# we1pingyu/CALD

Hardware: AMD Instinct MI355X
Metric: unlabeled images scored/sec (CALD consistency sweep) (higher is better)
Workload: dtype f32

## Files before the change

### cald_amd/_ffi.py

```python
import ctypes as C
import os

_HERE = os.path.dirname(os.path.abspath(__file__))
LIB_PATH = os.path.join(_HERE, "lib", "libcaldhip.so")
_lib = None

c_f = C.POINTER(C.c_float)
c_i = C.POINTER(C.c_int)
c_i64 = C.POINTER(C.c_int64)
c_d = C.POINTER(C.c_double)
c_u8 = C.POINTER(C.c_uint8)
c_i8 = C.POINTER(C.c_int8)


class ModelCfg(C.Structure):
    _fields_ = [("arch", C.c_int), ("depth", C.c_int), ("num_classes", C.c_int), ("min_size", C.c_int),
                ("max_size", C.c_int), ("box_score_thresh", C.c_float), ("box_nms_thresh", C.c_float),
                ("detections_per_img", C.c_int), ("rpn_pre_nms_top_n", C.c_int), ("rpn_post_nms_top_n", C.c_int),
                ("rpn_nms_thresh", C.c_float), ("precision", C.c_int)]


PRECISION = {"fp32": 0, "f16x3": 1}


# ... 141 lines not shown
    "cald_op_gap": (C.c_int, [C.c_void_p, c_f, C.c_int, C.c_int, C.c_int, c_f]),
    "cald_op_lossnet": (C.c_int, [C.c_void_p, C.c_int, c_f, c_f]),
    "cald_op_consistency": (C.c_int, [C.c_void_p, C.c_int, c_f, c_f, c_f, C.c_int, c_f, c_f, c_f, C.c_int, C.c_float, c_f]),
    "cald_op_cls_corr": (C.c_int, [C.c_void_p, C.c_int, c_f, c_i64, C.c_int, c_f]),
    "cald_op_score_batch": (C.c_int, [C.c_void_p, C.POINTER(ScoreProbe)]),
    "cald_op_pair_params": (C.c_int, [C.c_int, C.c_int, C.c_int, C.c_double, c_f]),
    "cald_op_ls_tail": (C.c_int, [C.c_int, c_f, C.c_int, c_f, c_i, c_i, c_d]),
    "cald_op_coco_match": (C.c_int, [C.c_void_p, C.c_int, c_i64, c_i64, c_d, c_d, c_d, c_d, c_u8, c_u8, C.c_int, c_d, C.c_int, c_d,
                                     C.POINTER(C.c_int32), c_u8, c_u8]),
    "cald_op_voc_match": (C.c_int, [C.c_void_p, C.c_int, c_i64, c_i64, c_d, c_u8, c_d, c_i64, C.c_int, c_d, C.c_int64, c_d, c_i64, c_u8, c_u8]),
    "cald_op_pil_resize": (C.c_int, [C.c_void_p, C.c_void_p, C.c_int, C.c_int, C.c_void_p, C.c_int, C.c_int]),
    "cald_op_cutout_rects": (C.c_int, [C.c_uint64, C.c_int, C.c_int, C.c_int, c_f, C.c_int, c_i, c_i]),
    "cald_op_cutout_geometry": (C.c_int, [C.c_int, C.c_int, C.c_int, C.c_int, C.c_int, c_i, C.c_int, c_i, c_i]),
    "cald_op_augment": (C.c_int, [C.c_void_p, C.c_int, C.c_double, C.c_uint64, C.c_void_p, C.c_int, C.c_int, C.c_int, c_f,
                                  C.c_void_p, c_f, c_i]),
    "cald_op_noise_stream": (C.c_int, [C.c_void_p, C.c_uint64, C.c_void_p, C.c_int, C.c_int, C.c_int, c_i, c_d, C.POINTER(C.c_void_p)]),
    "cald_op_frcnn_postprocess": (C.c_int, [C.c_void_p, C.c_int, C.c_int, c_f, c_f, c_f, C.c_int, C.c_int, C.c_int, C.c_int, C.c_float, C.c_float,
                                            C.c_int, c_f, c_f, c_i64, c_f, c_f, c_f, c_i]),
    "cald_op_frcnn_postprocess_min": (C.c_int, [C.c_void_p, C.c_int, C.c_int, c_f, c_f, c_f, C.c_int, C.c_int, C.c_int, C.c_int, C.c_float, C.c_float,
                                                C.c_int, C.c_float, c_f, c_f, c_i64, c_f, c_f, c_f, c_i]),
    "cald_op_ssm_postprocess": (C.c_int, [C.c_void_p, C.c_int, C.c_int, c_f, c_f, c_f, C.c_int, C.c_int, C.c_int, C.c_int, C.c_float, C.c_int,
                                          c_i, c_i, c_f, c_f, c_i8]),
    "cald_op_retina_postprocess": (C.c_int, [C.c_void_p, C.POINTER(c_f), C.POINTER(c_f), c_i, C.c_int, C.c_int, c_f] + [C.c_int] * 6
                                   + [C.c_float, C.c_float, C.c_int, c_f, c_f, c_i64, c_f, c_f, c_i]),
    "cald_op_retina_ssm_postprocess": (C.c_int, [C.c_void_p, C.POINTER(c_f), C.POINTER(c_f), c_i, C.c_int, C.c_int, c_f] + [C.c_int] * 6
                                       + [C.c_float, C.c_float, C.c_int, C.c_void_p, C.c_void_p, c_i, c_i, c_i, c_f, c_f, c_i8]),
    "cald_op_rpn_prune": (C.c_int, [C.c_void_p, C.POINTER(RpnPruneProbe)]),
    "cald_op_roi_align": (C.c_int, [C.c_void_p, C.POINTER(c_f), c_i, C.c_int, C.c_int, c_f, c_f]),
    "cald_op_conv2d": (C.c_int, [C.c_void_p, c_f, C.c_int, C.c_int, C.c_int, c_f, C.c_int, C.c_int, C.c_int, C.c_int,
                                 C.c_int, c_f, c_f, c_f, c_f, C.c_int, c_f]),
    "cald_op_conv_probe": (C.c_int, [C.c_void_p, C.c_int, C.POINTER(ConvProbe), C.c_int, C.c_int, C.c_int, C.c_char_p, C.c_int]),
    "cald_op_mfma_f16": (C.c_int, [C.c_void_p, C.POINTER(C.c_uint16), C.POINTER(C.c_uint16), C.POINTER(C.c_uint32), C.POINTER(C.c_uint32), C.c_int64]),
    "cald_op_conv2d_f16x3": (C.c_int, [C.c_void_p, c_f, C.c_int, C.c_int, C.c_int, c_f, C.c_int, C.c_int, C.c_int, C.c_int,
                                       C.c_int, c_f, c_f, c_f, c_f, C.c_int, c_f]),
    "cald_op_conv_bench": (C.c_int, [C.c_void_p] + [C.c_int] * 12 + [c_d, c_d]),
    "cald_op_row_pack_lookup": (C.c_int, [C.c_int, c_i, c_i, C.c_int, C.c_int, C.c_int64, c_i64, c_i, c_i64, c_i64]),
    "cald_op_transform_size": (C.c_int, [C.c_int, C.c_int, C.c_int, C.c_int, c_i, c_i, c_i, c_i]),
    "cald_debug_tensor": (C.c_int, [C.c_void_p, C.c_char_p, C.c_int, c_f, C.c_int64, c_i64]),
    "cald_jpeg_info": (C.c_int, [C.c_void_p, C.c_size_t, c_i, c_i, c_i]),
    "cald_jpeg_decode_batch": (C.c_int, [C.c_void_p, C.c_int, C.POINTER(C.c_void_p), C.POINTER(C.c_size_t), C.POINTER(C.c_void_p)]),
    "cald_jpeg_probe": (C.c_int, [C.c_void_p, C.c_size_t, c_i, c_i, c_i, c_i]),
    "cald_jpeg_decode_batch_any": (C.c_int, [C.c_void_p, C.c_int, C.POINTER(C.c_void_p), C.POINTER(C.c_size_t), C.POINTER(C.c_void_p)]),
    "cald_jpeg_decode_host": (C.c_int, [C.c_void_p, C.c_size_t, C.c_void_p]),
    "cald_profile_enable": (C.c_int, [C.c_void_p, C.c_int]),
    "cald_profile_read": (C.c_int, [C.c_void_p, c_d, c_d, c_i64, c_d]),
    "cald_profile_prune": (C.c_int, [C.c_void_p, c_d, c_d, c_d, c_d, c_d]),
    "cald_profile_roi_rows": (C.c_int, [C.c_void_p, c_d, c_i64]),
    "cald_profile_cutout": (C.c_int, [C.c_void_p, c_d, c_d, c_i64, c_i64]),
    "cald_model_set_cutout_reuse": (C.c_int, [C.c_void_p, C.c_int, c_i]),
    "cald_profile_cutout_stages": (C.c_int, [C.c_void_p, c_d, c_d, c_d, c_d, c_i64]),
    "cald_model_set_cutout_retention_cap": (C.c_int, [C.c_void_p, C.c_int64, c_i64]),
    "cald_op_cutout_fpn_geometry": (C.c_int, [C.c_int, C.c_int, C.c_int, C.c_int, C.c_int, c_i, C.c_int, c_i, c_i]),
    "cald_model_set_look_fuse": (C.c_int, [C.c_void_p, C.c_int, c_i]),
    "cald_model_set_row_packing": (C.c_int, [C.c_void_p, C.c_int, c_i]),
    "cald_model_set_box_min_size": (C.c_int, [C.c_void_p, C.c_float, c_f]),
    "cald_profile_dump": (C.c_int, [C.c_void_p, C.c_char_p]),
    "cald_train_packed_floats": (C.c_int, [C.c_int] * 6 + [c_i64]),
    "cald_train_pack_conv": (C.c_int, [C.c_void_p] * 5 + [C.c_int] * 6 + [C.c_void_p]),
    "cald_train_pack_plan_scratch_floats": (C.c_int, [C.c_int, C.POINTER(PackJob), c_i64]),
    "cald_train_pack_plan_create": (C.c_int, [C.c_void_p, C.c_int, C.POINTER(PackJob), C.c_void_p, C.c_int64, C.POINTER(C.c_void_p)]),
    "cald_train_pack_plan_run": (C.c_int, [C.c_void_p, C.c_void_p]),
    "cald_train_pack_plan_destroy": (C.c_int, [C.c_void_p]),
    "cald_train_conv": (C.c_int, [C.c_void_p, C.c_int, C.c_int, C.c_int, C.c_void_p, C.c_int, C.c_void_p] + [C.c_int] * 8
                        + [C.c_void_p, C.c_void_p, C.c_int, C.c_int, C.c_void_p, C.c_void_p, C.c_int]),
    "cald_train_conv_group": (C.c_int, [C.c_void_p, C.c_int, C.c_int, c_i, C.POINTER(C.c_void_p), C.c_int, C.POINTER(C.c_void_p)] + [C.c_int] * 8
                              + [C.POINTER(C.c_void_p), C.POINTER(C.c_void_p), C.c_int]),
    "cald_train_conv_wgrad": (C.c_int, [C.c_void_p, C.c_int, C.c_int, C.c_int, C.c_void_p, C.c_int, C.c_int, C.c_void_p, C.c_int,
                                        C.c_int, C.c_int, C.c_int, C.c_int, C.c_int, C.c_void_p, C.c_void_p, C.c_void_p, C.c_int]),
    "cald_train_linear_wgrad": (C.c_int, [C.c_void_p, C.c_int, C.c_void_p, C.c_int, C.c_void_p, C.c_int, C.c_int, C.c_int,
                                          C.c_void_p, C.c_void_p, C.c_int]),
    "cald_train_wgrad_plan": (C.c_int, [C.c_longlong] + [C.c_int] * 12 + [C.POINTER(WgradPlan)]),
    "cald_train_relu_bwd": (C.c_int, [C.c_void_p, C.c_longlong, C.c_int, C.c_void_p, C.c_void_p, C.c_void_p]),
    "cald_train_add": (C.c_int, [C.c_void_p, C.c_longlong, C.c_void_p, C.c_void_p, C.c_void_p]),
    "cald_train_dilate": (C.c_int, [C.c_void_p] + [C.c_int] * 7 + [C.c_void_p, C.c_void_p]),
    "cald_train_upsample_bwd": (C.c_int, [C.c_void_p] + [C.c_int] * 6 + [C.c_void_p, C.c_void_p]),
    "cald_train_rpn_proposals": (C.c_int, [C.c_void_p, C.c_int, C.c_int, C.c_int, c_i, C.POINTER(C.c_void_p), c_i, C.c_int, C.c_int, C.c_int,
                                           C.c_float, C.c_float, C.c_void_p, C.c_void_p]),
    "cald_train_roi_sample_host": (C.c_int, [C.c_int, c_i, c_i, c_i, C.c_void_p, C.c_void_p, C.c_void_p, C.c_int, C.c_double, C.c_int, C.c_int,
                                             C.c_void_p, C.c_void_p, C.c_void_p, C.c_void_p, C.c_void_p, C.c_void_p, c_i, c_i, c_i]),
    "cald_train_roi_gather": (C.c_int, [C.c_void_p, C.c_void_p, C.c_void_p, C.c_void_p, C.c_int, C.c_int, C.c_int] + [C.c_float] * 4 + [C.c_void_p, C.c_void_p]),
    "cald_train_anchors": (C.c_int, [C.c_void_p, C.c_int, C.c_int, C.c_int, c_i, C.c_void_p]),
    "cald_train_match": (C.c_int, [C.c_void_p, C.c_int, C.c_void_p, C.c_int, C.c_void_p, C.c_float, C.c_float, C.c_int, C.c_void_p, C.c_void_p]),
    "cald_train_box_encode": (C.c_int, [C.c_void_p, C.c_int, C.c_void_p, C.c_void_p, C.c_float, C.c_float, C.c_float, C.c_float, C.c_void_p]),
    "cald_train_roi_align": (C.c_int, [C.c_void_p, C.POINTER(C.c_void_p), c_i, C.c_int, C.c_int, C.c_void_p, C.c_void_p]),
    "cald_train_roi_align_bwd": (C.c_int, [C.c_void_p, C.c_int, C.POINTER(C.c_void_p), c_i, C.c_int, C.c_int, C.c_void_p, C.c_void_p]),
    "cald_train_softmax_ce": (C.c_int, [C.c_void_p, C.c_int, C.c_int, C.c_int, C.c_void_p, C.c_void_p, C.c_float, C.c_void_p, C.c_void_p]),
    "cald_train_smooth_l1": (C.c_int, [C.c_void_p, C.c_int, C.c_void_p, C.c_void_p, C.c_void_p, C.c_float, C.c_float, C.c_void_p, C.c_float,
                                       C.c_void_p, C.c_void_p]),
    "cald_train_focal_loss": (C.c_int, [C.c_void_p, C.c_int, c_i, C.c_int, C.c_int, C.c_int, C.c_void_p, C.c_void_p, C.c_void_p, C.c_void_p,
                                        C.c_void_p, C.c_float, C.c_float, C.c_void_p, C.c_void_p]),
    "cald_train_bce_logits": (C.c_int, [C.c_void_p, C.c_int, C.c_void_p, C.c_void_p, C.c_void_p, C.c_float, C.c_void_p, C.c_void_p]),
    "cald_train_softmax_ce_seg": (C.c_int, [C.c_void_p, C.c_int, c_i, C.c_int, C.c_int, C.c_void_p, C.c_void_p, C.c_void_p, C.c_void_p, C.c_void_p]),
    "cald_train_smooth_l1_seg": (C.c_int, [C.c_void_p, C.c_int, c_i, C.c_void_p, C.c_void_p, C.c_void_p, C.c_float, c_f, C.c_void_p, C.c_void_p,
                                           C.c_void_p]),
    "cald_train_bce_logits_seg": (C.c_int, [C.c_void_p, C.c_int, c_i, C.c_void_p, C.c_void_p, C.c_void_p, C.c_void_p, C.c_void_p, C.c_void_p]),
    "cald_train_focal_loss_seg": (C.c_int, [C.c_void_p, C.c_int, c_i, C.c_int, C.c_int, C.c_int, C.c_void_p, C.c_void_p, C.c_void_p, C.c_void_p,
                                            c_f, C.c_float, C.c_void_p, C.c_void_p, C.c_void_p, C.c_void_p]),
    "cald_train_seg_mean": (C.c_int, [C.c_void_p, C.c_int, C.c_void_p, C.c_void_p]),
    "cald_train_add_bcast": (C.c_int, [C.c_void_p, C.c_int, C.c_longlong, C.c_int, C.c_void_p, C.c_void_p, C.c_void_p, C.c_void_p, C.c_longlong]),
    "cald_train_preprocess": (C.c_int, [C.c_void_p, C.c_int, C.POINTER(C.c_void_p), C.POINTER(C.c_void_p), c_i, C.c_int, C.c_int, C.c_void_p]),
    "cald_train_maxpool": (C.c_int, [C.c_void_p, C.c_int, C.c_int, C.c_int, C.c_int, C.c_void_p, C.c_void_p]),
    "cald_train_subsample2": (C.c_int, [C.c_void_p, C.c_int, C.c_int, C.c_int, C.c_int, C.c_void_p, C.c_void_p]),
    "cald_train_sgd": (C.c_int, [C.c_void_p, C.c_longlong, C.c_void_p, C.c_void_p, C.c_void_p, C.c_float, C.c_float, C.c_float, C.c_int]),
    "cald_train_seg_cache_size": (C.c_int, []),
    "cald_comm_unique_id": (C.c_int, [C.c_void_p]),
    "cald_comm_init_rank": (C.c_int, [C.c_void_p, C.c_void_p, C.c_int, C.c_int, C.POINTER(C.c_void_p)]),
# ... 36 lines not shown
```

### cald_amd/csrc/conv_h4.hip

```cpp
#include "h16.h"

typedef float f32x16 __attribute__((ext_vector_type(16)));
typedef _Float16 h8 __attribute__((ext_vector_type(8)));
typedef __attribute__((address_space(3))) void lds_void;

#define H4_STAGE 32768
#define H4_NSTAGE 4

template <int EPI, bool HEAD = false>
__device__ __forceinline__ void conv_h4_body(const ConvArgs& a, const int blk) {
    extern __shared__ __attribute__((aligned(1024))) unsigned char smem[];
    const int tid = threadIdx.x, lane = tid & 63, wave = __builtin_amdgcn_readfirstlane(tid >> 6);
    const int NT = a.CoutPad >> 8;
    const int MT2 = (a.total_mtiles + 1) >> 1;
    int mt2, nt;
    {
        const int total = MT2 * NT, b = blk, xcd = b & 7, idx = b >> 3, Q = total >> 3, R = total & 7;
        const int L = (xcd < R ? xcd * (Q + 1) : R * (Q + 1) + (xcd - R) * Q) + idx;
        mt2 = L / NT; nt = L - mt2 * NT;
    }
    const int n0 = nt << 8;
    const int Cin = a.Cin, KW = a.KW, KH = a.KH, CoutPad = a.CoutPad;

    const bool ldA = wave < 4;
    const int lw = wave & 3;
    const int l_row = lane >> 2;
    const int l_piece = (lane & 3) ^ ((lane >> 4) & 3);
    int voff[4];
    unsigned rowmask[4];
    __amdgpu_buffer_rsrc_t rs;
    int Wi_l = 1;
    if (ldA) {
        const int mt = 2 * mt2 + (lw >> 1);
        const int v = seg_find_view(a.seg_out, a.V, mt);
        const LevelSeg so = a.seg_out[v], si = a.seg_in[v];
        const int Wo = so.W, Hi = si.H, Wi = si.W;
        Wi_l = Wi;
        int Mv = so.H * Wo;
        if (a.dyn_rows) { const int d = a.dyn_rows[v]; Mv = d < Mv ? d : Mv; }
        if (mt >= a.total_mtiles) Mv = 0;
        const int mrow0 = (mt - so.tile_start) * 128 + (lw & 1) * 64;
#pragma unroll
        for (int i = 0; i < 4; i++) {
            const int m = mrow0 + 16 * i + l_row;
            const int oy = m / Wo, ox = m - oy * Wo;
            const int iy0 = oy * a.stride - a.pad, ix0 = ox * a.stride - a.pad;
            unsigned msk = 0;
            if (m < Mv)
                for (int t = 0; t < KH * KW; t++) {
                    const int th = t / KW, tw = t - th * KW;
                    const int iy = iy0 + th, ix = ix0 + tw;
                    if (iy >= 0 && iy < Hi && ix >= 0 && ix < Wi) msk |= 1u << t;
                }
            rowmask[i] = msk;
            voff[i] = ((oy * a.stride) * Wi + ox * a.stride) * Cin * 4 + l_piece * 16;
        }
        const unsigned char* in_v = reinterpret_cast<const unsigned char*>(a.in16) + (si.pix_off * (long long)Cin - (long long)a.pad * (Wi + 1) * Cin) * 4;
        rs = __builtin_amdgcn_make_buffer_rsrc((void*)in_v, 0, 0x7FFE0000, 0x00020000);
    } else {
#pragma unroll
        for (int i = 0; i < 4; i++) {
            const int n = 64 * lw + 16 * i + l_row;
            rowmask[i] = 0xffffffffu;
            voff[i] = ((l_piece >> 1) * CoutPad + n) * 32 + (l_piece & 1) * 16;
        }
        rs = __builtin_amdgcn_make_buffer_rsrc((void*)(reinterpret_cast<const unsigned char*>(a.w16) + (long long)n0 * 32), 0, 0x7FFE0000, 0x00020000);
    }
    const int lds_l = (ldA ? 0 : 16384) + lw * 4096;
    int u_kh = 0, u_kw = 0, u_ci = 0, u_kt = 0;

#define H4_ISSUE(SLOT)                                                                                                       \
    {                                                                                                                        \
        const int soffA = ((u_kh * Wi_l + u_kw) * Cin + u_ci) * 4, soffB = u_kt * (2 * CoutPad * 32);                        \
        const int soff = ldA ? soffA : soffB;                                                                                \
        const unsigned bit = ldA ? (1u << (u_kh * KW + u_kw)) : 1u;                                                          \
        _Pragma("unroll") for (int i = 0; i < 4; i++) {                                                                      \
            const int vo = (rowmask[i] & bit) ? voff[i] : 0x7FFF0000;                                                        \
            __builtin_amdgcn_raw_ptr_buffer_load_lds(rs, (lds_void*)(smem + (SLOT) * H4_STAGE + lds_l + i * 1024), 16, vo, soff, 0, 0); \
        }                                                                                                                    \
        u_kt++; u_kw++;                                                                                                      \
        const bool ww = u_kw == KW; u_kw = ww ? 0 : u_kw; u_kh += ww ? 1 : 0;                                                \
        const bool wh = u_kh == KH; u_kh = wh ? 0 : u_kh; u_ci += wh ? 16 : 0;                                               \
    }

    const int wm = wave >> 2, wn = wave & 3;
    const int l31 = lane & 31, kh_lane = lane >> 5, sw = (l31 >> 2) & 3;
    const int fa = (wm * 128 + l31) * 64, fb = 16384 + (wn * 64 + l31) * 64;
    const int s_hi = ((kh_lane) ^ sw) * 16, s_lo = ((2 + kh_lane) ^ sw) * 16;

    f32x16 acc[4][2];
#pragma unroll
    for (int i = 0; i < 4; i++)
#pragma unroll
        for (int j = 0; j < 2; j++)
#pragma unroll
            for (int r = 0; r < 16; r++) acc[i][j][r] = 0.0f;

    const int KT = a.Kpad >> 4;
// ... 92 lines not shown
#undef H4_MFMA4
#undef H4_READ
#undef H4_ISSUE
#undef H4_STEP

    if (HEAD) {
        int tid = threadIdx.x;
        asm volatile("" : "+v"(tid));
        const int wave = __builtin_amdgcn_readfirstlane(tid >> 6), wm = wave >> 2, wn = wave & 3, l31 = tid & 31, kh_lane = (tid >> 5) & 1;
        const float unscale = a.w16_unscale;
        const float bs0 = a.bias[wn * 64 + l31], bs1 = a.bias[wn * 64 + 32 + l31];
        const bool have2 = 2 * mt2 + 1 < a.total_mtiles;
#pragma unroll
        for (int t = 0; t < 2; t++) {
            __syncthreads();
            if (wm == 0 || have2) {
                int sbase = (wm << 16) + (kh_lane << 12) + (((wn * 16 + (l31 >> 2)) ^ (4 * kh_lane)) << 4) + (l31 & 3) * 4;
                asm volatile("" : "+v"(sbase));
#pragma unroll
                for (int j = 0; j < 2; j++) {
                    const float bs = j ? bs1 : bs0;
#pragma unroll
                    for (int ii = 0; ii < 2; ii++)
#pragma unroll
                        for (int r = 0; r < 16; r++) {
                            float val = acc[2 * t + ii][j][r] * unscale;
                            val = val + bs;
                            val = val > 0.0f ? val : 0.0f;
                            const int rc = ii * 32 + (r & 3) + 8 * (r >> 2);
                            *reinterpret_cast<float*>(smem + (sbase ^ (((j << 7) ^ (rc << 4)) | (rc << 10)))) = val;
                        }
                }
            }
            __syncthreads();
            if (wave < 6) {
                const int srow = tid & 127, q = wave >> 1;
                const int mt = 2 * mt2 + (srow >> 6);
                if (mt < a.total_mtiles) {
                    const int v = seg_find_view(a.seg_out, a.V, mt);
                    const LevelSeg so = a.seg_out[v];
                    const int m = (mt - so.tile_start) * 128 + 64 * t + (srow & 63);
                    const float4* const hrow = reinterpret_cast<const float4*>(smem + srow * 1024);
                    typedef const __attribute__((address_space(4))) float cfloat;
                    cfloat* const w = (cfloat*)a.head_w + q * 256;
                    float s0 = 0.0f;
#pragma unroll 16
                    for (int g = 0; g < 64; g++) {
                        const float4 hv = hrow[(g ^ srow) & 63];
                        s0 = __builtin_fmaf(hv.x, w[4 * g], s0);
                        s0 = __builtin_fmaf(hv.y, w[4 * g + 1], s0);
                        s0 = __builtin_fmaf(hv.z, w[4 * g + 2], s0);
                        s0 = __builtin_fmaf(hv.w, w[4 * g + 3], s0);
                    }
                    if (m < so.H * so.W) a.head_out[(so.pix_off + m) * (long long)a.head_ld + q] = s0 + a.head_b[q];
                }
            }
        }
        return;
    }

    const int mt = 2 * mt2 + wm;
    if (mt >= a.total_mtiles) return;
    const int v = seg_find_view(a.seg_out, a.V, mt);
    const LevelSeg so = a.seg_out[v];
    int Mv = so.H * so.W;
    if (a.dyn_rows) { const int d = a.dyn_rows[v]; Mv = d < Mv ? d : Mv; }
    const int m0 = (mt - so.tile_start) * 128;
    if (m0 >= Mv) return;
    h16_epilogue<EPI, 4, 2>(a, acc, so, v, m0, n0 + wn * 64, Mv, lane);
}

template <int EPI>
__global__ __launch_bounds__(512, 2) void conv_h4_kernel(const ConvArgs a) { conv_h4_body<EPI>(a, (int)blockIdx.x); }
__global__ __launch_bounds__(512, 2) void conv_h4_group_kernel(const ConvGroup g) {
    int i = 0;
    while (i + 1 < g.n && g.blk0[i + 1] <= (int)blockIdx.x) i++;
    const int local = (int)blockIdx.x - g.blk0[i];
    const ConvArgs& a = g.p[i];
    if (local >= ((a.total_mtiles + 1) >> 1) * (a.CoutPad >> 8)) return;
    conv_h4_body<0>(a, local);
}

__global__ __launch_bounds__(512, 2) void conv_h4_look_kernel(const ConvGroup g) {
    int i = 0;
    while (i + 1 < g.n && g.blk0[i + 1] <= (int)blockIdx.x) i++;
    const int local = (int)blockIdx.x - g.blk0[i];
    const ConvArgs& a = g.p[i];
    if (local >= (a.total_mtiles + 1) >> 1) return;
    conv_h4_body<0, true>(a, local);
}

static bool h4_covers(const ConvArgs& a) {
    if (a.head_out && !(a.head_w && a.head_ld >= 3 && a.Cout == 256 && a.CoutPad == 256 && !a.residual && !a.up && !a.dyn_rows && a.bias && !a.scale && a.relu)) return false;
    return a.w16 && a.in16 && !a.in_relu && a.CoutPad % 256 == 0 && a.Cin % 16 == 0 && a.KH * a.KW <= 32 && !a.mask && !(a.residual && a.up) &&
           !a.gather && !a.row_map && !a.energy4 && (a.out || a.out16 || a.head_out);
}
static int h4_mode() { static const int mode = getenv("CALD_H4") ? atoi(getenv("CALD_H4")) : 1; return mode; }
static PerDeviceOnce h4_once[5];
const char* launch_conv_h4(const ConvArgs& a, hipStream_t stream, bool forced) {
    if (!(forced || h4_mode()) || !h4_covers(a) || a.head_out) return nullptr;
    const int wgs = ((a.total_mtiles + 1) >> 1) * (a.CoutPad >> 8);
    if (!forced && h4_mode() == 1 && (a.Kpad < 1024 || wgs < 512)) return nullptr;
    if (wgs == 0) return "none (no output tiles)";
    const dim3 grid((unsigned)wgs), block(512);
    const size_t lds = (size_t)H4_NSTAGE * H4_STAGE;
    if (a.residual) { allow_big_lds(h4_once[1], conv_h4_kernel<1>); hipLaunchKernelGGL((conv_h4_kernel<1>), grid, block, lds, stream, a); return "conv_h4_kernel<1>"; }
    if (a.up) { allow_big_lds(h4_once[2], conv_h4_kernel<2>); hipLaunchKernelGGL((conv_h4_kernel<2>), grid, block, lds, stream, a); return "conv_h4_kernel<2>"; }
    allow_big_lds(h4_once[0], conv_h4_kernel<0>); hipLaunchKernelGGL((conv_h4_kernel<0>), grid, block, lds, stream, a);
    return "conv_h4_kernel<0>";
}
static int h4_group_plan(const ConvArgs* p, int n, bool forced, ConvGroup* g, int* blocks) {
    if (!(forced || h4_mode()) || n < 1 || n > CALD_MAX_GROUP) return 0;
    int blk = 0;
    const bool head = p[0].head_out != nullptr;
    for (int i = 0; i < n; i++) {
        if (!h4_covers(p[i]) || p[i].residual || p[i].up || (p[i].head_out != nullptr) != head) return 0;
        if (g) { g->blk0[i] = blk; g->p[i] = p[i]; }
        blk += (((p[i].total_mtiles + 1) >> 1) * (p[i].CoutPad >> 8) + 7) & ~7;
    }
    if (g) { g->n = n; g->blk0[n] = blk; }
    if (!forced && h4_mode() == 1 && (blk < 512 || p[0].Kpad < 1024)) return 0;
    *blocks = blk;
    return blk == 0 ? 2 : 1;
}
bool conv_h4_group_takes(const ConvArgs* p, int n, bool forced) { int blk; return h4_group_plan(p, n, forced, nullptr, &blk) != 0; }
const char* launch_conv_h4_group(const ConvArgs* p, int n, hipStream_t stream, bool forced) {
    ConvGroup g; int blk = 0;
    const int take = h4_group_plan(p, n, forced, &g, &blk);
    if (!take) return nullptr;
    if (take == 2) return "none (no output tiles)";
    if (p[0].head_out) {
        allow_big_lds(h4_once[4], conv_h4_look_kernel);
        hipLaunchKernelGGL(conv_h4_look_kernel, dim3((unsigned)blk), dim3(512), (size_t)H4_NSTAGE * H4_STAGE, stream, g);
        return "conv_h4_look_kernel";
    }
    allow_big_lds(h4_once[3], conv_h4_group_kernel);
    hipLaunchKernelGGL(conv_h4_group_kernel, dim3((unsigned)blk), dim3(512), (size_t)H4_NSTAGE * H4_STAGE, stream, g);
    return "conv_h4_group_kernel";
}
```

### cald_amd/csrc/ctx.hip

```cpp
#include "host.h"

static thread_local char g_err[512] = "";
int cald_host::fail(int code, const char* fmt, ...) {
    va_list ap; va_start(ap, fmt); vsnprintf(g_err, sizeof(g_err), fmt, ap); va_end(ap);
    return code;
}

int cald_internal_fail(int code, const char* fmt, ...) {
    va_list ap; va_start(ap, fmt); vsnprintf(g_err, sizeof(g_err), fmt, ap); va_end(ap);
    return code;
}
void cald_internal_train_release(cald_ctx* c);

extern "C" const char* cald_last_error(void) { return g_err; }
extern "C" int cald_version(void) { return 100; }

hipStream_t cald_internal_stream(cald_ctx* c) { return c->stream; }
int cald_internal_device(cald_ctx* c) { return c->device; }
const float* cald_internal_zeros(cald_ctx* c) { return c->d_zeros; }
int cald_internal_scratch(cald_ctx* c, size_t bytes, void** out) {
    if (bytes > c->train_scratch_cap) {
        HIPCHK(hipStreamSynchronize(c->stream));
        if (c->train_scratch) HIPCHK(hipFree(c->train_scratch));
        c->train_scratch = nullptr; c->train_scratch_cap = 0;
// ... 109 lines not shown
    return 0;
}

extern "C" int cald_profile_prune(cald_ctx* c, double* look_ms, double* look_flops, double* selected_frac2, double* worst_bound_ratio, double* pruned_flops) {
    if (!c) return fail(CALD_ERR_INVALID, "ctx is null");
    HIPCHK(hipStreamSynchronize(c->stream));
    double ms = 0.0, fl = 0.0;
    for (const ProfLaunch& L : c->prof_launches)
        if (L.tag) { float t = 0.f; HIPCHK(hipEventElapsedTime(&t, L.e0, L.e1)); ms += t; fl += L.flops; }
    unsigned long long st[4] = {0, 0, 0, 0};
    HIPCHK(hipMemcpy(st, c->d_prune_stat, 32, hipMemcpyDeviceToHost));
    if (look_ms) *look_ms = ms;
    if (look_flops) *look_flops = fl;
    if (selected_frac2) for (int l = 0; l < 2; l++) selected_frac2[l] = st[2 * l + 1] ? (double)st[2 * l] / (double)st[2 * l + 1] : 0.0;
    if (worst_bound_ratio) *worst_bound_ratio = (double)c->prune_worst;
    if (pruned_flops) {
        double fl2 = 0.0;
        for (int l = 0; l < 2; l++) if (st[2 * l + 1]) fl2 += c->prof_prune_flops_cap[l] / 2.0 * (1.0 - (double)st[2 * l] / (double)st[2 * l + 1]);
        *pruned_flops = fl2;
    }
    return 0;
}

extern "C" int cald_profile_roi_rows(cald_ctx* c, double* mean_rows_per_view, int64_t* views) {
    if (!c) return fail(CALD_ERR_INVALID, "ctx is null");
    HIPCHK(hipStreamSynchronize(c->stream));
    unsigned long long rows = 0;
    HIPCHK(hipMemcpy(&rows, c->d_roi_rows, 8, hipMemcpyDeviceToHost));
    if (views) *views = c->prof_roi_views;
    if (mean_rows_per_view) *mean_rows_per_view = c->prof_roi_views ? (double)rows / (double)c->prof_roi_views : 0.0;
    return 0;
}

extern "C" int cald_profile_cutout(cald_ctx* c, double* rows3, double* dense_rows3, int64_t* batches, int64_t* fallbacks) {
    if (!c) return fail(CALD_ERR_INVALID, "ctx is null");
    for (int i = 0; i < 3; i++) { if (rows3) rows3[i] = c->cut_rows[i]; if (dense_rows3) dense_rows3[i] = c->cut_dense[i]; }
    if (batches) *batches = c->cut_batches;
    if (fallbacks) *fallbacks = c->cut_fallbacks;
    return 0;
}

extern "C" int cald_profile_cutout_stages(cald_ctx* c, double* rows6, double* dense_rows6, double* tiles6, double* dense_tiles6, int64_t* kept3) {
    if (!c) return fail(CALD_ERR_INVALID, "ctx is null");
    for (int i = 0; i < 6; i++) {
        if (rows6) rows6[i] = c->cut_st_rows[i];
        if (dense_rows6) dense_rows6[i] = c->cut_st_dense[i];
        if (tiles6) tiles6[i] = c->cut_st_tiles[i];
        if (dense_tiles6) dense_tiles6[i] = c->cut_st_dense_tiles[i];
    }
    if (kept3) for (int i = 0; i < 3; i++) kept3[i] = c->cut_kept[i];
    return 0;
}

extern "C" int cald_profile_dump(cald_ctx* c, const char* path) {
    if (!c || !path) return fail(CALD_ERR_INVALID, "null argument");
    HIPCHK(hipStreamSynchronize(c->stream));
    FILE* f = fopen(path, "w");
    if (!f) return fail(CALD_ERR_INVALID, "cannot open %s", path);
    fprintf(f, "launch,desc,gflop,ms,tflops\n");
    std::vector<unsigned long long> lg((size_t)CALD_PRUNE_LOG * 4, 0ull);
    if (!c->prof_gather.empty()) HIPCHK(hipMemcpy(lg.data(), c->d_prune_log, lg.size() * 8, hipMemcpyDeviceToHost));
    for (size_t i = 0; i < c->prof_launches.size(); i++) {
        const ProfLaunch& L = c->prof_launches[i];
        float t = 0.f; hipEventElapsedTime(&t, L.e0, L.e1);
        double fl = L.flops;
        const char* extra = L.tag ? ",f16x3-lookahead" : "";
        auto g = c->prof_gather.find(i);
        if (g != c->prof_gather.end()) {
            for (int l = 0; l < 2; l++) {
                const unsigned long long sel = lg[(size_t)g->second.log * 4 + 2 * l], tot = lg[(size_t)g->second.log * 4 + 2 * l + 1];
                if (tot) fl -= g->second.cap[l] * (1.0 - (double)sel / (double)tot);
            }
            extra = ",gathered-rows";
        }
        fprintf(f, "%zu,\"%s%s\",%.3f,%.4f,%.2f\n", i, L.desc.c_str(), extra, fl / 1e9, t, fl / (t * 1e-3) / 1e12);
    }
    fclose(f);
    return 0;
}
extern "C" int cald_profile_prune_fallbacks(cald_ctx* c, int64_t* n) {
    if (!c || !n) return fail(CALD_ERR_INVALID, "null argument");
    *n = (int64_t)c->prune_fallbacks;
    return 0;
}

int cald_host::prof_begin(cald_ctx* c, ProfLaunch& t) {
    if (!c->prof) return 0;
    HIPCHK(hipEventCreate(&t.e0)); HIPCHK(hipEventCreate(&t.e1));
    HIPCHK(hipEventRecord(t.e0, c->stream));
    return 0;
}
int cald_host::prof_end(cald_ctx* c, ProfLaunch& t, double flops, int tag, const char* fmt, ...) {
    if (!c->prof) return 0;
    HIPCHK(hipEventRecord(t.e1, c->stream));
    char d[160];
    va_list ap; va_start(ap, fmt); vsnprintf(d, sizeof(d), fmt, ap); va_end(ap);
    t.flops = flops; t.tag = tag; t.desc = d;
    c->prof_launches.push_back(t); c->prof_flops += flops;
    return 0;
}

int cald_host::conv_refused(const ConvArgs& a) {
    return fail(CALD_ERR_UNSUPPORTED, "no conv kernel implements this launch (Cin=%d Cout=%d k=%dx%d residual=%d up=%d mask=%d gather=%d energy4=%d out16=%d)",
                a.Cin, a.Cout, a.KH, a.KW, a.residual != nullptr, a.up != nullptr, a.mask != nullptr, a.gather != nullptr, a.energy4 != nullptr,
                a.out16 != nullptr);
}
// ... 9 lines not shown
```

### cald_amd/csrc/forward.hip

```cpp
#include "host.h"

#define ROI_DENSE_VIEWS 32
void cald_host::build_plan(BatchPlan& P, int V, const ViewDesc* views, const int (*hp)[2], bool retina) {
    memset(&P, 0, sizeof(P));
    for (int l = 0; l < CALD_MAX_LEVELS; l++) {
        long long off = 0; int tile = 0;
        for (int v = 0; v <= V; v++) {
            LevelSeg& s = P.seg[l][v];
            s.pix_off = off; s.tile_start = tile;
            if (v == V) break;
            int H, W;
            if (l == 7 && retina) { int h6 = (hp[v][0] / 32 - 1) / 2 + 1, w6 = (hp[v][1] / 32 - 1) / 2 + 1; H = (h6 - 1) / 2 + 1; W = (w6 - 1) / 2 + 1; }
            else if (l == 7) { H = 1; W = CALD_ROI_CAP; }
            else if (l == 8) {
                const int first = v * ROI_DENSE_VIEWS, cnt = first < V ? (V - first < ROI_DENSE_VIEWS ? V - first : ROI_DENSE_VIEWS) : 0;
                H = cnt ? 1 : 0; W = cnt * CALD_ROI_CAP;
            }
            else if (l == 6) { H = (hp[v][0] / 32 - 1) / 2 + 1; W = (hp[v][1] / 32 - 1) / 2 + 1; }
            else { H = hp[v][0] >> l; W = hp[v][1] >> l; }
            s.H = H; s.W = W;
            off += (long long)H * W;
            tile += (H * W + 127) / 128;
        }
    }
// ... 14 lines not shown
        T1 = B.get<float>(px[2] * 128); T2 = B.get<float>(px[2] * 64); D = B.get<float>(px[2] * 256);
        for (int i = 0; i < 4; i++) { Cf[i] = B.get<float>(px[2 + i] * CCH[i]); S.only(Cf[i]); }
        S.only(p1); S.only(T1); S.only(T2); S.only(X[0]); S.only(X[1]); S.only(D);
    }
};
struct PyramidBufs {
    float *inner[4], *Pf[5]; unsigned* Pf16[5];
    void layout(Bump& B, SplitReg& S, const long long* px, bool retina) {
        const int first = retina ? 3 : 2, nl = retina ? 3 : 4;
        for (int i = 0; i < nl; i++) { inner[i] = B.get<float>(px[first + i] * 256); S.only(inner[i]); }
        for (int i = 0; i < 5; i++) {
            Pf[i] = B.get<float>(px[first + i] * 256);
            if (i == 4 || (retina && i < 3)) S.only(Pf[i]); else S.both(Pf[i], Pf16[i], px[first + i] * 256);
        }
    }
};
void cald_host::RetinaTailBufs::layout(Bump& B, int V, int K, int per_class, int maxa) {
    max_anchors = maxa;
    cand_cap = 1024; while (cand_cap < maxa) cand_cap <<= 1;
    cand_count = B.get<int>((size_t)V * K); cand_key = B.get<unsigned long long>((size_t)V * K * cand_cap);
    cand_box = B.get<float>((size_t)V * K * cand_cap * 4); cand_skip = B.get<unsigned char>((size_t)V * K * cand_cap);
    kept_anchor = B.get<int>((size_t)V * K * per_class); kept_box = B.get<float>((size_t)V * K * per_class * 4); kept_count = B.get<int>((size_t)V * K);
}
void cald_host::RetinaSsmBufs::layout(Bump& B, int V, int K, int per_class, int maxa) {
    cand_cap = maxa > 0 ? maxa : 1; nblk = (cand_cap + 255) / 256;
    const size_t VK = (size_t)V * K, rows = VK * per_class;
    cand_count = B.get<int>(VK); blk_off = B.get<int>(VK * nblk); list = B.get<int>(VK * cand_cap); vmax = B.get<unsigned>(V); al = B.get<int>(V);
    picks = B.get<int>(VK * CALD_SSM_RETINA_TAKE); n_picks = B.get<int>(VK);
    kept_anchor = B.get<int>(rows); kept_box = B.get<float>(rows * 4); kept_count = B.get<int>(VK);
    row_off = B.get<int>(VK); count = B.get<int>(V); total = B.get<int>(1);
    boxes = B.get<float>(rows * 4); scores = B.get<float>(rows); labels = B.get<signed char>(rows * (K - 1));
}
struct RetinaBufs {
    float *ret_t[2][2][5], *cls_h[5], *reg_h[5]; RetinaTailBufs tail;
    void layout(Bump& B, SplitReg& S, const long long* px, int V, int cls_ld, int K, int per_class, int max_anchors, RetinaSsmBufs* ssm_tail) {
        for (int h = 0; h < 2; h++) for (int q = 0; q < 2; q++) for (int i = 0; i < 5; i++) { ret_t[h][q][i] = B.get<float>(px[3 + i] * 256); S.only(ret_t[h][q][i]); }
        for (int i = 0; i < 5; i++) { cls_h[i] = B.get<float>(px[3 + i] * cls_ld); reg_h[i] = B.get<float>(px[3 + i] * 36); }
        if (ssm_tail) ssm_tail->layout(B, V, K, per_class, max_anchors); else tail.layout(B, V, K, per_class, max_anchors);
    }
};
void cald_host::ProposalBufs::layout(Bump& B, int V) { proposals = B.get<float>((size_t)V * CALD_ROI_CAP * 4); prop_count = B.get<int>(V); }
struct RpnBufs {
    float *rpn_tl[5], *rpn_h[5], *cand_box, *sorted_box, *sorted_raw; unsigned long long* cand_key; int* sorted_count; ProposalBufs prop;
    void layout(Bump& B, const long long* px, int V, int pre) {
        for (int i = 0; i < 5; i++) { rpn_tl[i] = B.get<float>(px[2 + i] * 256); rpn_h[i] = B.get<float>(px[2 + i] * 15); }
        cand_key = B.get<unsigned long long>((size_t)V * 5 * pre); cand_box = B.get<float>((size_t)V * 5 * pre * 4);
        sorted_box = B.get<float>((size_t)V * 5 * pre * 4); sorted_raw = B.get<float>((size_t)V * 5 * pre * 4); sorted_count = B.get<int>(V);
        prop.layout(B, V);
    }
};
struct PruneBufs {
    float *energy[2] = {}, *pn[2] = {}, *rows[2][2] = {}; int *map[2][2] = {}, *nsel[2] = {}; unsigned* p16[2] = {}; unsigned* tau = nullptr;
    float* look[2] = {};
    void layout(Bump& B, const long long* px, int V, bool capture) {
        for (int i = 0; i < 2; i++) {
            energy[i] = B.get<float>(px[2 + i] * 4); pn[i] = B.get<float>(px[2 + i]); p16[i] = B.get<unsigned>(px[2 + i] * 256);
            for (int s2 = 0; s2 < 2; s2++) { rows[s2][i] = B.get<float>(px[2 + i] * 15); map[s2][i] = B.get<int>(px[2 + i]); }
            if (capture) look[i] = B.get<float>(px[2 + i] * 15);
        }
        for (int s2 = 0; s2 < 2; s2++) nsel[s2] = B.get<int>((size_t)2 * V);
        tau = B.get<unsigned>((size_t)2 * V);
    }
};
void cald_host::RoiBufs::layout(Bump& B, int V, int C) { order = B.get<int>((size_t)V * 1024); roi = B.get<float>((size_t)V * CALD_ROI_CAP * 49 * C); }
void cald_host::PostBufs::layout(Bump& B, int V, int C, int cap) {
    key_cap = cap;
    prob = B.get<float>((size_t)V * CALD_ROI_CAP * C); pmax = B.get<float>((size_t)V * CALD_ROI_CAP);
    keys = B.get<unsigned long long>((size_t)V * key_cap); cbox = B.get<float>((size_t)V * 2 * key_cap * 4); key_count = B.get<int>(V);
    skip = B.get<unsigned char>((size_t)V * key_cap);
}
void cald_host::SsmBufs::layout(Bump& B, int V, int C, int cap) {
    const size_t K = (size_t)(C - 1), rows = (size_t)V * K * cap;
    prob = B.get<float>((size_t)V * CALD_ROI_CAP * C); vmax = B.get<unsigned>(V);
    kept_prop = B.get<int>(rows); kept_box = B.get<float>(rows * 4); cls_count = B.get<int>((size_t)V * K); row_off = B.get<int>((size_t)V * K);
    al = B.get<int>(V); count = B.get<int>(V); total = B.get<int>(1);
    boxes = B.get<float>(rows * 4); scores = B.get<float>(rows * K); labels = B.get<signed char>(rows * K);
}
struct BoxBufs {
    RoiBufs roi; float *f6, *f7, *pr; PostBufs post;
    void layout(Bump& B, SplitReg& S, int V, int pred_ld, int C, int key_cap) {
        roi.layout(B, V, 256);
        f6 = B.get<float>((size_t)V * CALD_ROI_CAP * 1024); f7 = B.get<float>((size_t)V * CALD_ROI_CAP * 1024);
        S.only(roi.roi); S.only(f6); S.only(f7);
        pr = B.get<float>((size_t)V * CALD_ROI_CAP * pred_ld);
        post.layout(B, V, C, key_cap);
    }
};
struct AuditBufs {
    unsigned long long *next_key, *trunc_key, *kept_key; float* post_maxc;
    void layout(Bump& B, int V, int det_cap) {
        next_key = B.get<unsigned long long>((size_t)V * 10); trunc_key = B.get<unsigned long long>((size_t)V * 2);
        kept_key = B.get<unsigned long long>((size_t)V * det_cap); post_maxc = B.get<float>(V);
    }
};

RoiArgs cald_host::roi_args(const RoiBufs& S, const float* const* feat, const BatchPlan* plan, int C, int V, const ProposalBufs& P, bool out16) {
    RoiArgs ro{};
    for (int i = 0; i < 4; i++) { ro.feat[i] = feat[i]; ro.seg[i] = plan->seg[2 + i]; }
    ro.C = C; ro.V = V; ro.proposals = P.proposals; ro.prop_count = P.prop_count; ro.out = S.roi; ro.order = S.order; ro.out16 = out16 ? 1 : 0;
    return ro;
}
PostArgs cald_host::post_args(const PostBufs& S, const float* pred, int pred_ld, int C, int V, const ProposalBufs& P, const ViewDesc* views,
                              float score_thr, float nms_thr, const DetBuffers& det) {
    PostArgs pa{};
    pa.pred = pred; pa.pred_ld = pred_ld; pa.C = C; pa.V = V; pa.proposals = P.proposals; pa.prop_count = P.prop_count; pa.views = views; pa.score_thr = score_thr; pa.nms_thr = nms_thr;
    pa.prob = S.prob; pa.pmax = S.pmax; pa.keys = S.keys; pa.cbox = S.cbox; pa.key_count = S.key_count; pa.key_cap = S.key_cap; pa.det = det;
    pa.skip = S.skip;
    return pa;
}
// ... 57 lines not shown
    for (int v = 0; v < V; v++) {
        const LevelSeg& s = seg[v];
        if (!(s.H % 8 == 0 && s.W % 16 == 0 && seg[v + 1].tile_start - s.tile_start == (s.H / 8) * (s.W / 16))) return false;
    }
    return true;
}
static double fill_conv_args(cald_model* m, ConvArgs& a, const ConvLayer& L, const float* in, float* out, int lin, int lout, int V, bool relu,
                             const float* residual = nullptr, const float* up = nullptr, int lup = 0, const int* dyn = nullptr,
                             bool in_relu = false) {
    const BatchPlan* dp = m->ctx->d_plan;
    a.in = in; a.out = out; a.w = L.w; a.w4 = L.w4; a.w16 = L.w16; a.w16_unscale = L.w16_unscale; a.bias = L.bias; a.scale = L.scale; a.shift = L.shift;
    a.residual = residual; a.up = up;
    a.seg_in = dp->seg[lin]; a.seg_out = dp->seg[lout]; a.seg_up = dp->seg[lup];
    a.dyn_rows = dyn; a.row_map = nullptr; a.gather = nullptr; a.V = V;
    a.Cin = L.Cin; a.Cout = L.Cout; a.CoutPad = L.CoutPad; a.Kpad = L.Kpad;
    a.KH = L.KH; a.KW = L.KW; a.stride = L.stride; a.pad = L.pad; a.relu = relu ? 1 : 0;
    a.total_mtiles = level_tiles(m->plan, lout, V); a.packed_rows = 0;
    a.out_ld = L.Cout; a.in_relu = in_relu ? 1 : 0; a.zeros = m->ctx->d_zeros;
    a.mask = nullptr;
    for (int v = 0; v < V; v++) {
        const long long pin = (long long)m->plan.seg[lin][v].H * m->plan.seg[lin][v].W, pout = (long long)m->plan.seg[lout][v].H * m->plan.seg[lout][v].W;
        if (pin * L.Cin * 4 > 0x7FFE0000LL || pout * L.Cout * 4 > 0x7FFE0000LL) {
            return (double)fail(CALD_ERR_UNSUPPORTED, "a view's activation tensor exceeds 2 GB (level %d -> %d, %lld x %d / %lld x %d elements)", lin, lout, pin, L.Cin, pout, L.Cout);
        }
    }
    a.in16 = nullptr; a.out16 = nullptr; a.ex16 = 0; a.energy4 = nullptr; a.trace = nullptr;
    a.head_w = nullptr; a.head_out = nullptr; a.head_ld = 0; a.head_b[0] = a.head_b[1] = a.head_b[2] = 0.0f;
    if (!m->split.empty()) {
        const float* ex = residual ? residual : up;
        if (ex) {
            auto fe = m->split.find(ex);
            if (fe != m->split.end() && fe->second.fp32_dead) {
                if (!a.w16) return (double)fail(CALD_ERR_STATE, "a layer outside conv_h3 / conv_h4 adds a tensor kept in split form only");
                a.ex16 = 1;
            }
        }
        auto fi = m->split.find(in);
        if (fi != m->split.end()) {
            if (a.w16 && !in_relu) a.in16 = fi->second.s16;
            else if (fi->second.fp32_dead) return (double)fail(CALD_ERR_STATE, "a layer outside conv_h3 reads a tensor kept in split form only");
        }
        auto fo = m->split.find(out);
        if (fo != m->split.end()) {
            if (!a.w16) return (double)fail(CALD_ERR_STATE, "a layer outside conv_h3 writes a tensor with a split twin");
            a.out16 = fo->second.s16;
            if (fo->second.fp32_dead) a.out = nullptr;
        }
    }
    a.wstem = L.wstem && stem_grid_exact(m->plan.seg[lout], V) ? L.wstem : nullptr;
    return 2.0 * (double)level_pix(m->plan, lout, V) * (double)L.Cout * (double)(L.KH * L.KW * L.CinTrue);
}
bool cald_host::conv_pack_default() {
    static const bool on = !(getenv("CALD_CONV_PACK") && atoi(getenv("CALD_CONV_PACK")) == 0);
    return on;
}
static void offer_packing(cald_model* m, ConvArgs& a, int lin, int lout, int lup, int V) {
    if (!(m->row_packing < 0 ? conv_pack_default() : m->row_packing != 0) || a.dyn_rows || a.row_map || a.gather || a.mask) return;
    a.packed_rows = conv_pack_rows(m->plan.seg[lin], m->plan.seg[lout], a.up ? m->plan.seg[lup] : nullptr, V, a.Cin, a.out_ld);
}
static int conv_on(cald_model* m, const ConvLayer& L, const float* in, float* out, int lin, int lout, int V, bool relu,
                   const float* residual = nullptr, const float* up = nullptr, int lup = 0, const int* dyn = nullptr,
                   bool in_relu = false) {
    ConvArgs a;
    const double flops = fill_conv_args(m, a, L, in, out, lin, lout, V, relu, residual, up, lup, dyn, in_relu);
    if (flops < 0.0) return (int)flops;
    offer_packing(m, a, lin, lout, lup, V);
    return run_conv(m->ctx, a, flops);
}
static int conv_pair_on(cald_model* m, const ConvLayer& L2, const ConvLayer& L3, const float* in, float* mid, float* out, int lin, int lout,
                        int V, const float* residual) {
    cald_ctx* c = m->ctx;
    if (m->cfg.precision == CALD_PRECISION_FP32 && L2.stride == 1 && lin == lout) {
        ConvArgs a2, a3;
            const double f2 = fill_conv_args(m, a2, L2, in, mid, lin, lout, V, true);
        const double f3 = fill_conv_args(m, a3, L3, mid, out, lout, lout, V, true, residual);
        if (f2 < 0.0 || f3 < 0.0) return (int)(f2 < 0.0 ? f2 : f3);
        ProfLaunch t; int rc;
        if ((rc = prof_begin(c, t))) return rc;
        if (launch_conv_p4_fused(a2, a3, c->stream) != nullptr)
            return prof_end(c, t, f2 + f3, 0, "mt=%d,Cin=%d,Cout=%d,k=3x3+1x1,s=1,fused->%d", a2.total_mtiles, a2.Cin, a2.Cout, a3.Cout);
        if (c->prof) { hipEventDestroy(t.e0); hipEventDestroy(t.e1); }
    }
    int rc = conv_on(m, L2, in, mid, lin, lout, V, true);
    if (rc) return rc;
    return conv_on(m, L3, mid, out, lout, lout, V, true, residual);
}
static int conv_group_on(cald_model* m, const ConvSpec* sp, int n, int V) {
    ConvArgs a[CALD_MAX_GROUP];
    double flops = 0.0; int tiles = 0;
    for (int i = 0; i < n; i++) {
        const double f = fill_conv_args(m, a[i], *sp[i].L, sp[i].in, sp[i].out, sp[i].level, sp[i].level, V, sp[i].relu, nullptr, nullptr, 0, sp[i].dyn);
        if (f < 0.0) return (int)f;
        a[i].row_map = sp[i].row_map;
        if (sp[i].in16) a[i].in16 = sp[i].in16;
        if (sp[i].out16) a[i].out16 = sp[i].out16;
        a[i].energy4 = sp[i].energy4;
        offer_packing(m, a[i], sp[i].level, sp[i].level, 0, V);
        flops += f; tiles += a[i].total_mtiles;
    }
    cald_ctx* c = m->ctx;
    const char* names[CALD_MAX_GROUP];
    ProfLaunch t; int rc;
    if ((rc = prof_begin(c, t))) return rc;
    const int launches = launch_conv_group(a, n, c->stream, names);
    if (c->prof) c->prof_extra_launches += launches - 1;
    if ((rc = prof_end(c, t, flops, c->prof_tag_now, "mt=%d,Cin=%d,Cout=%d,k=%dx%d,s=%d,group=%d", tiles, a[0].Cin, a[0].Cout, a[0].KH, a[0].KW, a[0].stride, n))) return rc;
// ... 113 lines not shown
        HIPCHK(hipEventSynchronize(c->stage_ev[si]));
        memcpy(c->h_stage[si], &m->plan, sizeof(BatchPlan));
        memcpy(c->h_stage[si] + sizeof(BatchPlan), views, sizeof(ViewDesc) * V);
        HIPCHK(hipMemcpyAsync(c->d_plan, c->h_stage[si], sizeof(BatchPlan), hipMemcpyHostToDevice, c->stream));
        HIPCHK(hipMemcpyAsync(c->d_views, c->h_stage[si] + sizeof(BatchPlan), sizeof(ViewDesc) * V, hipMemcpyHostToDevice, c->stream));
        HIPCHK(hipEventRecord(c->stage_ev[si], c->stream));
        dp = c->d_plan; st = c->stream;
        m->dbg.clear();
        return 0;
    }
    int dense_block(const Bottleneck& B, const float* cur, float* dst, int lvl, int lout) {
        int rc; const float* idn = cur;
        if (B.has_down) { if ((rc = conv_on(m, B.down, cur, Fb.D, lvl, lout, V, false))) return rc; idn = Fb.D; }
        if ((rc = conv_on(m, B.c1, cur, Fb.T1, lvl, lvl, V, true))) return rc;
        return conv_pair_on(m, B.c2, B.c3, Fb.T1, Fb.T2, dst, lvl, lout, V, idn);
    }
    int gathered_block(const Bottleneck& B, int b, const float* cur, float* dst, int lvl, int lout) {
        int rc; const float* idn = cur;
        if (B.has_down) { if ((rc = gconv_on(m, B.down, cur, Fb.D, lvl, lout, V, false, nullptr, *ru, b, 0))) return rc; idn = Fb.D; }
        if ((rc = gconv_on(m, B.c1, cur, Fb.T1, lvl, lvl, V, true, nullptr, *ru, b, 1))) return rc;
        if ((rc = gconv_on(m, B.c2, Fb.T1, Fb.T2, lvl, lout, V, true, nullptr, *ru, b, 0))) return rc;
        return gconv_on(m, B.c3, Fb.T2, dst, lout, lout, V, true, idn, *ru, b, 0);
    }
    int body() {
        int rc;
        launch_preprocess(c->d_views, dp->seg[0], Fb.in0, V, max_pix0, st);
        m->dbg["input"] = {Fb.in0, 0, 4, 0};
        if ((rc = conv_on(m, m->conv1, Fb.in0, Fb.c1, 0, 1, V, true))) return rc;
        m->dbg["conv1"] = {Fb.c1, 1, 64, 0};
        launch_maxpool(Fb.c1, Fb.p1, dp->seg[1], dp->seg[2], 64, V, max_pix2, st, m->split.count(Fb.p1) != 0);
        m->dbg["pool1"] = {Fb.p1, 2, 64, 0};
        const float* cur = Fb.p1; int lvl = 2, layer = 0, xi = 0;
        for (size_t b = 0; b < m->blocks.size(); b++) {
            const Bottleneck& B = m->blocks[b];
            const int lout = lvl + (B.c2.stride == 2 ? 1 : 0);
            const bool kept = ru && (int)b < ru->nblk;
            float* dst = kept ? ru->out[b] : (B.layer_end ? Fb.Cf[layer] : Fb.X[xi]);
            if ((rc = kept && ru->mode == 2 && ru->gather[layer] ? gathered_block(B, (int)b, cur, dst, lvl, lout) : dense_block(B, cur, dst, lvl, lout))) return rc;
            if (B.layer_end) Fb.Cf[layer] = dst;
            cur = dst; lvl = lout;
            if (B.layer_end) layer++; else xi ^= 1;
        }
        const char* cn[4] = {"C2", "C3", "C4", "C5"};
        for (int i = 0; i < 4; i++) m->dbg[cn[i]] = {Fb.Cf[i], 2 + i, CCH[i], 0};
        return 0;
    }
    void name_pyramid(int first, int n) { for (int i = 0; i < n; i++) m->dbg["P" + std::to_string(first + i)] = {Fp.Pf[i], first + i, 256, 0}; }
    int fpn() {
        const int first = retina ? 3 : 2, nl = retina ? 3 : 4, c0 = 4 - nl;
        int rc; ConvSpec sp[4];
        const bool kept = ru && ru->fpn && !retina;
        if (kept) {
            for (int i = 0; i < 4; i++) Fp.Pf[i] = ru->pf[i];
            if (prune) for (int i = 0; i < 2; i++) { Fq.p16[i] = ru->p16[i]; Fq.energy[i] = ru->energy[i]; }
        }
        if ((rc = conv_on(m, m->fpn_inner[nl - 1], Fb.Cf[3], Fp.inner[nl - 1], 5, 5, V, false))) return rc;
        for (int i = nl - 2; i >= 0; i--)
            if ((rc = conv_on(m, m->fpn_inner[i], Fb.Cf[c0 + i], Fp.inner[i], first + i, first + i, V, false, nullptr, Fp.inner[i + 1], first + 1 + i))) return rc;
        for (int i = 0; i < nl; i++) m->dbg["inner" + std::to_string(first + i)] = {Fp.inner[i], first + i, 256, 0};
        for (int i = 0; i < nl; i++) sp[i] = {&m->fpn_layer[i], Fp.inner[i], Fp.Pf[i], first + i, false};
        if (prune)
            for (int i = 0; i < 2; i++) { sp[i].out16 = Fq.p16[i]; sp[i].energy4 = Fq.energy[i]; }
        if ((rc = kept && ru->mode == 2 && ru->gather_fpn ? gconv_group_on(m, sp, nl, V, *ru) : conv_group_on(m, sp, nl, V))) return rc;
        if (!retina) return 0;
        if ((rc = conv_on(m, m->p6, Fp.Pf[2], Fp.Pf[3], 5, 6, V, false))) return rc;
        if (feat && !feat->p7) return 0;
        return conv_on(m, m->p7, Fp.Pf[3], Fp.Pf[4], 6, 7, V, false, nullptr, nullptr, 0, nullptr, true);
    }
    void hand_out(int first, int n) {
        name_pyramid(first, n);
        for (int i = 0; i < n; i++) {
            auto sp = m->split.find(Fp.Pf[i]);
            feat->P[i] = Fp.Pf[i]; feat->split_only[i] = sp != m->split.end() && sp->second.fp32_dead; feat->plan_level[i] = first + i;
        }
    }
    int retina_head_and_tail() {
        int rc;
        for (int t = 0; t < 4; t++) {
            ConvSpec sp[10];
            for (int hsel = 0; hsel < 2; hsel++)
                for (int i = 0; i < 5; i++)
                    sp[hsel * 5 + i] = {&(hsel == 0 ? m->cls_tower : m->reg_tower)[t], t == 0 ? Fp.Pf[i] : Fr.ret_t[hsel][(t - 1) & 1][i],
                                        Fr.ret_t[hsel][t & 1][i], 3 + i, true};
            if ((rc = conv_group_on(m, sp, 10, V))) return rc;
        }
        for (int hsel = 0; hsel < 2; hsel++) {
            ConvSpec sp[5];
            for (int i = 0; i < 5; i++) sp[i] = {hsel == 0 ? &m->cls_out : &m->reg_out, Fr.ret_t[hsel][1][i], hsel == 0 ? Fr.cls_h[i] : Fr.reg_h[i], 3 + i, false};
            if ((rc = conv_group_on(m, sp, 5, V))) return rc;
        }
        for (int i = 0; i < 5; i++) {
            m->dbg["cls" + std::to_string(i)] = {Fr.cls_h[i], 3 + i, m->cls_out.Cout, 0};
            m->dbg["reg" + std::to_string(i)] = {Fr.reg_h[i], 3 + i, 36, 0};
        }
        if (rssm) return retina_ssm_tail();
        launch_retina_postprocess(retina_args(Fr.tail, Fr.cls_h, Fr.reg_h, dp, c->d_views, m->d_anchors, 9, m->cfg.num_classes, V, m->cfg.box_score_thresh,
                                              m->cfg.box_nms_thresh, m->cfg.detections_per_img, det), Fr.tail.max_anchors, st);
        return 0;
    }
    int retina_ssm_tail() {
        const RetinaSsmArgs sa = retina_ssm_args(rssm->out, Fr.cls_h, Fr.reg_h, dp, c->d_views, m->d_anchors, 9, m->cfg.num_classes, V, m->cfg.box_score_thresh,
                                                 m->cfg.box_nms_thresh, m->cfg.detections_per_img);
        launch_retina_ssm_phase_a(sa, st);
        HIPCHK(hipGetLastError());
        if (int rc = retina_ssm_pick_stop(c, rssm->out, V, m->cfg.num_classes, rssm->pick, rssm->user, rssm->image0, nullptr)) return rc;
        launch_retina_ssm_phase_b(sa, st);
        return 0;
    }
    void p6_subsample() {
        auto tw = m->split.find(Fp.Pf[3]);
        const bool p6_split = m->split.count(Fp.Pf[4]) != 0 && tw != m->split.end();
        launch_subsample2(p6_split ? reinterpret_cast<const float*>(tw->second.s16) : Fp.Pf[3], Fp.Pf[4], dp->seg[5], dp->seg[6], 256, V, max_pix6, st);
        name_pyramid(2, 5);
    }
    void name_rpn(int first) { for (int i = first; i < 5; i++) m->dbg["rpn" + std::to_string(i)] = {Fn.rpn_h[i], 2 + i, 15, 0}; }
    int rpn_dense() {
        int rc; ConvSpec sp[5];
        for (int i = 0; i < 5; i++) sp[i] = {&m->rpn_conv, Fp.Pf[i], Fn.rpn_tl[i], 2 + i, true};
        if ((rc = conv_group_on(m, sp, 5, V))) return rc;
        for (int i = 0; i < 5; i++) sp[i] = {&m->rpn_head, Fn.rpn_tl[i], Fn.rpn_h[i], 2 + i, false};
        if ((rc = conv_group_on(m, sp, 5, V))) return rc;
        name_rpn(0);
        return 0;
    }
    int look_fused_on(const ConvSpec* sp, bool* fused) {
        ConvArgs a[2]; double flops = 0.0; int tiles = 0;
        for (int i = 0; i < 2; i++) {
            const double f = fill_conv_args(m, a[i], *sp[i].L, sp[i].in, nullptr, sp[i].level, sp[i].level, V, sp[i].relu);
            if (f < 0.0) return (int)f;
            a[i].in16 = sp[i].in16;
            a[i].head_w = m->look_head_w; a[i].head_out = Fn.rpn_h[i]; a[i].head_ld = 15;
            for (int q = 0; q < 3; q++) a[i].head_b[q] = m->look_head_b[q];
            flops += f + 2.0 * (double)level_pix(m->plan, sp[i].level, V) * 256.0 * 3.0; tiles += a[i].total_mtiles;
        }
        if (!m->look_head_w || !conv_h4_group_takes(a, 2, m->look_fuse == 2)) return 0;
        if (m->prune_capture)
            for (int i = 0; i < 2; i++) HIPCHK(hipMemsetAsync(Fn.rpn_h[i], 0, (size_t)level_pix(m->plan, 2 + i, V) * 15 * sizeof(float), st));
        ProfLaunch t; int rc;
        if ((rc = prof_begin(c, t))) return rc;
        const char* k = launch_conv_h4_group(a, 2, st, m->look_fuse == 2);
        *fused = true;
        if (!k) { prof_end(c, t, 0.0, c->prof_tag_now, "refused"); return conv_refused(a[0]); }
        return prof_end(c, t, flops, c->prof_tag_now, "mt=%d,Cin=%d,Cout=%d,k=%dx%d,s=%d,group=2,head=3", tiles, a[0].Cin, a[0].Cout, a[0].KH, a[0].KW, a[0].stride);
    }
    int rpn_pruned() {
        int rc; ConvSpec sp[5];
        RpnPruneArgs pr;
        for (int i = 0; i < 2; i++) {
            pr.seg[i] = dp->seg[2 + i]; pr.energy[i] = Fq.energy[i]; pr.pnorm[i] = Fq.pn[i]; pr.head[i] = Fn.rpn_h[i]; pr.head_out[i] = Fn.rpn_h[i];
            for (int s2 = 0; s2 < 2; s2++) { pr.head_rows[s2][i] = Fq.rows[s2][i]; pr.row_map[s2][i] = Fq.map[s2][i]; }
        }
        int log_slot[2];
        for (int s2 = 0; s2 < 2; s2++) {
            log_slot[s2] = (c->prof && c->prune_log_n < CALD_PRUNE_LOG) ? c->prune_log_n++ : -1;
            pr.nsel[s2] = Fq.nsel[s2]; pr.log[s2] = log_slot[s2] >= 0 ? c->d_prune_log + (size_t)log_slot[s2] * 4 : nullptr;
        }
        pr.tau_key = Fq.tau; pr.stat = c->prof ? c->d_prune_stat : nullptr; pr.check = c->d_prune_check;
        for (int q = 0; q < 3; q++) { pr.c1[q] = m->prune_c1[q]; pr.c0[q] = m->prune_c0[q]; }
        pr.head_ld = 15; pr.pre_n = m->cfg.rpn_pre_nms_top_n; pr.V = V;
        c->prof_tag_now = 1;
        for (int i = 0; i < 2; i++) { sp[i] = {&m->rpn_conv16, Fp.Pf[i], Fn.rpn_tl[i], 2 + i, true}; sp[i].in16 = Fq.p16[i]; }
        bool fused = false;
        rc = m->look_fuse ? look_fused_on(sp, &fused) : 0;
        if (!rc && !fused) {
            rc = conv_group_on(m, sp, 2, V);
            for (int i = 0; i < 2; i++) sp[i] = {&m->rpn_head, Fn.rpn_tl[i], Fn.rpn_h[i], 2 + i, false};
            if (!rc) rc = conv_group_on(m, sp, 2, V);
        }
        c->prof_tag_now = 0;
        if (rc) return rc;
        const double cap_conv[2] = {2.0 * (double)level_pix(m->plan, 2, V) * 2304.0 * 256.0, 2.0 * (double)level_pix(m->plan, 3, V) * 2304.0 * 256.0};
        const double cap_head[2] = {2.0 * (double)level_pix(m->plan, 2, V) * 256.0 * 15.0, 2.0 * (double)level_pix(m->plan, 3, V) * 256.0 * 15.0};
        if (m->prune_capture)
            for (int i = 0; i < 2; i++) {
                HIPCHK(hipMemcpyAsync(Fq.look[i], Fn.rpn_h[i], (size_t)level_pix(m->plan, 2 + i, V) * 15 * sizeof(float), hipMemcpyDeviceToDevice, st));
                const char* ln[2] = {"rpn_look0", "rpn_look1"}; const char* bn[2] = {"rpn_pnorm0", "rpn_pnorm1"};
                m->dbg[ln[i]] = {Fq.look[i], 2 + i, 15, 0}; m->dbg[bn[i]] = {Fq.pn[i], 2 + i, 1, 0};
            }
        for (int s2 = 0; s2 < 2; s2++) {
            const int np = s2 == 1 ? 5 : 2;
            launch_rpn_prune_select(pr, max_pix2, s2, st);
            for (int i = 0; i < np; i++) sp[i] = {&m->rpn_conv, Fp.Pf[i], Fn.rpn_tl[i], 2 + i, true};
            for (int i = 0; i < 2; i++) { sp[i].dyn = Fq.nsel[s2] + i * V; sp[i].row_map = Fq.map[s2][i]; }
            if ((rc = conv_group_on(m, sp, np, V))) return rc;
            if (c->prof) {
                for (int i = 0; i < 2; i++) c->prof_prune_flops_cap[i] += cap_conv[i];
                if (log_slot[s2] >= 0) c->prof_gather[c->prof_launches.size() - 1] = {log_slot[s2], {cap_conv[0], cap_conv[1]}};
            }
            for (int i = 0; i < np; i++) sp[i] = {&m->rpn_head, Fn.rpn_tl[i], i < 2 ? Fq.rows[s2][i] : Fn.rpn_h[i], 2 + i, false};
            for (int i = 0; i < 2; i++) sp[i].dyn = Fq.nsel[s2] + i * V;
            if ((rc = conv_group_on(m, sp, np, V))) return rc;
            if (c->prof) {
                for (int i = 0; i < 2; i++) c->prof_prune_flops_cap[i] += cap_head[i];
                if (log_slot[s2] >= 0) c->prof_gather[c->prof_launches.size() - 1] = {log_slot[s2], {cap_head[0], cap_head[1]}};
            }
        }
        launch_rpn_prune_scatter(pr, max_pix2, st);
        name_rpn(m->prune_capture ? 0 : 2);
        return 0;
    }
    void proposals() {
        RpnArgs ra;
        for (int i = 0; i < 5; i++) { ra.head[i] = Fn.rpn_h[i]; ra.seg[i] = dp->seg[2 + i]; }
        ra.seg0 = dp->seg[0]; ra.views = c->d_views; ra.base_anchors = m->d_anchors;
        ra.head_ld = 15; ra.A = 3; ra.V = V; ra.pre_n = m->cfg.rpn_pre_nms_top_n; ra.post_n = m->cfg.rpn_post_nms_top_n;
        ra.nms_thr = m->cfg.rpn_nms_thresh; ra.min_size = RPN_MIN_SIZE;
        ra.cand_key = Fn.cand_key; ra.cand_box = Fn.cand_box; ra.sorted_box = Fn.sorted_box; ra.sorted_raw = Fn.sorted_raw;
        ra.sorted_count = Fn.sorted_count; ra.proposals = Fn.prop.proposals; ra.prop_stride = CALD_ROI_CAP; ra.prop_count = Fn.prop.prop_count;
        ra.next_key = audit_out ? Fa.next_key : nullptr; ra.trunc_key = audit_out ? Fa.trunc_key : nullptr;
        launch_rpn(ra, st);
        m->dbg["proposals"] = {Fn.prop.proposals, 7, 4, 1};
    }
    int box_head() {
        int rc;
        launch_roi_align(roi_args(Fx.roi, Fp.Pf, dp, 256, V, Fn.prop, m->split.count(Fx.roi.roi) != 0), st);
        m->dbg["roi"] = {Fx.roi.roi, 7, 12544, 1};
// ... 108 lines not shown
```

### cald_amd/csrc/host.h

```cpp
#pragma once
#include "../../include/cald_hip.h"
#include "common.h"
#include "kernels.h"
#include "host_logic.h"

#include <climits>
#include <cmath>
#include <cstdarg>
#include <cstdio>
#include <cstring>
#include <algorithm>
#include <map>
#include <string>
#include <vector>

namespace cald_host {
int fail(int code, const char* fmt, ...);
#define HIPCHK(x) do { hipError_t e_ = (x); if (e_ != hipSuccess) return fail(CALD_ERR_HIP, "%s failed: %s (%s:%d)", #x, hipGetErrorString(e_), __FILE__, __LINE__); } while (0)

struct PilCoef { int ksize; int* d_bounds; int* d_kk; };
struct PilKey { int in, out, fid; bool operator<(const PilKey& o) const { return in != o.in ? in < o.in : (out != o.out ? out < o.out : fid < o.fid); } };
struct ProfLaunch {
    hipEvent_t e0 = nullptr, e1 = nullptr;
    double flops = 0.0;
    int tag = 0;
    std::string desc;
};
}
using namespace cald_host;

#define CALD_PRUNE_LOG 4096
struct cald_ctx {
    int device = 0;
    hipStream_t stream = nullptr;
    bool own_stream = false;
    char* arena = nullptr; size_t arena_cap = 0, arena_off = 0;
    BatchPlan* d_plan = nullptr;
    ViewDesc* d_views = nullptr;
    float* d_zeros = nullptr;
    static const int NSTAGE = 8;
    char* h_stage[NSTAGE] = {nullptr}; hipEvent_t stage_ev[NSTAGE] = {nullptr}; int stage_i = 0;
    bool prof = false;
    std::vector<ProfLaunch> prof_launches;
    double prof_flops = 0.0; int64_t prof_extra_launches = 0;
    int prof_tag_now = 0;
    double prof_prune_flops_cap[2] = {0.0, 0.0};
    hipEvent_t tot0 = nullptr, tot1 = nullptr; bool tot_open = false; double tot_ms = 0.0;
    float prune_worst = 0.0f;
    long long prune_fallbacks = 0;
    float* d_prune_check = nullptr;
    unsigned long long* d_prune_stat = nullptr;
    unsigned long long* d_prune_log = nullptr; int prune_log_n = 0;
    struct GatherNote { int log; double cap[2]; };
    std::map<size_t, GatherNote> prof_gather;
    unsigned long long* d_roi_rows = nullptr; double prof_roi_rows_cap = 0.0, prof_roi_flops_cap = 0.0; long long prof_roi_views = 0;
    std::map<PilKey, PilCoef> pil;
    char* train_scratch = nullptr; size_t train_scratch_cap = 0;
    double cut_rows[3] = {0.0, 0.0, 0.0}, cut_dense[3] = {0.0, 0.0, 0.0};
    long long cut_batches = 0, cut_fallbacks = 0;
    double cut_st_rows[6] = {}, cut_st_dense[6] = {}, cut_st_tiles[6] = {}, cut_st_dense_tiles[6] = {};
    long long cut_kept[3] = {0, 0, 0};
};

namespace cald_host {
struct ScopedDev {
    std::vector<void*> ptrs;
    hipStream_t st;
    explicit ScopedDev(hipStream_t s) : st(s) {}
    ~ScopedDev() { if (!ptrs.empty()) { hipStreamSynchronize(st); for (void* p : ptrs) hipFree(p); } }
    void release() { ptrs.clear(); }
    template <typename T> int alloc(T** out, size_t bytes) {
        HIPCHK(hipMalloc((void**)out, bytes ? bytes : 1));
        ptrs.push_back((void*)*out);
        return 0;
    }
    template <typename T> int upload(T** out, const void* h, size_t bytes) {
        *out = nullptr;
        if (!h) return 0;
        if (int rc = alloc(out, bytes)) return rc;
        HIPCHK(hipMemcpy((void*)*out, h, bytes, hipMemcpyHostToDevice));
        return 0;
    }
};
struct Bump {
    char* base; size_t off = 0; bool dry;
    explicit Bump(char* b, bool d) : base(b), dry(d) {}
    template <typename T> T* get(size_t count) {
        size_t bytes = (count * sizeof(T) + 255) & ~(size_t)255;
        T* p = dry ? nullptr : reinterpret_cast<T*>(base + off);
        off += bytes;
        return p;
    }
};

struct HostTensor { std::vector<float> data; std::vector<int64_t> shape; };
struct ConvLayer {
    float *w = nullptr, *w4 = nullptr, *bias = nullptr, *scale = nullptr, *shift = nullptr;
    float* wstem = nullptr;
    uint16_t* w16 = nullptr; float w16_unscale = 1.0f;
    int Cin = 0, Cout = 0, CoutPad = 0, K = 0, Kpad = 0, KH = 1, KW = 1, stride = 1, pad = 0;
    int CinTrue = 0;
};
struct Bottleneck { ConvLayer c1, c2, c3, down; bool has_down = false; bool layer_end = false; };
struct DebugEntry { const float* ptr; int level; int C; int kind; };
}

struct cald_model {
    cald_ctx* ctx = nullptr;
    cald_model_cfg cfg;
    std::map<std::string, HostTensor> sd;
    bool finalized = false;
    ConvLayer conv1; std::vector<Bottleneck> blocks;
    ConvLayer fpn_inner[4], fpn_layer[4], rpn_conv, rpn_head, fc6, fc7, pred;
    ConvLayer rpn_conv16; bool prune = false; float prune_c1[3] = {0, 0, 0}, prune_c0[3] = {0, 0, 0};
    bool prune_allowed = false;
    int look_fuse = 1; float* look_head_w = nullptr; float look_head_b[3] = {0, 0, 0};
    int row_packing = -1;
    bool prune_bound_voided = false;
    bool prune_capture = false;
    ConvLayer p6, p7, cls_tower[4], reg_tower[4], cls_out, reg_out;
    int det_cap() const { return cfg.arch == CALD_ARCH_RETINANET ? cfg.num_classes * cfg.detections_per_img : cfg.detections_per_img; }
    float* d_anchors = nullptr;
    std::vector<void*> owned;
    std::map<std::string, DebugEntry> dbg;
    BatchPlan plan; int last_V = 0;
    struct SplitFmt { unsigned* s16; bool fp32_dead; };
    std::map<const float*, SplitFmt> split;
    std::vector<ViewDesc> last_views;
    DetBuffers sweep_det; int sweep_det_views = 0;
    DetBuffers sweep_det2; int sweep_det2_views = 0;
    struct SweepScratch {
        size_t dev_bytes = 0, pin_bytes = 0, aug_cap = 0;
        char* dev = nullptr; char* pin = nullptr; uint8_t* d_aug = nullptr;
        hipEvent_t ev_ref[2] = {nullptr, nullptr}, ev_score[2] = {nullptr, nullptr};
    } ss;
    float box_min_size = 0.0f;
    int key_cap = 32768;
    struct CutReuse {
        int mode = -1;
        char* slot[2] = {nullptr, nullptr}; size_t cap[2] = {0, 0};
        bool ext_refused = false;
        size_t ext_cap = 0;
        char* h_gp[2] = {nullptr, nullptr}; char* d_gp = nullptr;
    } cr;
};

namespace cald_host {
struct ConvPack {
    std::vector<float> w, w4, wstem;
    std::vector<uint16_t> w16; float w16_unscale = 1.0f;
    int Cout = 0, CoutPad = 0, K = 0, Kpad = 0;
};
struct ConvSpec { const ConvLayer* L; const float* in; float* out; int level; bool relu; const int* dyn = nullptr; const int* row_map = nullptr; const unsigned* in16 = nullptr;
                  unsigned* out16 = nullptr; float* energy4 = nullptr; };

#define CUT_MAX_BLOCKS 36
#define CUT_STAGE_LATERAL 4
#define CUT_STAGE_OUTPUT 5
#define CUT_KEPT_FPN 0
#define CUT_KEPT_STAGES 1
#define CUT_KEPT_NONE 2
struct FwdReuse {
    int mode = 0;
    int nblk = 0;
    float* out[CUT_MAX_BLOCKS] = {};
    bool gather[3] = {false, false, false};
    const char* d_gp = nullptr;
    int tiles[CUT_MAX_BLOCKS][2] = {};
    double rows[CUT_MAX_BLOCKS][2] = {};
    bool fpn = false, gather_fpn = false;
    float* pf[4] = {}; unsigned* p16[2] = {}; float* energy[2] = {};
    int fpn_tiles[4] = {};
    double fpn_rows[4] = {};
};
struct FwdFeatures {
    const int (*pad_to)[2] = nullptr;
    bool p7 = false;
    const float* P[5] = {}; bool split_only[5] = {}; int plan_level[5] = {};
};
struct ProposalBufs { float* proposals = nullptr; int* prop_count = nullptr; void layout(Bump& B, int V); };
struct RoiBufs { float* roi = nullptr; int* order = nullptr; void layout(Bump& B, int V, int C); };
struct PostBufs {
    float *prob = nullptr, *pmax = nullptr, *cbox = nullptr; unsigned long long* keys = nullptr; int* key_count = nullptr; int key_cap = 0;
    unsigned char* skip = nullptr;
    void layout(Bump& B, int V, int C, int key_cap);
};
struct SsmBufs {
    float *prob = nullptr, *kept_box = nullptr, *boxes = nullptr, *scores = nullptr; unsigned* vmax = nullptr; signed char* labels = nullptr;
    int *kept_prop = nullptr, *cls_count = nullptr, *row_off = nullptr, *al = nullptr, *count = nullptr, *total = nullptr;
    void layout(Bump& B, int V, int C, int cap);
};
struct FwdSsm { SsmBufs out; };
#define SSM_NMS_THR 0.3f
#define SSM_CONF_THR 0.5f
struct RetinaTailBufs {
    int *cand_count = nullptr, *kept_anchor = nullptr, *kept_count = nullptr, cand_cap = 0, max_anchors = 0; unsigned long long* cand_key = nullptr;
    float *cand_box = nullptr, *kept_box = nullptr; unsigned char* cand_skip = nullptr;
    void layout(Bump& B, int V, int K, int per_class, int max_anchors);
};
struct RetinaSsmBufs {
    int *cand_count = nullptr, *blk_off = nullptr, *list = nullptr, *al = nullptr, *picks = nullptr, *n_picks = nullptr, *kept_anchor = nullptr, *kept_count = nullptr,
        *row_off = nullptr, *count = nullptr, *total = nullptr, cand_cap = 0, nblk = 0;
    unsigned* vmax = nullptr; float *kept_box = nullptr, *boxes = nullptr, *scores = nullptr; signed char* labels = nullptr;
    void layout(Bump& B, int V, int K, int per_class, int max_anchors);
};
struct FwdRetinaSsm { cald_ssm_pick_fn pick = nullptr; void* user = nullptr; int image0 = 0; RetinaSsmBufs out; };
RetinaSsmArgs retina_ssm_args(const RetinaSsmBufs& S, const float* const* cls, const float* const* reg, const BatchPlan* plan, const ViewDesc* views,
                              const float* base_anchors, int A, int K, int V, float score_thr, float nms_thr, int per_class);
int retina_ssm_pick_stop(cald_ctx* c, const RetinaSsmBufs& S, int V, int K, cald_ssm_pick_fn pick, void* user, int image0, int* h_counts);
RoiArgs roi_args(const RoiBufs& S, const float* const* feat, const BatchPlan* plan, int C, int V, const ProposalBufs& P, bool out16);
PostArgs post_args(const PostBufs& S, const float* pred, int pred_ld, int C, int V, const ProposalBufs& P, const ViewDesc* views,
                   float score_thr, float nms_thr, const DetBuffers& det);
SsmArgs ssm_args(const SsmBufs& S, const float* pred, int pred_ld, int C, int V, const ProposalBufs& P, const ViewDesc* views, float score_thr, int cap);
RetinaArgs retina_args(const RetinaTailBufs& S, const float* const* cls, const float* const* reg, const BatchPlan* plan, const ViewDesc* views,
                       const float* base_anchors, int A, int K, int V, float score_thr, float nms_thr, int per_class, const DetBuffers& det);
inline size_t cut_plan_set_bytes(int V) { return (size_t)(V + 1) * sizeof(LevelSeg) + (size_t)V * sizeof(GatherSet); }
inline long long level_pix(const BatchPlan& P, int l, int V) { return P.seg[l][V].pix_off; }

int arena_reserve(cald_ctx* c, size_t bytes);
int prof_begin(cald_ctx* c, ProfLaunch& t);
int prof_end(cald_ctx* c, ProfLaunch& t, double flops, int tag, const char* fmt, ...);
int conv_refused(const ConvArgs& a);
int run_conv(cald_ctx* c, const ConvArgs& a, double flops);
int pil_resize(cald_ctx* c, const uint8_t* src, int H, int W, uint8_t* dst, int oh, int ow, uint8_t* tmp, int fid = 0);
std::vector<float> pack_w4(const std::vector<float>& w, int Kpad, int CoutPad);
void pack_conv(const std::vector<const float*>& ts, const std::vector<int>& couts, int cin, int cinp, int kh, int kw, int stride, int pad,
// ... 29 lines not shown
```

### cald_amd/csrc/host_logic.h

```cpp
#pragma once
#include <algorithm>
#include <cmath>
#include <cstdint>
#include <cstdio>
#include <cstdlib>
#include <cstring>
#include <vector>

static inline void transform_size(int H, int W, int min_size, int max_size, int* Hr, int* Wr, int* Hp, int* Wp) {
    double mn = (double)(H < W ? H : W), mx = (double)(H > W ? H : W);
    double scale = (double)min_size / mn;
    if (mx * scale > (double)max_size) scale = (double)max_size / mx;
    *Hr = (int)std::floor((double)H * scale);
    *Wr = (int)std::floor((double)W * scale);
    *Hp = ((*Hr + 31) / 32) * 32;
    *Wp = ((*Wr + 31) / 32) * 32;
}

struct PyRandom {
    uint32_t mt[624]; int idx;
    void init_genrand(uint32_t s) {
        mt[0] = s;
        for (int i = 1; i < 624; i++) mt[i] = 1812433253u * (mt[i - 1] ^ (mt[i - 1] >> 30)) + (uint32_t)i;
        idx = 624;
// ... 270 lines not shown
static inline bool cut_resize_span(int a, int b, int n_src, int nr, int* lo, int* hi) {
    const double sc = (double)n_src / (double)nr;
    int l = nr, h = -1;
    for (int y = 0; y < nr; y++) {
        double f = sc * ((double)y + 0.5) - 0.5; if (f < 0.0) f = 0.0;
        const int t0 = (int)f;
        if (t0 + 2 >= a && t0 - 1 <= b) { if (y < l) l = y; h = y; }
    }
    *lo = l; *hi = h;
    return l <= h;
}
static inline void cut_geometry(int H, int W, int Hr, int Wr, int Hp, int Wp, int nrect, const int* rects, int nblk, const int* stride,
                                CutSet* pool1, CutSet* out, CutSet* t1) {
    CutSet s; s.n = 0;
    for (int i = 0; i < nrect && i < CUT_SET_MAX; i++) {
        const int* q = rects + 4 * i;
        if (q[2] <= q[0] || q[3] <= q[1]) continue;
        CutRect r;
        if (cut_resize_span(q[0], q[2] - 1, W, Wr, &r.x0, &r.x1) && cut_resize_span(q[1], q[3] - 1, H, Hr, &r.y0, &r.y1)) s.r[s.n++] = r;
    }
    s = cut_map(s, 7, 2, 3, Hp >> 1, Wp >> 1);
    s = cut_map(s, 3, 2, 1, Hp >> 2, Wp >> 2);
    *pool1 = s;
    int l = 2;
    for (int b = 0; b < nblk; b++) {
        const int lo = l + (stride[b] == 2 ? 1 : 0);
        out[b] = cut_map(s, 3, stride[b], 1, Hp >> lo, Wp >> lo);
        t1[b] = cut_window(out[b], stride[b], Hp >> l, Wp >> l);
        s = out[b]; l = lo;
    }
}
static inline CutRect cut_hull(const CutRect& a, const CutRect& b) {
    return {a.x0 < b.x0 ? a.x0 : b.x0, a.y0 < b.y0 ? a.y0 : b.y0, a.x1 > b.x1 ? a.x1 : b.x1, a.y1 > b.y1 ? a.y1 : b.y1};
}
static inline void cut_fpn_geometry(int Hp, int Wp, const CutSet* c, CutSet* inner, CutSet* outp) {
    inner[3] = c[3];
    for (int i = 2; i >= 0; i--) {
        const int Hl = Hp >> (2 + i), Wl = Wp >> (2 + i);
        const CutSet& up = inner[i + 1];
        CutSet s; s.n = 0;
        if (up.n == c[i].n) {
            for (int q = 0; q < up.n; q++) {
                CutRect u = {2 * up.r[q].x0, 2 * up.r[q].y0, 2 * up.r[q].x1 + 1, 2 * up.r[q].y1 + 1};
                if (u.x1 > Wl - 1) u.x1 = Wl - 1; if (u.y1 > Hl - 1) u.y1 = Hl - 1;
                s.r[s.n++] = cut_hull(u, c[i].r[q]);
            }
        } else if (up.n || c[i].n) {
            s.n = 1; s.r[0] = {0, 0, Wl - 1, Hl - 1};
        }
        inner[i] = s;
    }
    for (int i = 0; i < 4; i++) outp[i] = cut_map(inner[i], 3, 1, 1, Hp >> (2 + i), Wp >> (2 + i));
}
static inline int cut_disjoint(const CutSet& s, CutRect* o, int cap) {
    int ys[2 * CUT_SET_MAX], ny = 0;
    for (int i = 0; i < s.n; i++) { ys[ny++] = s.r[i].y0; ys[ny++] = s.r[i].y1 + 1; }
    for (int i = 1; i < ny; i++) for (int j = i; j > 0 && ys[j] < ys[j - 1]; j--) { const int t = ys[j]; ys[j] = ys[j - 1]; ys[j - 1] = t; }
    int n = 0;
    for (int k = 0; k + 1 < ny; k++) {
        const int ya = ys[k], yb = ys[k + 1] - 1;
        if (ya > yb) continue;
        int x0[CUT_SET_MAX], x1[CUT_SET_MAX], nx = 0;
        for (int i = 0; i < s.n; i++)
            if (s.r[i].y0 <= ya && s.r[i].y1 >= yb) { x0[nx] = s.r[i].x0; x1[nx] = s.r[i].x1; nx++; }
        for (int i = 1; i < nx; i++) for (int j = i; j > 0 && x0[j] < x0[j - 1]; j--) {
            int t = x0[j]; x0[j] = x0[j - 1]; x0[j - 1] = t; t = x1[j]; x1[j] = x1[j - 1]; x1[j - 1] = t;
        }
        for (int i = 0; i < nx;) {
            const int a = x0[i];
            int b = x1[i++];
            while (i < nx && x0[i] <= b + 1) { if (x1[i] > b) b = x1[i]; i++; }
            bool ext = false;
            for (int q = 0; q < n && !ext; q++)
                if (o[q].x0 == a && o[q].x1 == b && o[q].y1 == ya - 1) { o[q].y1 = yb; ext = true; }
            if (ext) continue;
            if (n == cap) return -1;
            o[n++] = {a, ya, b, yb};
        }
    }
    return n;
}
```

### cald_amd/csrc/kernels.h

```cpp
#pragma once
#include "common.h"

struct ViewDesc {
    const uint8_t* src;
    int H, W;
    int flip;
    int nrect;
    int rects[4 * CALD_MAX_CUT];
    int Hr, Wr;
    int Ho, Wo;
    const float* noise;
    int swap;
};

struct DetBuffers {
    float* boxes;
    float* scores;
    long long* labels;
    float* props;
    float* prob_max;
    float* scores_cls;
    int* count;
    int cap;
    int C;
// ... 97 lines not shown
    int pred_ld, C, V;
    const float* proposals;
    const int* prop_count;
    const ViewDesc* views;
    float score_thr, nms_thr, conf_thr;
    int cap;
    float* prob;
    unsigned* vmax;
    int* kept_prop;
    float* kept_box;
    int* cls_count;
    int* row_off;
    int* al;
    int* count;
    int* total;
    float* boxes;
    float* scores;
    signed char* labels;
};
void launch_ssm_postprocess(const SsmArgs& a, hipStream_t st);

struct ScoreArgs {
    DetBuffers det;
    const int* ref_view;
    const int* aug_view;
    const int* aug_kind;
    const float* aug_param;
    const int* ref_sel;
    const int* ref_n;
    const int* pair_img;
    int P;
    float bp;
    float* cons;
};
void launch_consistency(const ScoreArgs& a, hipStream_t st);
void launch_cls_corr(const DetBuffers& det, const int* ref_sel, const int* ref_n, const int* view_img, const int* view_is_ref,
                     int V, float* out , hipStream_t st);

struct RpnPruneArgs {
    const LevelSeg* seg[2];
    float* energy[2];
    float* pnorm[2];
    const float* head[2];
    float* head_out[2];
    const float* head_rows[2][2];
    int* row_map[2][2];
    int* nsel[2];
    unsigned* tau_key;
    unsigned long long* stat;
    unsigned long long* log[2];
    float* check;
    float c1[3], c0[3];
    int head_ld, pre_n, V;
};
void launch_rpn_prune_select(const RpnPruneArgs& a, int max_pix, int stage, hipStream_t st);
void launch_rpn_prune_scatter(const RpnPruneArgs& a, int max_pix, hipStream_t st);

#define CALD_VM 16
enum { VM_RPN_TOPK = 0, VM_RPN_IOU, VM_RPN_ORDER, VM_RPN_TRUNC, VM_RPN_SMALL, VM_ROI_LEVEL, VM_ROI_EDGE, VM_POST_THR, VM_POST_IOU,
       VM_POST_ORDER, VM_POST_CAP, VM_POST_SUBORDER, VM_POST_TOP2 };
struct AuditArgs {
    const unsigned long long* cand_key; const float* cand_box; const float* sorted_box; const unsigned char* flags;
    const unsigned long long* next_key; const unsigned long long* trunc_key;
    int pre_n, post_n; float rpn_nms_thr, min_size;
    const float* proposals; const int* prop_count; const LevelSeg* seg[4];
    const float* prob; const float* pred; int pred_ld, C; const ViewDesc* views;
    const unsigned long long* keys; const int* key_count; int key_cap;
    const unsigned long long* kept_key; const float* post_maxc; const int* det_count; int cap;
    float score_thr, post_nms_thr;
    int V;
    float delta;
    float* out;
};
void launch_audit(const AuditArgs& a, hipStream_t st);
void launch_pair_audit(const ScoreArgs& a, float* out, hipStream_t st);

struct RetinaArgs {
    const float* cls[5];
    const float* reg[5];
    const LevelSeg* seg[5];
    const LevelSeg* seg0;
    const ViewDesc* views;
    const float* base_anchors;
    int cls_ld, reg_ld, A, K, V;
    float score_thr, nms_thr, min_box;
    int per_class;
    int cand_cap;
    int* cand_count;
    unsigned long long* cand_key;
    float* cand_box;
    unsigned char* cand_skip;
    int* kept_anchor;
    float* kept_box;
    int* kept_count;
    DetBuffers det;
};
void launch_retina_postprocess(const RetinaArgs& a, int max_anchors, hipStream_t st);
__device__ inline int retina_level_of(const RetinaArgs& a, int v, int i, int* local) {
    int l = 0;
    int base = 0;
#pragma unroll
    for (int t = 0; t < 5; t++) {
        const int n = a.seg[t][v].H * a.seg[t][v].W * a.A;
        if (i >= base + n && t < 4) { base += n; l = t + 1; }
        else break;
    }
// ... 54 lines not shown
```

### cald_amd/csrc/model.hip

```cpp
#include "host.h"

extern "C" int cald_model_create(cald_ctx* ctx, const cald_model_cfg* cfg, cald_model** out) {
    if (!ctx || !cfg || !out) return fail(CALD_ERR_INVALID, "null argument");
    if (cfg->arch != CALD_ARCH_FRCNN && cfg->arch != CALD_ARCH_RETINANET) return fail(CALD_ERR_INVALID, "unknown arch %d", cfg->arch);
    if (cfg->depth != 50 && cfg->depth != 101) return fail(CALD_ERR_INVALID, "depth must be 50 or 101");
    if (cfg->num_classes < 2 || cfg->num_classes > 256) return fail(CALD_ERR_INVALID, "num_classes out of range");
    if (cfg->rpn_pre_nms_top_n > 1024 || cfg->rpn_post_nms_top_n > CALD_ROI_CAP || cfg->rpn_pre_nms_top_n < 1 || cfg->rpn_post_nms_top_n < 1)
        return fail(CALD_ERR_INVALID, "rpn top-n out of range (pre <= 1024, post <= %d)", CALD_ROI_CAP);
    if (cfg->detections_per_img < 1 || cfg->detections_per_img > 1024) return fail(CALD_ERR_INVALID, "detections_per_img out of range");
    if (cfg->precision != CALD_PRECISION_FP32 && cfg->precision != CALD_PRECISION_F16X3) return fail(CALD_ERR_INVALID, "unknown precision %d", cfg->precision);
    cald_model* m = new cald_model();
    m->ctx = ctx; m->cfg = *cfg;
    {
        const float thr = cfg->box_score_thresh;
        long long per = cfg->num_classes - 1;
        if (thr > 0.0f && std::isfinite(thr)) { const long long lim = (long long)std::ceil(1.0 / (double)thr) - 1; if (lim < per) per = lim < 1 ? 1 : lim; }
        long long need = (long long)CALD_ROI_CAP * per;
        int kc = 1024; while (kc < need) kc <<= 1;
        m->key_cap = kc;
    }
    memset(&m->sweep_det, 0, sizeof(m->sweep_det)); memset(&m->sweep_det2, 0, sizeof(m->sweep_det2));
    *out = m;
    return 0;
}
// ... 262 lines not shown
        if (m->cls_out.Cout != 9 * m->cfg.num_classes || m->reg_out.Cout != 36)
            return fail(CALD_ERR_INVALID, "RetinaNet heads must have 9*num_classes / 36 outputs (got %d / %d)", m->cls_out.Cout, m->reg_out.Cout);
        std::vector<float> base(5 * 9 * 4);
        const float ratios[3] = {0.5f, 1.0f, 2.0f};
        for (int l = 0; l < 5; l++) {
            const int x = 32 << l;
            const float sizes[3] = {(float)x, (float)(int)((double)x * pow(2.0, 1.0 / 3)), (float)(int)((double)x * pow(2.0, 2.0 / 3))};
            for (int r = 0; r < 3; r++) {
                float hr = sqrtf(ratios[r]), wr = 1.0f / hr;
                for (int sidx = 0; sidx < 3; sidx++) {
                    float ws = wr * sizes[sidx], hs = hr * sizes[sidx];
                    float* b = &base[((l * 9) + r * 3 + sidx) * 4];
                    b[0] = rintf(-ws / 2.0f); b[1] = rintf(-hs / 2.0f); b[2] = rintf(ws / 2.0f); b[3] = rintf(hs / 2.0f);
                }
            }
        }
        if ((rc = upload(m, base, &m->d_anchors))) return rc;
    }
    m->sd.clear();
    m->finalized = true;
    return 0;
}
extern "C" int cald_model_set_rpn_prune(cald_model* m, int on, int* was) {
    if (!m) return fail(CALD_ERR_INVALID, "model is null");
    if (!m->finalized) return fail(CALD_ERR_STATE, "model not finalized");
    if (was) *was = m->prune ? 1 : 0;
    m->prune = on != 0 && m->prune_allowed;
    return 0;
}
extern "C" int cald_model_set_cutout_reuse(cald_model* m, int mode, int* was) {
    if (!m || mode < -1 || mode > 2) return fail(CALD_ERR_INVALID, "bad argument");
    if (was) *was = m->cr.mode;
    m->cr.mode = mode;
    return 0;
}
extern "C" int cald_model_set_cutout_retention_cap(cald_model* m, int64_t bytes, int64_t* was) {
    if (!m || bytes < 0) return fail(CALD_ERR_INVALID, "bad argument");
    if (was) *was = (int64_t)m->cr.ext_cap;
    m->cr.ext_cap = (size_t)bytes;
    return 0;
}
extern "C" int cald_model_set_row_packing(cald_model* m, int mode, int* was) {
    if (!m || mode < -1 || mode > 1) return fail(CALD_ERR_INVALID, "bad argument");
    if (was) *was = m->row_packing;
    m->row_packing = mode;
    return 0;
}
extern "C" int cald_model_set_look_fuse(cald_model* m, int mode, int* was) {
    if (!m || mode < 0 || mode > 2) return fail(CALD_ERR_INVALID, "bad argument");
    if (was) *was = m->look_fuse;
    m->look_fuse = mode;
    return 0;
}
extern "C" int cald_model_set_box_min_size(cald_model* m, float min_size, float* was) {
    if (!m || !(min_size >= 0.0f)) return fail(CALD_ERR_INVALID, "bad argument");
    if (m->cfg.arch != CALD_ARCH_FRCNN) return fail(CALD_ERR_INVALID, "box_min_size belongs to the Faster R-CNN tail (RetinaNet's always removes small boxes)");
    if (was) *was = m->box_min_size;
    m->box_min_size = min_size;
    return 0;
}
extern "C" int cald_model_set_rpn_prune_capture(cald_model* m, int on) {
    if (!m) return fail(CALD_ERR_INVALID, "model is null");
    if (on && !(m->prune && m->prune_allowed)) return fail(CALD_ERR_STATE, "certified RPN pruning is not active on this model");
    m->prune_capture = on != 0;
    return 0;
}
extern "C" int cald_model_rpn_prune_bound(cald_model* m, float* c1, float* c0) {
    if (!m || !c1 || !c0) return fail(CALD_ERR_INVALID, "null argument");
    if (!m->rpn_conv16.w16) return fail(CALD_ERR_STATE, "the model has no look-ahead layer (not an exact Faster R-CNN model)");
    for (int a = 0; a < 3; a++) { c1[a] = m->prune_c1[a]; c0[a] = m->prune_c0[a]; }
    return 0;
}
extern "C" int cald_model_set_rpn_prune_bound(cald_model* m, const float* c1, const float* c0) {
    if (!m || !c1 || !c0) return fail(CALD_ERR_INVALID, "null argument");
    if (!m->rpn_conv16.w16) return fail(CALD_ERR_STATE, "the model has no look-ahead layer (not an exact Faster R-CNN model)");
    for (int a = 0; a < 3; a++) { m->prune_c1[a] = c1[a]; m->prune_c0[a] = c0[a]; }
    m->prune_bound_voided = true;
    return 0;
}
extern "C" int cald_model_destroy(cald_model* m) {
    if (!m) return 0;
    hipSetDevice(m->ctx->device);
    hipStreamSynchronize(m->ctx->stream);
    for (void* p : m->owned) hipFree(p);
    if (m->sweep_det_views) free_det(m->sweep_det);
    if (m->sweep_det2_views) free_det(m->sweep_det2);
    if (m->ss.dev) hipFree(m->ss.dev);
    if (m->ss.pin) hipHostFree(m->ss.pin);
    if (m->ss.d_aug) hipFree(m->ss.d_aug);
    for (int i = 0; i < 2; i++) { if (m->cr.slot[i]) hipFree(m->cr.slot[i]); if (m->cr.h_gp[i]) hipHostFree(m->cr.h_gp[i]); }
    if (m->cr.d_gp) hipFree(m->cr.d_gp);
    for (int i = 0; i < 2; i++) { if (m->ss.ev_ref[i]) hipEventDestroy(m->ss.ev_ref[i]); if (m->ss.ev_score[i]) hipEventDestroy(m->ss.ev_score[i]); }
    delete m;
    return 0;
}
```

### cald_amd/csrc/ops.hip

```cpp
#include "host.h"

extern "C" int cald_op_transform_size(int H, int W, int min_size, int max_size, int* Hr, int* Wr, int* Hp, int* Wp) {
    if (H <= 0 || W <= 0 || min_size <= 0 || max_size <= 0) return fail(CALD_ERR_INVALID, "bad sizes");
    transform_size(H, W, min_size, max_size, Hr, Wr, Hp, Wp);
    return 0;
}

extern "C" int cald_op_cutout_rects(uint64_t seed, int H, int W, int N, const float* boxes, int cut_num, int* rects_out, int* n_out) {
    if (cut_num < 0 || cut_num > CALD_MAX_CUT) return fail(CALD_ERR_INVALID, "cut_num must be 0..%d", CALD_MAX_CUT);
    *n_out = cutout_rects(seed, H, W, N, boxes, cut_num, rects_out);
    return 0;
}

extern "C" int cald_op_cutout_geometry(int H, int W, int min_size, int max_size, int nrect, const int* rects, int nblk, const int* strides, int* out) {
    if (H < 1 || W < 1 || nrect < 0 || nrect > CALD_MAX_CUT || (nrect && !rects) || nblk < 0 || nblk > 64 || (nblk && !strides) || !out)
        return fail(CALD_ERR_INVALID, "bad argument");
    int Hr, Wr, Hp, Wp;
    transform_size(H, W, min_size, max_size, &Hr, &Wr, &Hp, &Wp);
    std::vector<CutSet> o(nblk + 1), t(nblk + 1);
    cut_geometry(H, W, Hr, Wr, Hp, Wp, nrect, rects, nblk, strides, &o[0], o.data() + 1, t.data() + 1);
    t[0].n = 0;
    for (int e = 0; e <= nblk; e++)
        for (int k = 0; k < 2; k++) {
            const CutSet& sset = k ? t[e] : o[e];
            int* q = out + (size_t)(2 * e + k) * (1 + 4 * CUT_SET_MAX);
            memset(q, 0, sizeof(int) * (1 + 4 * CUT_SET_MAX));
            q[0] = sset.n;
            for (int i = 0; i < sset.n; i++) { q[1 + 4 * i] = sset.r[i].x0; q[2 + 4 * i] = sset.r[i].y0; q[3 + 4 * i] = sset.r[i].x1; q[4 + 4 * i] = sset.r[i].y1; }
        }
    return 0;
}
extern "C" int cald_op_cutout_fpn_geometry(int H, int W, int min_size, int max_size, int nrect, const int* rects, int nblk, const int* strides, int* out) {
    if (H < 1 || W < 1 || nrect < 0 || nrect > CALD_MAX_CUT || (nrect && !rects) || nblk < 4 || nblk > 64 || !strides || !out)
        return fail(CALD_ERR_INVALID, "bad argument");
    int ends[4], ne = 0;
    for (int b = 0; b < nblk; b++)
        if (b == nblk - 1 || strides[b + 1] == 2) { if (ne == 4) return fail(CALD_ERR_INVALID, "more than four stages"); ends[ne++] = b; }
    if (ne != 4) return fail(CALD_ERR_INVALID, "the strides describe %d stages, not four", ne);
    int Hr, Wr, Hp, Wp;
    transform_size(H, W, min_size, max_size, &Hr, &Wr, &Hp, &Wp);
    std::vector<CutSet> o(nblk), t(nblk);
    CutSet pool1, cs[4], sets[8];
    cut_geometry(H, W, Hr, Wr, Hp, Wp, nrect, rects, nblk, strides, &pool1, o.data(), t.data());
    for (int i = 0; i < 4; i++) cs[i] = o[ends[i]];
    cut_fpn_geometry(Hp, Wp, cs, sets, sets + 4);
    for (int e = 0; e < 8; e++) {
        int* q = out + (size_t)e * (1 + 4 * CUT_SET_MAX);
        memset(q, 0, sizeof(int) * (1 + 4 * CUT_SET_MAX));
        q[0] = sets[e].n;
        for (int i = 0; i < sets[e].n; i++) { q[1 + 4 * i] = sets[e].r[i].x0; q[2 + 4 * i] = sets[e].r[i].y0; q[3 + 4 * i] = sets[e].r[i].x1; q[4 + 4 * i] = sets[e].r[i].y1; }
    }
    return 0;
}
static int get_pil(cald_ctx* c, int inSize, int outSize, int fid, PilCoef* out) {
    PilKey key{inSize, outSize, fid};
    auto it = c->pil.find(key);
    if (it == c->pil.end()) {
        std::vector<int> b, k;
        PilCoef pc; pc.ksize = pil_coeffs(inSize, outSize, fid, b, k);
        ScopedDev sd(c->stream); int rc;
        if ((rc = sd.upload(&pc.d_bounds, b.data(), b.size() * sizeof(int))) || (rc = sd.upload(&pc.d_kk, k.data(), k.size() * sizeof(int)))) return rc;
        sd.release();
        it = c->pil.insert(std::make_pair(key, pc)).first;
    }
    *out = it->second;
    return 0;
}
int cald_host::pil_resize(cald_ctx* c, const uint8_t* src, int H, int W, uint8_t* dst, int oh, int ow, uint8_t* tmp, int fid) {
    const uint8_t* cur = src;
    if (ow != W) {
        PilCoef pc; int rc = get_pil(c, W, ow, fid, &pc); if (rc) return rc;
        uint8_t* hdst = (oh != H) ? tmp : dst;
        launch_pil_horizontal(src, H, W, hdst, ow, pc.d_bounds, pc.d_kk, pc.ksize, c->stream);
        cur = hdst;
    }
    if (oh != H) {
        PilCoef pc; int rc = get_pil(c, H, oh, fid, &pc); if (rc) return rc;
        launch_pil_vertical(cur, H, ow, dst, oh, pc.d_bounds, pc.d_kk, pc.ksize, c->stream);
    } else if (ow == W) {
        HIPCHK(hipMemcpyAsync(dst, src, (size_t)H * W * 3, hipMemcpyDeviceToDevice, c->stream));
    }
    return 0;
}
extern "C" int cald_op_pil_resize(cald_ctx* c, const uint8_t* src_dev, int H, int W, uint8_t* dst_dev, int oh, int ow) {
    if (!c || !src_dev || !dst_dev || H <= 0 || W <= 0 || oh <= 0 || ow <= 0) return fail(CALD_ERR_INVALID, "bad arguments");
    ScopedDev sd(c->stream);
    uint8_t* tmp; int rc;
    if ((rc = sd.alloc(&tmp, (size_t)H * ow * 3))) return rc;
    return pil_resize(c, src_dev, H, W, dst_dev, oh, ow, tmp);
}

extern "C" int cald_op_noise_stream(cald_ctx* c, uint64_t seed, const uint8_t* src_dev, int H, int W, int nseg, const int* kinds,
                                    const double* params, void* const* dsts) {
    if (!c || !src_dev || H <= 0 || W <= 0 || !kinds || !params || !dsts) return fail(CALD_ERR_INVALID, "cald_op_noise_stream: bad arguments");
    if (nseg < 1 || nseg > CALD_MAX_NOISE_SEG) return fail(CALD_ERR_INVALID, "cald_op_noise_stream: 1..%d segments", CALD_MAX_NOISE_SEG);
    NoiseJob nj; memset(&nj, 0, sizeof(nj));
    nj.seed = seed; nj.src = src_dev; nj.H = H; nj.W = W; nj.nseg = nseg;
    for (int g = 0; g < nseg; g++) {
        NoiseSeg& sg = nj.seg[g];
        if (!dsts[g]) return fail(CALD_ERR_INVALID, "cald_op_noise_stream: segment %d has no destination", g);
        sg.dst = dsts[g];
        if (kinds[g] == CALD_AUG_GAUSS) {
            if (randn_unsupported(H, W))
// ... 489 lines not shown

extern "C" int cald_op_retina_postprocess(cald_ctx* c, const float* const* cls, const float* const* reg, const int* level_hw, int A, int K,
                                          const float* base_anchors, int Hp, int Wp, int Hr, int Wr, int Ho, int Wo,
                                          float score_thr, float nms_thr, int per_class,
                                          float* boxes_out, float* scores_out, int64_t* labels_out, float* prob_max_out,
                                          float* scores_cls_out, int* n_out) {
    if (!c || !cls || !reg || !level_hw || !base_anchors || !boxes_out || !scores_out || !labels_out || !prob_max_out || !scores_cls_out || !n_out)
        return fail(CALD_ERR_INVALID, "null argument");
    RetinaHookIn in; int rc;
    if ((rc = in.check(cls, reg, level_hw, A, K, Hp, Wp, Hr, Wr, Ho, Wo, per_class))) return rc;
    HIPCHK(hipSetDevice(c->device));
    ScopedDev sd(c->stream); ScopedDet det;
    RetinaTailBufs S;
    if ((rc = carve(sd, [&](Bump& B) { in.layout(B, A, K); S.layout(B, 1, K, per_class, (int)in.anchors); })) || (rc = det.alloc(1, K * per_class, K)) ||
        (rc = in.upload(cls, reg, base_anchors, A, K))) return rc;
    launch_retina_postprocess(retina_args(S, in.d_cls, in.d_reg, in.d_p, in.d_vd, in.d_base, A, K, 1, score_thr, nms_thr, per_class, det.d), S.max_anchors, c->stream);
    HIPCHK(hipGetLastError());
    return download_dets(c, det.d, "retina", boxes_out, scores_out, labels_out, nullptr, prob_max_out, scores_cls_out, n_out);
}

extern "C" int cald_op_retina_ssm_postprocess(cald_ctx* c, const float* const* cls, const float* const* reg, const int* level_hw, int A, int K,
                                              const float* base_anchors, int Hp, int Wp, int Hr, int Wr, int Ho, int Wo,
                                              float score_thr, float nms_thr, int per_class, cald_ssm_pick_fn pick, void* user,
                                              int* al_out, int* n_out, int* counts_out, float* boxes_out, float* scores_out, int8_t* labels_out) {
    if (!c || !cls || !reg || !level_hw || !base_anchors || !pick || !al_out || !n_out || !counts_out || !boxes_out || !scores_out || !labels_out)
        return fail(CALD_ERR_INVALID, "null argument");
    if (K < 2) return fail(CALD_ERR_INVALID, "the RetinaNet SSM tail needs K >= 2 (labels have K - 1 columns)");
    RetinaHookIn in; int rc;
    if ((rc = in.check(cls, reg, level_hw, A, K, Hp, Wp, Hr, Wr, Ho, Wo, per_class))) return rc;
    HIPCHK(hipSetDevice(c->device));
    ScopedDev sd(c->stream);
    RetinaSsmBufs S;
    if ((rc = carve(sd, [&](Bump& B) { in.layout(B, A, K); S.layout(B, 1, K, per_class, (int)in.anchors); })) || (rc = in.upload(cls, reg, base_anchors, A, K))) return rc;
    const RetinaSsmArgs sa = retina_ssm_args(S, in.d_cls, in.d_reg, in.d_p, in.d_vd, in.d_base, A, K, 1, score_thr, nms_thr, per_class);
    launch_retina_ssm_phase_a(sa, c->stream);
    HIPCHK(hipGetLastError());
    if ((rc = retina_ssm_pick_stop(c, S, 1, K, pick, user, 0, counts_out))) return rc;
    launch_retina_ssm_phase_b(sa, c->stream);
    HIPCHK(hipGetLastError());
    HIPCHK(hipStreamSynchronize(c->stream));
    int al = 0, n = 0, total = 0;
    HIPCHK(hipMemcpy(&al, S.al, 4, hipMemcpyDeviceToHost)); HIPCHK(hipMemcpy(&n, S.count, 4, hipMemcpyDeviceToHost)); HIPCHK(hipMemcpy(&total, S.total, 4, hipMemcpyDeviceToHost));
    if (n < 0 || n > K * per_class || total != n || (al && n)) return fail(CALD_ERR_HIP, "retina ssm postprocess returned %d rows (al %d, total %d, cap %d)", n, al, total, K * per_class);
    if (n) {
        HIPCHK(hipMemcpy(boxes_out, S.boxes, (size_t)n * 16, hipMemcpyDeviceToHost));
        HIPCHK(hipMemcpy(scores_out, S.scores, (size_t)n * 4, hipMemcpyDeviceToHost));
        HIPCHK(hipMemcpy(labels_out, S.labels, (size_t)n * (K - 1), hipMemcpyDeviceToHost));
    }
    if (al) memset(counts_out, 0, (size_t)K * 4);
    *al_out = al; *n_out = n;
    return 0;
}

extern "C" int cald_op_rpn_prune(cald_ctx* c, cald_rpn_prune_probe* p) {
    if (!c || !p) return fail(CALD_ERR_INVALID, "cald_op_rpn_prune: null argument");
    if (p->V < 1 || p->V > CALD_PRUNE_PROBE_MAX_VIEWS || p->guard < 0 || p->guard > 4096 || p->head_ld < 3 || p->head_ld > 64 || p->pre_n < 1)
        return fail(CALD_ERR_INVALID, "cald_op_rpn_prune: 1..%d views, guard 0..4096, head_ld 3..64, pre_n >= 1", CALD_PRUNE_PROBE_MAX_VIEWS);
    const int V = p->V, ld = p->head_ld; const size_t G = (size_t)p->guard;
    constexpr int SV = CALD_PRUNE_PROBE_MAX_VIEWS + 1;
    LevelSeg seg[2 * SV]; memset(seg, 0, sizeof(seg));
    size_t pix[2]; int max_pix = 0;
    for (int l = 0; l < 2; l++) {
        for (int v = 0; v < V; v++) {
            const int H = p->hw[l][v][0], W = p->hw[l][v][1];
            if (H < 1 || W < 1 || (long long)H * W > (1 << 19)) return fail(CALD_ERR_INVALID, "cald_op_rpn_prune: level %d view %d: 1 <= H * W <= 2^19", l, v);
            seg[l * SV + v].H = H; seg[l * SV + v].W = W; seg[l * SV + v + 1].pix_off = seg[l * SV + v].pix_off + (long long)H * W;
            if (H * W > max_pix) max_pix = H * W;
        }
        pix[l] = (size_t)seg[l * SV + V].pix_off;
        if (!p->energy[l] || !p->exact[l] || !p->head[l] || !p->pnorm[l]) return fail(CALD_ERR_INVALID, "cald_op_rpn_prune: level %d: null array", l);
    }
    for (int s = 0; s < 2; s++) if (!p->nsel[s] || !p->row_map[s][0] || !p->row_map[s][1] || !p->tau_key) return fail(CALD_ERR_INVALID, "cald_op_rpn_prune: null output array");
    HIPCHK(hipSetDevice(c->device));
    ScopedDev sd(c->stream);
    RpnPruneArgs pr; memset(&pr, 0, sizeof(pr));
    const LevelSeg* d_seg; float* d_rows[2][2]; int rc;
    const size_t nw = (size_t)2 * V + G;
    if ((rc = sd.upload(&d_seg, seg, sizeof(seg))) || (rc = sd.upload(&pr.tau_key, p->tau_key, nw * 4)) || (rc = sd.upload(&pr.check, p->check, 8)) ||
        (rc = sd.alloc(&pr.stat, 32))) return rc;
    HIPCHK(hipMemset(pr.stat, 0, 32));
    for (int l = 0; l < 2; l++) {
        pr.seg[l] = d_seg + l * SV;
        if ((rc = sd.upload(&pr.energy[l], p->energy[l], pix[l] * 16)) || (rc = sd.upload(&pr.pnorm[l], p->pnorm[l], (pix[l] + G) * 4)) ||
            (rc = sd.upload(&pr.head_out[l], p->head[l], (pix[l] + G) * ld * 4))) return rc;
        pr.head[l] = pr.head_out[l];
        for (int s = 0; s < 2; s++) {
            if ((rc = sd.upload(&pr.row_map[s][l], p->row_map[s][l], (pix[l] + G) * 4)) || (rc = sd.alloc(&d_rows[s][l], pix[l] * ld * 4))) return rc;
            pr.head_rows[s][l] = d_rows[s][l];
        }
    }
    for (int s = 0; s < 2; s++) if ((rc = sd.upload(&pr.nsel[s], p->nsel[s], nw * 4))) return rc;
    for (int q = 0; q < 3; q++) { pr.c1[q] = p->c1[q]; pr.c0[q] = p->c0[q]; }
    pr.head_ld = ld; pr.pre_n = p->pre_n; pr.V = V;
    auto maps_back = [&](int s) {
        HIPCHK(hipMemcpy(p->nsel[s], pr.nsel[s], nw * 4, hipMemcpyDeviceToHost));
        for (int l = 0; l < 2; l++) HIPCHK(hipMemcpy(p->row_map[s][l], pr.row_map[s][l], (pix[l] + G) * 4, hipMemcpyDeviceToHost));
        return 0;
    };
    for (int s = 0; s < 2; s++) {
        launch_rpn_prune_select(pr, max_pix, s, c->stream);
        HIPCHK(hipGetLastError()); HIPCHK(hipStreamSynchronize(c->stream));
        if ((rc = maps_back(s))) return rc;
        if (s == 0) HIPCHK(hipMemcpy(p->tau_key, pr.tau_key, nw * 4, hipMemcpyDeviceToHost));
        for (int l = 0; l < 2; l++) {
            std::vector<float> rows(pix[l] * ld, NAN);
            for (int v = 0; v < V; v++) {
                const LevelSeg& sg = seg[l * SV + v];
                const int npx = sg.H * sg.W, ns = p->nsel[s][l * V + v];
                if (ns < 0 || ns > npx) return fail(CALD_ERR_HIP, "cald_op_rpn_prune: stage %d level %d view %d selected %d of %d pixels", s, l, v, ns, npx);
                for (int r = 0; r < ns; r++) {
                    const int px = p->row_map[s][l][sg.pix_off + r];
                    if (px < 0 || px >= npx) return fail(CALD_ERR_HIP, "cald_op_rpn_prune: stage %d level %d view %d row %d maps to pixel %d of %d", s, l, v, r, px, npx);
                    memcpy(&rows[(size_t)(sg.pix_off + r) * ld], p->exact[l] + (size_t)(sg.pix_off + px) * ld, (size_t)ld * 4);
                }
            }
            HIPCHK(hipMemcpy(d_rows[s][l], rows.data(), rows.size() * 4, hipMemcpyHostToDevice));
        }
    }
    launch_rpn_prune_scatter(pr, max_pix, c->stream);
    HIPCHK(hipGetLastError()); HIPCHK(hipStreamSynchronize(c->stream));
    for (int s = 0; s < 2; s++) if ((rc = maps_back(s))) return rc;
    for (int l = 0; l < 2; l++) {
        HIPCHK(hipMemcpy(p->head[l], pr.head_out[l], (pix[l] + G) * ld * 4, hipMemcpyDeviceToHost));
        HIPCHK(hipMemcpy(p->pnorm[l], pr.pnorm[l], (pix[l] + G) * 4, hipMemcpyDeviceToHost));
    }
    HIPCHK(hipMemcpy(p->check, pr.check, 8, hipMemcpyDeviceToHost));
    HIPCHK(hipMemcpy(p->stat, pr.stat, 32, hipMemcpyDeviceToHost));
    return 0;
}

extern "C" int cald_op_roi_align(cald_ctx* c, const float* const* feats, const int* level_hw, int C, int R, const float* rois, float* out) {
    if (!c || !feats || !level_hw || !rois || !out) return fail(CALD_ERR_INVALID, "null argument");
    if (R < 1 || R > CALD_ROI_CAP || C < 4 || C % 4) return fail(CALD_ERR_INVALID, "bad geometry (1 <= R <= %d, C a positive multiple of 4)", CALD_ROI_CAP);
    HIPCHK(hipSetDevice(c->device));
    BatchPlan P; memset(&P, 0, sizeof(P));
    size_t pix[4];
    for (int l = 0; l < 4; l++) {
        const int H = level_hw[2 * l], W = level_hw[2 * l + 1];
        if (H < 1 || W < 1 || !feats[l]) return fail(CALD_ERR_INVALID, "level %d is malformed", l);
        P.seg[2 + l][0].H = H; P.seg[2 + l][0].W = W; P.seg[2 + l][1].pix_off = (long long)H * W; pix[l] = (size_t)H * W;
    }
    ScopedDev sd(c->stream);
    ProposalBufs pb; RoiBufs S; float* d_f[4]; BatchPlan* d_p; int rc;
    if ((rc = carve(sd, [&](Bump& B) { for (int l = 0; l < 4; l++) d_f[l] = B.get<float>(pix[l] * C); d_p = B.get<BatchPlan>(1); pb.layout(B, 1); S.layout(B, 1, C); })) ||
        (rc = put_proposals(pb, rois, R))) return rc;
    for (int l = 0; l < 4; l++) HIPCHK(hipMemcpy(d_f[l], feats[l], pix[l] * C * 4, hipMemcpyHostToDevice));
    HIPCHK(hipMemcpy(d_p, &P, sizeof(P), hipMemcpyHostToDevice));
    launch_roi_align(roi_args(S, d_f, d_p, C, 1, pb, false), c->stream);
    HIPCHK(hipGetLastError()); HIPCHK(hipStreamSynchronize(c->stream));
    HIPCHK(hipMemcpy(out, S.roi, (size_t)R * 49 * C * 4, hipMemcpyDeviceToHost));
    return 0;
}

extern "C" int cald_op_cls_corr(cald_ctx* c, int n, const float* scores, const int64_t* labels, int C, float* out) {
    if (!c || !out || n < 0 || C < 2 || C > 256) return fail(CALD_ERR_INVALID, "bad arguments");
    HIPCHK(hipSetDevice(c->device));
    ScopedDev sd(c->stream); ScopedDet sdet;
    int rc = sdet.alloc(1, n > 0 ? n : 1, C); if (rc) return rc;
    const DetBuffers& d = sdet.d;
    if (n) { HIPCHK(hipMemcpy(d.scores, scores, (size_t)n * 4, hipMemcpyHostToDevice)); HIPCHK(hipMemcpy(d.labels, labels, (size_t)n * 8, hipMemcpyHostToDevice)); }
    HIPCHK(hipMemcpy(d.count, &n, 4, hipMemcpyHostToDevice));
    int h[2] = {0, 0}; int* dh; float* dout;
    if ((rc = sd.upload(&dh, h, 8)) || (rc = sd.alloc(&dout, (size_t)(C - 1) * 4))) return rc;
    launch_cls_corr(d, nullptr, nullptr, dh, dh + 1, 1, dout, c->stream);
    HIPCHK(hipGetLastError());
    HIPCHK(hipStreamSynchronize(c->stream));
    HIPCHK(hipMemcpy(out, dout, (size_t)(C - 1) * 4, hipMemcpyDeviceToHost));
    return 0;
}

extern "C" int cald_op_score_batch(cald_ctx* c, cald_score_probe* q) {
    if (!c || !q) return fail(CALD_ERR_INVALID, "null argument");
    const int V = q->V, cap = q->cap, C = q->C, B = q->n_img, P = q->P;
    if (!q->boxes || !q->props || !q->scores || !q->labels || !q->scores_cls || !q->prob_max || !q->count || !q->view_img || !q->view_isref ||
        !q->ref_sel || !q->ref_n || !q->ref_view || !q->aug_view || !q->pair_img || !q->aug_kind || !q->aug_param ||
        !q->cons || !q->cls_corr || !q->pair_audit || !q->max_iou || !q->lt) return fail(CALD_ERR_INVALID, "null argument");
    if (C < 2 || C > 256) return fail(CALD_ERR_INVALID, "C %d outside 2..256", C);
    if (V < 1 || V > CALD_MAX_VIEWS || cap < 1 || B < 1 || P < 0) return fail(CALD_ERR_INVALID, "bad geometry (1 <= V <= %d, cap >= 1, n_img >= 1, P >= 0)", CALD_MAX_VIEWS);
    for (int v = 0; v < V; v++) {
        if (q->count[v] < 0 || q->count[v] > cap) return fail(CALD_ERR_INVALID, "view %d: count %d outside 0..%d", v, q->count[v], cap);
        if (q->view_img[v] < 0 || q->view_img[v] >= B) return fail(CALD_ERR_INVALID, "view %d: image %d out of range", v, q->view_img[v]);
// ... 69 lines not shown
```

### cald_amd/csrc/rpn_prune.hip

```cpp
#include "common.h"
#include "kernels.h"
#include <cfloat>

namespace {
__device__ __forceinline__ float prune_patch_norm(const float* e, int y, int x, int H, int W) {
    float s = 0.0f;
#pragma unroll
    for (int dy = -1; dy <= 1; dy++)
#pragma unroll
        for (int dx = -1; dx <= 1; dx++) {
            const int yy = y + dy, xx = x + dx;
            if (yy >= 0 && yy < H && xx >= 0 && xx < W) {
                const float* q = e + (yy * W + xx) * 4;
                s = s + ((q[0] + q[1]) + (q[2] + q[3]));
            }
        }
    return sqrtf(s) * 1.0001f;
}
template <int MODE>
__global__ __launch_bounds__(1024) void prune_select_kernel(RpnPruneArgs a) {
    extern __shared__ unsigned mask[];
    __shared__ int hist[256];
    __shared__ unsigned s_prefix, s_mask;
    __shared__ int s_remaining, s_total, s_wave_cnt[16];
    const int l = blockIdx.x, v = blockIdx.y, tid = threadIdx.x;
    const LevelSeg sg = a.seg[l][v];
    const int H = sg.H, W = sg.W, npx = H * W, A = 3, n = npx * A;
    const int k = n < a.pre_n ? n : a.pre_n;
    const int ld = a.head_ld;
    const float* head = a.head[l] + sg.pix_off * (long long)ld;
    const float* en = a.energy[l] + sg.pix_off * 4;
    float* pnv = a.pnorm[l] + sg.pix_off;
    constexpr int ST = MODE == 2 ? 1 : 0;
    int* rmap = a.row_map[ST][l] + sg.pix_off;
    const int words = (npx + 31) >> 5;
    for (int i = tid; i < words; i += 1024) mask[i] = 0u;
    if (tid == 0) { s_prefix = 0u; s_mask = 0u; s_remaining = k; }
    __syncthreads();
    auto bound = [&](int an, float pn) { return a.c1[an] * pn + a.c0[an]; };
    if (MODE != 2) {
        for (int p = tid; p < npx; p += 1024) {
            const float pn = prune_patch_norm(en, p / W, p % W, H, W);
            pnv[p] = pn;
            if (!(pn < 4094.0f) && a.check) atomicMax(reinterpret_cast<unsigned*>(a.check) + 1, __float_as_uint(1.0f));
        }
    }
    const int ns0 = MODE == 2 ? a.nsel[0][l * a.V + v] : 0;
    const float* rows0 = MODE == 2 ? a.head_rows[0][l] + sg.pix_off * (long long)ld : nullptr;
    const bool all_kept = n <= k;
    if (!all_kept) {
        for (int pass = 0; pass < 4; pass++) {
            const int shift = 24 - 8 * pass;
            if (tid < 256) hist[tid] = 0;
            __syncthreads();
            const unsigned prefix = s_prefix, msk = s_mask;
            if (MODE == 2) {
                for (int i = tid; i < ns0 * A; i += 1024) {
                    const unsigned key = det_orderable(rows0[(long long)(i / A) * ld + (i % A)]);
                    if ((key & msk) == prefix) atomicAdd(&hist[(key >> shift) & 255u], 1);
                }
            } else {
                for (int p = tid; p < npx; p += 1024) {
                    const float pn = pnv[p];
                    for (int an = 0; an < A; an++) {
                        const unsigned key = det_orderable(head[(long long)p * ld + an] - bound(an, pn));
                        if ((key & msk) == prefix) atomicAdd(&hist[(key >> shift) & 255u], 1);
                    }
                }
            }
            __syncthreads();
            if (tid == 0) {
                int cum = 0, rem = s_remaining;
                for (int b = 255; b >= 0; b--) {
                    const int h = hist[b];
                    if (cum + h >= rem) { s_remaining = rem - cum; s_prefix = prefix | ((unsigned)b << shift); s_mask = msk | (255u << shift); break; }
                    cum += h;
                }
            }
            __syncthreads();
        }
    }
    unsigned tau = all_kept ? 0u : s_prefix;
    unsigned tau_lb = tau;
    if (MODE == 1 && tid == 0) a.tau_key[l * a.V + v] = tau;
    if (MODE == 2) {
        tau_lb = a.tau_key[l * a.V + v];
        tau = (ns0 * A >= k && tau > tau_lb) ? tau : tau_lb;
    }
    for (int p = tid; p < npx; p += 1024) {
        const float pn = pnv[p];
        bool keep = false, first = false;
        for (int an = 0; an < A; an++) {
            const float lg = head[(long long)p * ld + an];
            const float B = bound(an, pn);
            const float ub = lg + B, lb = lg - B;
            if (MODE == 1) keep = keep || !(lb == lb) || det_orderable(lb) >= tau;
            if (MODE == 2) { first = first || !(lb == lb) || det_orderable(lb) >= tau_lb; keep = keep || !(ub == ub) || det_orderable(ub) >= tau; }
        }
        if (MODE == 2) {
            if (first) keep = false;
            else if (!keep) { float* hw = a.head_out[l] + (sg.pix_off + p) * (long long)ld; hw[0] = -FLT_MAX; hw[1] = -FLT_MAX; hw[2] = -FLT_MAX; }
        }
        if (keep) atomicOr(&mask[p >> 5], 1u << (p & 31));
    }
    __syncthreads();
    const int lane = tid & 63, wave = tid >> 6;
    int base = 0;
    for (int w0 = 0; w0 < words; w0 += 1024) {
        const int wi = w0 + tid;
        const unsigned bits = wi < words ? mask[wi] : 0u;
        const int cnt = __popc(bits);
        int inc = cnt;
#pragma unroll
        for (int off = 1; off < 64; off <<= 1) { const int t = __shfl_up(inc, off, 64); if (lane >= off) inc += t; }
        if (lane == 63) s_wave_cnt[wave] = inc;
        __syncthreads();
        int wbase = 0;
        for (int q = 0; q < wave; q++) wbase += s_wave_cnt[q];
        int o = base + wbase + inc - cnt;
        unsigned b = bits;
        while (b) { const int t = __ffs(b) - 1; b &= b - 1; rmap[o++] = wi * 32 + t; }
        if (tid == 1023) s_total = wbase + inc;
        __syncthreads();
        base += s_total;
        __syncthreads();
    }
    if (tid == 0) {
        a.nsel[ST][l * a.V + v] = base;
        if (a.stat) { atomicAdd(a.stat + 2 * l, (unsigned long long)base); if (MODE != 2) atomicAdd(a.stat + 2 * l + 1, (unsigned long long)npx); }
        if (a.log[ST]) { atomicAdd(a.log[ST] + 2 * l, (unsigned long long)base); atomicAdd(a.log[ST] + 2 * l + 1, (unsigned long long)npx); }
    }
}

__global__ __launch_bounds__(256) void prune_scatter_kernel(RpnPruneArgs a) {
    __shared__ float s_worst[4];
    const int l = blockIdx.z & 1, st = blockIdx.z >> 1, v = blockIdx.y;
    const LevelSeg sg = a.seg[l][v];
    const int ns = a.nsel[st][l * a.V + v], ld = a.head_ld;
    const int* rmap = a.row_map[st][l] + sg.pix_off;
    const float* src = a.head_rows[st][l] + sg.pix_off * (long long)ld;
    const float* pnv = a.pnorm[l] + sg.pix_off;
    float* dst = a.head_out[l] + sg.pix_off * (long long)ld;
    float worst = 0.0f;
    for (int i = blockIdx.x * 256 + threadIdx.x; i < ns * ld; i += gridDim.x * 256) {
        const int r = i / ld, c = i - r * ld;
        const int p = rmap[r];
        const float exact = src[i];
        if (c < 3) {
            const float approx = dst[(long long)p * ld + c];
            const float B = a.c1[c] * pnv[p] + a.c0[c];
            const float ratio = fabsf(approx - exact) / B;
            worst = (ratio == ratio) ? fmaxf(worst, ratio) : INFINITY;
        }
        dst[(long long)p * ld + c] = exact;
    }
#pragma unroll
    for (int off = 32; off >= 1; off >>= 1) worst = fmaxf(worst, __shfl_xor(worst, off, 64));
    if ((threadIdx.x & 63) == 0) s_worst[threadIdx.x >> 6] = worst;
    __syncthreads();
    if (threadIdx.x == 0 && a.check) {
        worst = fmaxf(fmaxf(s_worst[0], s_worst[1]), fmaxf(s_worst[2], s_worst[3]));
        unsigned* const ck = reinterpret_cast<unsigned*>(a.check);
        const unsigned wb = __float_as_uint(worst);
        if (worst > 0.0f && *reinterpret_cast<volatile unsigned*>(ck) < wb) atomicMax(ck, wb);
    }
}
}

void launch_rpn_prune_select(const RpnPruneArgs& a, int max_pix, int stage, hipStream_t st) {
    const size_t lds = (size_t)((max_pix + 31) / 32) * 4;
    static PerDeviceOnce once1, once2;
    if (stage == 0) { allow_big_lds(once1, prune_select_kernel<1>); hipLaunchKernelGGL(prune_select_kernel<1>, dim3(2, a.V), dim3(1024), lds, st, a); }
    else { allow_big_lds(once2, prune_select_kernel<2>); hipLaunchKernelGGL(prune_select_kernel<2>, dim3(2, a.V), dim3(1024), lds, st, a); }
}
void launch_rpn_prune_scatter(const RpnPruneArgs& a, int max_pix, hipStream_t st) {
    const long long want = ((long long)max_pix * a.head_ld + 1023) / 1024;
    const unsigned bx = (unsigned)(want < 1 ? 1 : want > 64 ? 64 : want);
    hipLaunchKernelGGL(prune_scatter_kernel, dim3(bx, a.V, 4), dim3(256), 0, st, a);
}
```

### cald_amd/csrc/sweep.hip

```cpp
#include "host.h"

void cald_host::free_det(DetBuffers& d) {
    hipFree(d.boxes); hipFree(d.scores); hipFree(d.labels); hipFree(d.props); hipFree(d.prob_max); hipFree(d.scores_cls); hipFree(d.count);
    memset(&d, 0, sizeof(d));
}
int cald_host::alloc_det(DetBuffers& d, int V, int cap, int C) {
    memset(&d, 0, sizeof(d));
    d.cap = cap; d.C = C;
    hipError_t e = hipMalloc((void**)&d.boxes, (size_t)V * cap * 16);
    if (e == hipSuccess) e = hipMalloc((void**)&d.scores, (size_t)V * cap * 4);
    if (e == hipSuccess) e = hipMalloc((void**)&d.labels, (size_t)V * cap * 8);
    if (e == hipSuccess) e = hipMalloc((void**)&d.props, (size_t)V * cap * 16);
    if (e == hipSuccess) e = hipMalloc((void**)&d.prob_max, (size_t)V * cap * 4);
    if (e == hipSuccess) e = hipMalloc((void**)&d.scores_cls, (size_t)V * cap * C * 4);
    if (e == hipSuccess) e = hipMalloc((void**)&d.count, (size_t)V * 4);
    if (e != hipSuccess) {
        free_det(d);
        return fail(CALD_ERR_HIP, "hipMalloc of detection buffers (%d views x %d rows x %d classes) failed: %s", V, cap, C, hipGetErrorString(e));
    }
    return 0;
}
static int ensure_det(cald_model* m, DetBuffers& set, int& views, int VT) {
    if (views >= VT) return 0;
    if (views) {
        HIPCHK(hipStreamSynchronize(m->ctx->stream));
        free_det(set);
        views = 0;
    }
    int rc = alloc_det(set, VT, m->det_cap(), m->cfg.num_classes);
    if (rc) return rc;
    views = VT;
    return 0;
}
static DetBuffers det_at(const DetBuffers& D, size_t o) {
    DetBuffers d2 = D;
    const int cap = D.cap, C = D.C;
    d2.boxes += o * cap * 4; d2.scores += o * cap; d2.labels += o * cap; d2.props += o * cap * 4;
    d2.prob_max += o * cap; d2.scores_cls += o * cap * C; d2.count += o;
    return d2;
}
static ViewDesc plain_view(const uint8_t* src, int H, int W) {
    ViewDesc d; memset(&d, 0, sizeof(d));
    d.src = src; d.H = H; d.W = W;
    return d;
}
static std::vector<ViewDesc> ref_views(const uint8_t* const* images_dev, const int* H, const int* W, int i0, int nb) {
    std::vector<ViewDesc> views(nb);
    for (int i = 0; i < nb; i++) views[i] = plain_view(images_dev[i0 + i], H[i0 + i], W[i0 + i]);
    return views;
}

static int sweep_fwd_views() {
    static const int env = getenv("CALD_FWD_VIEWS") ? atoi(getenv("CALD_FWD_VIEWS")) : 96;
    return env < 1 ? 1 : (env > CALD_MAX_VIEWS ? CALD_MAX_VIEWS : env);
}
static int fwd_count(int n) { return (n + sweep_fwd_views() - 1) / sweep_fwd_views(); }
static void fwd_span(int n, int f, int* a0, int* nv) {
    const int n_fw = fwd_count(n);
    *a0 = (int)(((long long)n * f) / n_fw); *nv = (int)(((long long)n * (f + 1)) / n_fw) - *a0;
}
static bool cut_reuse_env() {
    static const bool on = !(getenv("CALD_CUTOUT_REUSE") && atoi(getenv("CALD_CUTOUT_REUSE")) == 0);
    return on;
}
#define CUT_GATHER_MAX_COST 0.7
#define CUT_FPN_MAX_COST CUT_GATHER_MAX_COST

namespace {
struct SweepBatch {
    int i0 = 0, nb = 0, P = 0, VV = 0; bool live = false;
    int* h_count; float* h_boxes; int* h_ints; float* h_par; NoiseJob* h_jobs; float* h_cons; float* h_clsc; float* h_vm; float* h_pm;
    std::vector<int> ref_n, pair_img, view_img, pair_aug, view_aug;
    std::vector<char> view_inert;
    std::vector<float> cut_margin;
    bool kept = false;
    bool kept_fpn = false;
    std::vector<int> ref_sel, pair_kind, view_isref;
    std::vector<float> pair_par;
    std::vector<ViewDesc> aviews;
};

struct SweepRun {
    cald_model* m; int n_images; const uint8_t* const* images_dev; const int* H; const int* W; const int64_t* pool_pos;
    const cald_sweep_cfg* cfg; double* consistency_out; double* cls_corr_out; float* margins_out; bool force_dense;
    cald_ctx* c = nullptr;
    bool audit = false, prune_ok = false, retina = false, reuse = false;
    int C = 0, cap = 0, A = 0, B = 0, VT = 0, NB = 0, P_MAX = 0, cut_a = -1;
    PairLayout lay{0, 0, 0}; size_t n_ints = 0;
    DetBuffers* DS[2] = {nullptr, nullptr};
    int* d_ints = nullptr; float *d_par = nullptr, *d_cons = nullptr, *d_clsc = nullptr; NoiseJob* d_jobs = nullptr; unsigned long long* d_lsum = nullptr;
    float *d_vm[2] = {nullptr, nullptr}, *d_pm = nullptr;
    SweepBatch bt[2];
    int nblk = 0, blk_lin[CUT_MAX_BLOCKS], blk_lout[CUT_MAX_BLOCKS], blk_stage[CUT_MAX_BLOCKS], blk_stride[CUT_MAX_BLOCKS];
    int ngeo = 0, geo_stride[CUT_MAX_BLOCKS], c_blk[4] = {0, 0, 0, 0};
    bool fpn_ok = false;
    std::vector<BatchPlan> rplan;

    static size_t al(size_t b) { return (b + 255) & ~(size_t)255; }

    int setup() {
        if (!m || !images_dev || !H || !W || !pool_pos || !cfg || !consistency_out || !cls_corr_out) return fail(CALD_ERR_INVALID, "null argument");
        audit = margins_out != nullptr;
        prune_ok = !audit && !force_dense;
        if (!m->finalized) return fail(CALD_ERR_STATE, "model not finalized");
        c = m->ctx;
        HIPCHK(hipSetDevice(c->device));
        C = m->cfg.num_classes; cap = m->det_cap();
        A = cfg->n_augs;
        if (A < 0 || A > CALD_MAX_AUGS) return fail(CALD_ERR_INVALID, "n_augs %d outside [0, %d]", A, CALD_MAX_AUGS);
        int n_noise = 0; bool any_gauss = false;
        for (int a = 0; a < A; a++) {
            const int k = cfg->augs[a].kind;
            if (k < CALD_AUG_FLIP || k > CALD_AUG_ROTATE) return fail(CALD_ERR_INVALID, "augmentation %d: unknown kind %d", a, k);
            if (k == CALD_AUG_CUTOUT && (cfg->augs[a].param < 1.0 || cfg->augs[a].param > (double)CALD_MAX_CUT))
                return fail(CALD_ERR_INVALID, "cutout: cut_num must be in [1, %d]", CALD_MAX_CUT);
// ... 40 lines not shown
            bt[q].h_count = b.get<int>(VT); bt[q].h_boxes = b.get<float>((size_t)B * cap * 4); bt[q].h_ints = b.get<int>(n_ints);
            bt[q].h_par = b.get<float>((size_t)P_MAX * 12); bt[q].h_jobs = b.get<NoiseJob>(B); bt[q].h_cons = b.get<float>(P_MAX);
            bt[q].h_clsc = b.get<float>((size_t)VT * (C - 1));
            bt[q].h_vm = b.get<float>((size_t)VT * CALD_VM); bt[q].h_pm = b.get<float>((size_t)P_MAX * 2);
        }
        if (m->prune && prune_ok) HIPCHK(hipMemsetAsync(c->d_prune_check, 0, 8, c->stream));
        for (int a = 0; a < A && cut_a < 0; a++) if (cfg->augs[a].kind == CALD_AUG_CUTOUT) cut_a = a;
        init_blocks();
        reuse = (m->cr.mode < 0 ? cut_reuse_env() : m->cr.mode != 0) && cut_a >= 0 && !audit && m->cfg.precision == CALD_PRECISION_FP32 && nblk < CUT_MAX_BLOCKS;
        rplan.resize(reuse ? 1 : 0);
        return 0;
    }
    void init_blocks() {
        retina = m->cfg.arch == CALD_ARCH_RETINANET;
        for (int b = 0, layer = 0, l = 2; b < (int)m->blocks.size() && layer < 3 && nblk < CUT_MAX_BLOCKS; b++) {
            const Bottleneck& Bk = m->blocks[b];
            blk_stride[nblk] = Bk.c2.stride; blk_lin[nblk] = l; l += Bk.c2.stride == 2 ? 1 : 0; blk_lout[nblk] = l; blk_stage[nblk] = layer;
            nblk++;
            if (Bk.layer_end) layer++;
        }
        {
            int layer = 0; bool fits = true;
            for (size_t b = 0; b < m->blocks.size(); b++) {
                if (ngeo == CUT_MAX_BLOCKS || layer > 3) { fits = false; break; }
                geo_stride[ngeo] = m->blocks[b].c2.stride;
                if (m->blocks[b].layer_end) c_blk[layer++] = ngeo;
                ngeo++;
            }
            fpn_ok = fits && layer == 4 && !retina && ngeo >= nblk;
            if (!fpn_ok) { ngeo = nblk; for (int b = 0; b < nblk; b++) geo_stride[b] = blk_stride[b]; }
        }
    }

    void plan_of(int nv, const ViewDesc* vs, BatchPlan& P) const {
        int hp[CALD_MAX_VIEWS][2];
        for (int v = 0; v < nv; v++) { int Hr, Wr; transform_size(vs[v].H, vs[v].W, m->cfg.min_size, m->cfg.max_size, &Hr, &Wr, &hp[v][0], &hp[v][1]); }
        build_plan(P, nv, vs, hp, retina);
    }
    size_t retain_layout(const BatchPlan& P, int nv, char* base, float** out) const {
        size_t off = 0;
        for (int b = 0; b < nblk; b++) {
            if (out) out[b] = reinterpret_cast<float*>(base + off);
            off += al((size_t)level_pix(P, blk_lout[b], nv) * (size_t)m->blocks[b].c3.Cout * 4);
        }
        return off;
    }
    size_t retain_layout_fpn(const BatchPlan& P, int nv, char* base, FwdReuse* ru) const {
        size_t off = retain_layout(P, nv, base, ru ? ru->out : nullptr);
        auto take = [&](size_t bytes) { char* p = base + off; off += al(bytes); return p; };
        for (int i = 0; i < 4; i++) { char* p = take((size_t)level_pix(P, 2 + i, nv) * 256 * 4); if (ru) ru->pf[i] = reinterpret_cast<float*>(p); }
        if (m->prune && prune_ok)
            for (int i = 0; i < 2; i++) {
                char* p = take((size_t)level_pix(P, 2 + i, nv) * 256 * 4); char* e = take((size_t)level_pix(P, 2 + i, nv) * 4 * 4);
                if (ru) { ru->p16[i] = reinterpret_cast<unsigned*>(p); ru->energy[i] = reinterpret_cast<float*>(e); }
            }
        if (ru) ru->fpn = true;
        return off;
    }

    int enqueue_ref(int k) {
        SweepBatch& b = bt[k & 1];
        b.i0 = k * B; b.nb = (n_images - b.i0 < B) ? n_images - b.i0 : B; b.live = true; b.P = 0; b.VV = b.nb;
        std::vector<ViewDesc> views = ref_views(images_dev, H, W, b.i0, b.nb);
        const DetBuffers& D = *DS[k & 1];
        FwdReuse ru;
        if (int r = retain(k, views.data(), ru)) return r;
        int r = forward_model(m, b.nb, views.data(), D, audit ? d_vm[k & 1] : nullptr, prune_ok, b.kept ? &ru : nullptr);
        if (r) return r;
        if (hipMemcpyAsync(b.h_count, D.count, (size_t)b.nb * 4, hipMemcpyDeviceToHost, c->stream) != hipSuccess ||
            hipMemcpyAsync(b.h_boxes, D.boxes, (size_t)b.nb * cap * 16, hipMemcpyDeviceToHost, c->stream) != hipSuccess ||
            hipEventRecord(m->ss.ev_ref[k & 1], c->stream) != hipSuccess) return fail(CALD_ERR_HIP, "D2H of reference detections failed");
        return 0;
    }
    int retain(int k, const ViewDesc* views, FwdReuse& ru) {
        SweepBatch& b = bt[k & 1];
        b.kept = b.kept_fpn = false;
        if (reuse) {
            plan_of(b.nb, views, rplan[0]);
            cald_model::CutReuse& R = m->cr;
            const int q = k & 1;
            const size_t need3 = retain_layout(rplan[0], b.nb, nullptr, nullptr), needx = fpn_ok ? retain_layout_fpn(rplan[0], b.nb, nullptr, nullptr) : 0;
            bool ext = fpn_ok && !R.ext_refused && !(R.ext_cap && needx > R.ext_cap);
            for (int attempt = 0; attempt < 2; attempt++) {
                const size_t need = ext ? needx : need3;
                if (need <= R.cap[q]) break;
                HIPCHK(hipStreamSynchronize(c->stream));
                if (R.slot[q]) hipFree(R.slot[q]);
                R.slot[q] = nullptr; R.cap[q] = 0;
                if (hipMalloc((void**)&R.slot[q], need + (need >> 3)) == hipSuccess) { R.cap[q] = need + (need >> 3); break; }
                (void)hipGetLastError(); R.slot[q] = nullptr;
                if (!ext) break;
                ext = false; R.ext_refused = true;
            }
            if (R.slot[q]) {
                ru.mode = 1; ru.nblk = nblk; b.kept = true; b.kept_fpn = ext;
                if (ext) retain_layout_fpn(rplan[0], b.nb, R.slot[q], &ru); else retain_layout(rplan[0], b.nb, R.slot[q], ru.out);
            } else c->cut_fallbacks++;
            c->cut_kept[!b.kept ? CUT_KEPT_NONE : b.kept_fpn ? CUT_KEPT_FPN : CUT_KEPT_STAGES]++;
        }
        return 0;
    }

    int build_aug_views(int k) {
        SweepBatch& b = bt[k & 1];
        cald_model::SweepScratch& S = m->ss;
        const int nb = b.nb, i0 = b.i0;
        if (hipEventSynchronize(S.ev_ref[k & 1]) != hipSuccess) return fail(CALD_ERR_HIP, "reference forward failed: %s", hipGetErrorString(hipGetLastError()));
// ... 54 lines not shown
            for (int a = 0; a < A && !r; a++) {
                const int kd = cfg->augs[a].kind; const double prm = cfg->augs[a].param;
                float par[12] = {0};
                cur_a = a;
                if (kd == CALD_AUG_FLIP) { ViewDesc v = base; v.flip = 1; pair_params(1, Hi, Wi, prm, par); add_view(v, 1, par); }
                else if (kd == CALD_AUG_GAUSS) {
                    NoiseSeg& sg = nj.seg[nj.nseg++]; sg.kind = 0; sg.p0 = (float)prm; sg.p1 = 0.0f;
                    sg.dst = take((size_t)Hi * Wi * 3 * sizeof(float));
                    ViewDesc v = base; v.noise = reinterpret_cast<const float*>(sg.dst); add_view(v, 0, nullptr);
                } else if (kd == CALD_AUG_SALT_PEPPER) {
                    NoiseSeg& sg = nj.seg[nj.nseg++]; sg.kind = 1; sg.p0 = (float)(prm / 2.0); sg.p1 = (float)(1.0 - prm / 2.0);
                    sg.dst = take((size_t)Hi * Wi * 3);
                    ViewDesc v = base; v.src = reinterpret_cast<const uint8_t*>(sg.dst); add_view(v, 0, nullptr);
                } else if (kd == CALD_AUG_COLOR_ADJUST) {
                    uint8_t* tmp = take((size_t)Hi * Wi * 3); uint8_t* dst = take((size_t)Hi * Wi * 3);
                    launch_color_adjust(images_dev[i0 + i], Hi, Wi, (float)prm, tmp, d_lsum + b.pair_img.size(), dst, c->stream);
                    ViewDesc v = base; v.src = dst; add_view(v, 0, nullptr);
                } else if (kd == CALD_AUG_COLOR_SWAP) {
                    ViewDesc v = base; v.swap = pyrng.randbelow(6); add_view(v, 0, nullptr);
                } else if (kd == CALD_AUG_CUTOUT) {
                    ViewDesc v = base;
                    float cm = INFINITY;
                    v.nrect = cutout_rects(pyrng, Hi, Wi, b.ref_n[i], sub, (int)prm, v.rects, &cm);
                    if (cm < b.cut_margin[i]) b.cut_margin[i] = cm;
                    add_view(v, 0, nullptr);
                } else if (kd == CALD_AUG_RESIZE) {
                    const int ow = (int)((double)Wi * prm), oh = (int)((double)Hi * prm);
                    uint8_t* dst = take((size_t)oh * ow * 3); uint8_t* tmp = take((size_t)Hi * ow * 3);
                    if ((r = pil_resize(c, images_dev[i0 + i], Hi, Wi, dst, oh, ow, tmp, 0))) break;
                    pair_params(2, Hi, Wi, prm, par); add_view(plain_view(dst, oh, ow), 2, par);
                } else if (kd == CALD_AUG_ROTATE) {
                    int fx[6], nh, nw; pil_rotate_setup(Hi, Wi, prm, fx, &nh, &nw);
                    uint8_t* rot = take((size_t)nh * nw * 3); uint8_t* tmp = take((size_t)nh * Wi * 3); uint8_t* dst = take((size_t)Hi * Wi * 3);
                    launch_affine_nearest(images_dev[i0 + i], Hi, Wi, rot, nh, nw, fx, c->stream);
                    if ((r = pil_resize(c, rot, nh, nw, dst, Hi, Wi, tmp, 1))) break;
                    ViewDesc v = base; v.src = dst;
                    pair_params(3, Hi, Wi, prm, par);
                    add_view(v, 3, par);
                }
            }
            if (r) return r;
            if (nj.nseg) b.h_jobs[njobs++] = nj;
        }
        if (njobs) {
            if (hipMemcpyAsync(d_jobs, b.h_jobs, sizeof(NoiseJob) * njobs, hipMemcpyHostToDevice, c->stream) != hipSuccess) return fail(CALD_ERR_HIP, "H2D of noise jobs failed");
            launch_noise_stream(d_jobs, njobs, c->stream);
        }
        return 0;
    }

    int cut_plan(int k, int V, const ViewDesc* vs, FwdReuse& ru) {
        cald_model::CutReuse& R = m->cr;
        const bool fpn = bt[k & 1].kept_fpn;
        const size_t per = cut_plan_set_bytes(V), total = per * (2 * (size_t)nblk + (fpn ? 4 : 0));
        if (!R.d_gp) {
            const size_t cap = cut_plan_set_bytes(CALD_MAX_VIEWS) * (2 * CUT_MAX_BLOCKS + 4);
            HIPCHK(hipMalloc((void**)&R.d_gp, cap));
            HIPCHK(hipHostMalloc((void**)&R.h_gp[0], cap)); HIPCHK(hipHostMalloc((void**)&R.h_gp[1], cap));
        }
        plan_of(V, vs, rplan[0]);
        const BatchPlan& P = rplan[0];
        char* const h = R.h_gp[k & 1];
        std::vector<CutSet> g_out((size_t)V * ngeo), g_t1((size_t)V * ngeo), g_fpn((size_t)V * 4);
        for (int v = 0; v < V; v++) {
            int Hr, Wr, Hp, Wp; CutSet pool1;
            transform_size(vs[v].H, vs[v].W, m->cfg.min_size, m->cfg.max_size, &Hr, &Wr, &Hp, &Wp);
            cut_geometry(vs[v].H, vs[v].W, Hr, Wr, Hp, Wp, vs[v].nrect, vs[v].rects, ngeo, geo_stride, &pool1, &g_out[(size_t)v * ngeo], &g_t1[(size_t)v * ngeo]);
            if (fpn) {
                CutSet cs[4], inner[4];
                for (int i = 0; i < 4; i++) cs[i] = g_out[(size_t)v * ngeo + c_blk[i]];
                cut_fpn_geometry(Hp, Wp, cs, inner, &g_fpn[(size_t)v * 4]);
            }
        }
        auto put_set = [&](size_t index, int lvl, const CutSet* sets, size_t stride_v, int* tiles_out, double* rows_out) {
            LevelSeg* sg = reinterpret_cast<LevelSeg*>(h + index * per);
            GatherSet* gs = reinterpret_cast<GatherSet*>(reinterpret_cast<char*>(sg) + (size_t)(V + 1) * sizeof(LevelSeg));
            int tiles = 0; double rows = 0.0;
            for (int v = 0; v < V; v++) {
                LevelSeg L = P.seg[lvl][v]; L.tile_start = tiles; sg[v] = L;
                CutRect rr[CALD_GATHER_RECTS];
                int n = cut_disjoint(sets[(size_t)v * stride_v], rr, CALD_GATHER_RECTS);
                if (n < 0) { n = 1; rr[0] = {0, 0, L.W - 1, L.H - 1}; }
                GatherSet& G = gs[v]; memset(&G, 0, sizeof(G));
                G.nr = n;
                for (int q = 0; q < n; q++) {
                    G.x0[q] = rr[q].x0; G.y0[q] = rr[q].y0; G.w[q] = rr[q].x1 - rr[q].x0 + 1;
                    G.cum[q + 1] = G.cum[q] + G.w[q] * (rr[q].y1 - rr[q].y0 + 1);
                }
                tiles += (G.cum[n] + 127) / 128; rows += (double)G.cum[n];
            }
            sg[V] = P.seg[lvl][V]; sg[V].tile_start = tiles;
            *tiles_out = tiles; *rows_out = rows;
        };
        auto kf = [](const ConvLayer& L) { return (double)L.Cout * (double)(L.KH * L.KW * L.CinTrue); };
        double cost_g[3] = {0, 0, 0}, cost_d[3] = {0, 0, 0}, rows_g[3] = {0, 0, 0}, rows_d[3] = {0, 0, 0}, tiles_g[3] = {0, 0, 0}, tiles_d[3] = {0, 0, 0};
        for (int b = 0; b < nblk; b++)
            for (int kind = 0; kind < 2; kind++) {
                const int lvl = kind ? blk_lin[b] : blk_lout[b];
                int tiles; double rows;
                put_set((size_t)(2 * b + kind), lvl, (kind ? g_t1.data() : g_out.data()) + b, (size_t)ngeo, &tiles, &rows);
                ru.tiles[b][kind] = tiles; ru.rows[b][kind] = rows;
                const Bottleneck& Bk = m->blocks[b];
                const double w = kind ? kf(Bk.c1) : kf(Bk.c2) + kf(Bk.c3) + (Bk.has_down ? kf(Bk.down) : 0.0);
                const double nconv = kind ? 1.0 : (Bk.has_down ? 3.0 : 2.0), dense = (double)level_pix(P, lvl, V);
                const int st = blk_stage[b];
                cost_g[st] += 128.0 * tiles * w; cost_d[st] += dense * w;
                rows_g[st] += rows * nconv; rows_d[st] += dense * nconv;
                tiles_g[st] += tiles * nconv; tiles_d[st] += (double)P.seg[lvl][V].tile_start * nconv;
            }
        for (int st = 0; st < 3; st++) {
            ru.gather[st] = m->cr.mode != 2 && cost_g[st] <= CUT_GATHER_MAX_COST * cost_d[st];
            c->cut_rows[st] += ru.gather[st] ? rows_g[st] : rows_d[st]; c->cut_dense[st] += rows_d[st];
            c->cut_st_rows[st] += ru.gather[st] ? rows_g[st] : rows_d[st]; c->cut_st_dense[st] += rows_d[st];
            c->cut_st_tiles[st] += ru.gather[st] ? tiles_g[st] : tiles_d[st]; c->cut_st_dense_tiles[st] += tiles_d[st];
        }
        {
            double r4 = 0.0, t4 = 0.0, rl = 0.0, tl = 0.0;
            int lvl = 2;
            for (size_t b = 0; b < m->blocks.size(); b++) {
                const Bottleneck& Bk = m->blocks[b];
                const int lo = lvl + (Bk.c2.stride == 2 ? 1 : 0);
                if ((int)b >= nblk) {
                    const double n_in = 1.0, n_out = Bk.has_down ? 3.0 : 2.0;
                    r4 += n_in * (double)level_pix(P, lvl, V) + n_out * (double)level_pix(P, lo, V);
                    t4 += n_in * (double)P.seg[lvl][V].tile_start + n_out * (double)P.seg[lo][V].tile_start;
                }
                lvl = lo;
            }
            if (!retina) for (int i = 0; i < 4; i++) { rl += (double)level_pix(P, 2 + i, V); tl += (double)P.seg[2 + i][V].tile_start; }
            c->cut_st_rows[3] += r4; c->cut_st_dense[3] += r4; c->cut_st_tiles[3] += t4; c->cut_st_dense_tiles[3] += t4;
            c->cut_st_rows[CUT_STAGE_LATERAL] += rl; c->cut_st_dense[CUT_STAGE_LATERAL] += rl;
            c->cut_st_tiles[CUT_STAGE_LATERAL] += tl; c->cut_st_dense_tiles[CUT_STAGE_LATERAL] += tl;
            double fg = 0.0, fd = 0.0, frg = 0.0, frd = 0.0;
            if (fpn)
                for (int i = 0; i < 4; i++) {
                    put_set(2 * (size_t)nblk + i, 2 + i, g_fpn.data() + i, 4, &ru.fpn_tiles[i], &ru.fpn_rows[i]);
                    fg += ru.fpn_tiles[i]; frg += ru.fpn_rows[i];
                }
            if (!retina) for (int i = 0; i < 4; i++) { fd += (double)P.seg[2 + i][V].tile_start; frd += (double)level_pix(P, 2 + i, V); }
            ru.gather_fpn = fpn && m->cr.mode != 2 && 128.0 * fg <= CUT_FPN_MAX_COST * frd;
            c->cut_st_rows[CUT_STAGE_OUTPUT] += ru.gather_fpn ? frg : frd; c->cut_st_dense[CUT_STAGE_OUTPUT] += frd;
            c->cut_st_tiles[CUT_STAGE_OUTPUT] += ru.gather_fpn ? fg : fd; c->cut_st_dense_tiles[CUT_STAGE_OUTPUT] += fd;
        }
        if (hipMemcpyAsync(R.d_gp, h, total, hipMemcpyHostToDevice, c->stream) != hipSuccess) return fail(CALD_ERR_HIP, "H2D of the cut_out gather plan failed");
        ru.mode = 2; ru.nblk = nblk; ru.d_gp = R.d_gp;
        if (fpn) retain_layout_fpn(P, V, m->cr.slot[k & 1], &ru); else retain_layout(P, V, m->cr.slot[k & 1], ru.out);
        c->cut_batches++;
        return 0;
    }

    int enqueue_aug_forwards(int k) {
        SweepBatch& b = bt[k & 1];
        const DetBuffers& D = *DS[k & 1];
        const int nb = b.nb, na = (int)b.aviews.size();
        int r, n_rest = na, rest_slot = nb;
        ViewDesc* rest_views = b.aviews.data();
        std::vector<ViewDesc> rest;
        int n_cut = 0;
        for (int j = 0; j < na; j++) n_cut += b.view_aug[nb + j] == cut_a;
        b.VV = nb + na;
        if (b.kept && n_cut > 0 && 2 * nb + (na - n_cut) <= VT) {
            std::vector<ViewDesc> cutv(nb);
            std::vector<int> slot(na), nimg(VT, 0), naug(VT, 0);
            std::vector<char> has(nb, 0), ninert(VT, 0);
            for (int i = 0; i < nb; i++) nimg[i] = i;
            int nr2 = 0;
            for (int j = 0; j < na; j++) {
                const int img = b.view_img[nb + j];
                if (b.view_aug[nb + j] == cut_a) { slot[j] = nb + img; cutv[img] = b.aviews[j]; has[img] = 1; }
                else { slot[j] = 2 * nb + nr2++; rest.push_back(b.aviews[j]); }
                nimg[slot[j]] = img; naug[slot[j]] = b.view_aug[nb + j];
            }
            for (int i = 0; i < nb; i++)
                if (!has[i]) {
                    cutv[i] = plain_view(images_dev[b.i0 + i], H[b.i0 + i], W[b.i0 + i]);
                    nimg[nb + i] = i; naug[nb + i] = cut_a; ninert[nb + i] = 1;
                }
            for (size_t p = 0; p < b.pair_aug.size(); p++) b.pair_aug[p] = slot[b.pair_aug[p] - nb];
            b.view_img = nimg; b.view_aug = naug; b.view_inert = ninert;
            FwdReuse ru;
            if ((r = cut_plan(k, nb, cutv.data(), ru))) return r;
            if ((r = forward_model(m, nb, cutv.data(), det_at(D, (size_t)nb), nullptr, prune_ok, &ru))) return r;
            b.VV = 2 * nb + nr2; n_rest = nr2; rest_slot = 2 * nb; rest_views = rest.data();
        } else if (b.kept) {
            c->cut_fallbacks++;
        }
        for (int f = 0; f < fwd_count(n_rest); f++) {
            int a0, nv; fwd_span(n_rest, f, &a0, &nv);
            const size_t o = (size_t)(rest_slot + a0);
            if ((r = forward_model(m, nv, rest_views + a0, det_at(D, o), audit ? d_vm[k & 1] + o * CALD_VM : nullptr, prune_ok))) return r;
        }
        return 0;
    }

    int enqueue_scoring(int k) {
// ... 360 lines not shown
```

### cald_amd/detector.py

```python
import ctypes as C

import numpy as np
import torch

from . import _ffi

_CTX = {}


def get_ctx(device_index=None):
    if not torch.cuda.is_available():
        raise RuntimeError("cald_amd needs a visible MI355X (torch.cuda.is_available() is False); there is no CPU fallback")
    if device_index is None:
        device_index = torch.cuda.current_device()
    if device_index not in _CTX:
        h = C.c_void_p()
        stream = torch.cuda.current_stream(device_index).cuda_stream
        _ffi.check(_ffi.lib().cald_ctx_create(device_index, C.c_void_p(stream), C.byref(h)))
        _CTX[device_index] = h
    return _CTX[device_index]


_SIDE_CTX = {}

# ... 153 lines not shown
                assert noise.dtype == torch.float32 and noise.is_cuda and noise.is_contiguous() and tuple(noise.shape) == (3, img.shape[0], img.shape[1])
                arr[i].noise_dev = noise.data_ptr()
            arr[i].flip = int(bool(flip)); arr[i].nrect = 0 if rects is None else len(rects)
            if rects is not None:
                for j, r in enumerate(np.asarray(rects, np.int32).reshape(-1)):
                    arr[i].rects[j] = int(r)
        d = _ffi.Dets(out["boxes"].data_ptr(), out["scores"].data_ptr(), out["labels"].data_ptr(), out["props"].data_ptr(),
                      out["prob_max"].data_ptr(), out["scores_cls"].data_ptr(), out["count"].data_ptr(), cap)
        _ffi.check(L.cald_forward(h, n, arr, C.byref(d)) if _entry is None else _entry(L, h, n, arr, C.byref(d)))
        counts = out["count"].cpu().tolist()
        res = []
        for i, k in enumerate(counts):
            keys = ("boxes", "labels", "scores", "props", "prob_max", "scores_cls") if self.arch == 0 else \
                   ("boxes", "scores", "labels", "scores_cls", "prob_max")
            res.append({key: out[key][i, :k] for key in keys})
        return res

    def __call__(self, images, targets=None):
        if self.training:
            if targets is None:
                raise ValueError("In training mode, targets should be passed")
            return self._train_fn(images, targets)
        views = []
        for img in images:
            if img.dtype == torch.uint8:
                u8 = img if img.shape[-1] == 3 else img.permute(1, 2, 0)
                views.append((u8.contiguous().cuda(), False, None))
                continue
            x = img.detach().to(torch.float32).cuda().contiguous()
            if not bool(torch.isfinite(x).all()):
                raise ValueError("non-finite pixel values in the input image")
            g = (x * 255.0).round().clamp(0, 255).to(torch.uint8)
            base = _u8_over_255(x.device)[g.long()]
            rem = x - base
            if not bool(torch.equal(base + rem, x)):
                raise RuntimeError("float input is not representable as uint8 grid + float32 remainder")
            noise = rem.contiguous() if bool((rem != 0).any()) else None
            views.append((g.permute(1, 2, 0).contiguous(), False, None, noise))
        return self.forward_views(views)

    def debug_cutout_forward(self, views, prune=False):
        return self.forward_views(views, _entry=lambda L, h, n, arr, d: L.cald_debug_cutout_forward(h, n, arr, d, int(bool(prune))))

    def set_rpn_prune(self, on):
        was = C.c_int(0)
        _ffi.check(_ffi.lib().cald_model_set_rpn_prune(self.handle(), int(bool(on)), C.byref(was)))
        return bool(was.value)

    def set_look_fuse(self, mode):
        was = C.c_int(0)
        _ffi.check(_ffi.lib().cald_model_set_look_fuse(self.handle(), int(mode), C.byref(was)))
        return was.value

    def set_rpn_prune_capture(self, on):
        _ffi.check(_ffi.lib().cald_model_set_rpn_prune_capture(self.handle(), int(bool(on))))

    def rpn_prune_bound(self):
        import numpy as np
        c1 = np.zeros(3, np.float32); c0 = np.zeros(3, np.float32)
        _ffi.check(_ffi.lib().cald_model_rpn_prune_bound(self.handle(), _ffi.ptr(c1), _ffi.ptr(c0)))
        return c1, c0

    def set_rpn_prune_bound(self, c1, c0):
        import numpy as np
        c1 = np.ascontiguousarray(c1, np.float32); c0 = np.ascontiguousarray(c0, np.float32)
        assert c1.shape == (3,) and c0.shape == (3,)
        _ffi.check(_ffi.lib().cald_model_set_rpn_prune_bound(self.handle(), _ffi.ptr(c1), _ffi.ptr(c0)))

    def debug_tensor(self, name, view=0):
        shape = (C.c_int64 * 3)()
        cap = 1 << 26
        buf = np.empty(cap, np.float32)
        _ffi.check(_ffi.lib().cald_debug_tensor(self.handle(), name.encode(), view, _ffi.ptr(buf), cap, shape))
        n = shape[0] * shape[1] * shape[2]
        return buf[:n].reshape(shape[0], shape[1], shape[2]).copy()


def fasterrcnn_resnet50_fpn_feature(pretrained=False, progress=True, num_classes=91, pretrained_backbone=True, **kwargs):
    return HipDetector(num_classes, depth=50, **kwargs)


def fasterrcnn_resnet101_fpn_feature(pretrained=False, progress=True, num_classes=91, pretrained_backbone=True, **kwargs):
    return HipDetector(num_classes, depth=101, **kwargs)


def retinanet_resnet50_fpn_cal(pretrained=False, progress=True, num_classes=91, pretrained_backbone=True,
                               score_thresh=0.05, nms_thresh=0.5, detections_per_img=300, **kwargs):
    return HipDetector(num_classes, depth=50, box_score_thresh=score_thresh, box_nms_thresh=nms_thresh,
                       box_detections_per_img=detections_per_img, arch=1, **kwargs)


def from_torch_module(task_model):
    sd = task_model.state_dict()
    tr = getattr(task_model, "transform", None)
    min_size = getattr(tr, "min_size", 800)
    min_size = int(min_size[0] if isinstance(min_size, (tuple, list)) else min_size)
    max_size = int(getattr(tr, "max_size", 1333))
    depth = 101 if any(k.startswith("backbone.body.layer3.22.") for k in sd) else 50
    if any(k.startswith("head.classification_head.") for k in sd):
        ncls = int(sd["head.classification_head.cls_logits.weight"].shape[0]) // 9
        m = HipDetector(ncls, depth=depth, min_size=min_size, max_size=max_size, arch=1,
                        box_score_thresh=float(getattr(task_model, "score_thresh", 0.05)),
                        box_nms_thresh=float(getattr(task_model, "nms_thresh", 0.5)),
                        box_detections_per_img=int(getattr(task_model, "detections_per_img", 50 if hasattr(task_model, "ssm") else 300)))
    else:
        ncls = int(sd["roi_heads.box_predictor.cls_score.weight"].shape[0])
# ... 11 lines not shown
```

### include/cald_hip.h

```cpp
#ifndef CALD_HIP_H
#define CALD_HIP_H
#include <stddef.h>
#include <stdint.h>
#ifdef __cplusplus
extern "C" {
#endif

typedef struct cald_ctx cald_ctx;
typedef struct cald_model cald_model;

#define CALD_OK 0
#define CALD_ERR_INVALID (-1)
#define CALD_ERR_HIP (-2)
#define CALD_ERR_STATE (-3)
#define CALD_ERR_MISSING_WEIGHT (-4)
#define CALD_ERR_UNSUPPORTED (-5)

#define CALD_PRECISION_FP32 0
#define CALD_PRECISION_F16X3 1

#define CALD_ARCH_FRCNN 0
#define CALD_ARCH_RETINANET 1

const char* cald_last_error(void);
// ... 259 lines not shown
    int rect[CALD_PROBE_MAX_VIEWS][CALD_PROBE_MAX_RECTS][4];
    int Cin, Cout, KH, KW, stride, pad, relu, in_relu, out_ld;
    int cin_true;
    const float* weight;
    const float* bias;
    const float* bn_scale;
    const float* bn_shift;
    const float* in;
    const uint32_t* in16;
    const float* residual;
    const float* up;
    int ex16;
    const float* mask;
    const int* row_map;
    float* out; int64_t out_n;
    uint32_t* out16; int64_t out16_n;
    float* energy4; int64_t energy4_n;
    const float* head_w; const float* head_b;
    float* head_out; int64_t head_out_n; int head_ld;
    int row_packing;
} cald_conv_probe;
#define CALD_PROBE_PACK_AUTO 0
#define CALD_PROBE_PACK_OFF 1
#define CALD_PROBE_PACK_ON 2
int cald_op_conv_probe(cald_ctx* ctx, int precision, cald_conv_probe* probs, int n, int path, int tile, char* kernel, int kernel_cap);
int cald_op_row_pack_lookup(int V, const int* in_hw, const int* out_hw, int Cin, int out_ld, int64_t n, const int64_t* rows,
                            int* view_out, int64_t* local_out, int64_t* packed_rows_out);
int cald_op_mfma_f16(cald_ctx* ctx, const uint16_t* A, const uint16_t* B, const uint32_t* C, uint32_t* D, int64_t n);
int cald_op_conv_bench(cald_ctx* ctx, int n_views, int H, int W, int Cin, int Cout, int KH, int stride, int pad, int residual,
                       int relu, int iters, int group, double* ms_out, double* tflops_out);
int cald_op_transform_size(int H, int W, int min_size, int max_size, int* Hr, int* Wr, int* Hp, int* Wp);
int cald_debug_tensor(cald_model* m, const char* name, int view, float* host_out, int64_t capacity, int64_t* shape3);

#define CALD_JPEG_BASELINE 0
#define CALD_JPEG_GPU_EXTENDED 1
#define CALD_JPEG_HOST_ONLY 2
int cald_jpeg_info(const uint8_t* data, size_t size, int* H, int* W, int* ncomp);
int cald_jpeg_decode_batch(cald_ctx* ctx, int n, const uint8_t* const* data, const size_t* sizes, uint8_t* const* out_dev);
int cald_jpeg_probe(const uint8_t* data, size_t size, int* H, int* W, int* ncomp, int* kind);
int cald_jpeg_decode_batch_any(cald_ctx* ctx, int n, const uint8_t* const* data, const size_t* sizes, uint8_t* const* out_dev);
int cald_jpeg_decode_host(const uint8_t* data, size_t size, uint8_t* out_host);

int cald_profile_enable(cald_ctx* ctx, int on);
int cald_profile_read(cald_ctx* ctx, double* gemm_ms, double* gemm_flops, int64_t* gemm_launches, double* total_ms);
int cald_profile_prune(cald_ctx* ctx, double* lookahead_ms, double* lookahead_flops, double* selected_fraction_p2_p3, double* worst_bound_ratio,
                       double* pruned_flops);
int cald_profile_prune_fallbacks(cald_ctx* ctx, int64_t* n);
int cald_model_set_cutout_reuse(cald_model* m, int mode, int* was);
int cald_model_set_look_fuse(cald_model* m, int mode, int* was);
int cald_model_set_row_packing(cald_model* m, int mode, int* was);
int cald_model_set_box_min_size(cald_model* m, float min_size, float* was);
int cald_profile_cutout(cald_ctx* ctx, double* rows3, double* dense_rows3, int64_t* batches, int64_t* fallbacks);
int cald_profile_cutout_stages(cald_ctx* ctx, double* rows6, double* dense_rows6, double* tiles6, double* dense_tiles6, int64_t* kept3);
int cald_model_set_cutout_retention_cap(cald_model* m, int64_t bytes, int64_t* was);
int cald_debug_cutout_forward(cald_model* m, int n_views, const cald_view* views, const cald_dets* out, int prune);
int cald_profile_roi_rows(cald_ctx* ctx, double* mean_rows_per_view, int64_t* views);
int cald_profile_dump(cald_ctx* ctx, const char* path);

int cald_train_packed_floats(int Cout, int Cin, int KH, int KW, int CinK, int mode, int64_t* floats_out);
int cald_train_pack_conv(cald_ctx* ctx, const float* weight, const float* bias, const float* bn_scale, const float* bn_shift,
                         int Cout, int Cin, int KH, int KW, int CinK, int mode, float* packed);
typedef struct cald_pack_job {
    const float *weight, *bias, *bn_scale, *bn_shift;
    int Cout, Cin, KH, KW, CinK, mode;
    float* packed;
} cald_pack_job;
typedef struct cald_pack_plan cald_pack_plan;
int cald_train_pack_plan_scratch_floats(int n, const cald_pack_job* jobs, int64_t* floats_out);
int cald_train_pack_plan_create(cald_ctx* ctx, int n, const cald_pack_job* jobs, float* scratch, int64_t scratch_floats, cald_pack_plan** plan_out);
int cald_train_pack_plan_run(cald_ctx* ctx, const cald_pack_plan* plan);
int cald_train_pack_plan_destroy(cald_pack_plan* plan);
int cald_train_conv(cald_ctx* ctx, int N, int H, int W, const float* in, int CinK, const float* packed, int Cout, int Cin,
                    int KH, int KW, int stride, int pad, int mode, int flags, const float* residual, const float* up,
                    int Hup, int Wup, const float* mask, float* out, int out_ld);
int cald_train_conv_group(cald_ctx* ctx, int n, int N, const int* hw, const float* const* ins, int CinK, const float* const* packed,
                          int Cout, int Cin, int KH, int KW, int stride, int pad, int mode, int flags, const float* const* masks,
                          float* const* outs, int out_ld);
int cald_train_conv_wgrad(cald_ctx* ctx, int N, int H, int W, const float* x, int Cin, int ldx, const float* g, int Cout, int ldg,
                          int KH, int KW, int stride, int pad, const float* row_scale, float* dw, float* db, int accumulate);
int cald_train_linear_wgrad(cald_ctx* ctx, int R, const float* x, int K, const float* g, int Cout, int ldg, int taps,
                            float* dw, float* db, int accumulate);
enum { CALD_WGRAD_POINTWISE = 0, CALD_WGRAD_TABLE = 1, CALD_WGRAD_GENERAL = 2, CALD_WGRAD_GENERAL32 = 3, CALD_WGRAD_WIDE = 4 };
enum { CALD_WGRAD_REDUCE_FLAT = 0, CALD_WGRAD_REDUCE_TAPS = 1 };
typedef struct cald_wgrad_plan {
    int variant, reduce;
    int MT, JT;
    long long S, chunk;
    long long csplit, rows_per_block;
    long long scratch_bytes;
    char kernel[48], reduce_kernel[32];
} cald_wgrad_plan;
int cald_train_wgrad_plan(long long Q, int N, int H, int W, int Cin, int ldx, int Cout, int ldg, int KH, int KW, int stride, int pad,
                          int red_taps, cald_wgrad_plan* out);
int cald_train_relu_bwd(cald_ctx* ctx, long long rows, int C, float* g, const float* act, const float* scale);
int cald_train_add(cald_ctx* ctx, long long n, float* dst, const float* a, const float* b);
int cald_train_dilate(cald_ctx* ctx, int N, int Ho, int Wo, int C, int s, int Hd, int Wd, const float* g, float* out);
int cald_train_upsample_bwd(cald_ctx* ctx, int N, int Hf, int Wf, int Hc, int Wc, int C, const float* fine, float* coarse);
int cald_train_rpn_proposals(cald_ctx* ctx, int N, int Hp, int Wp, const int* image_sizes, const float* const* heads,
                             const int* level_hw, int head_ld, int pre_n, int post_n, float nms_thr, float min_size,
                             float* proposals_out, int* counts_out);
int cald_train_roi_sample_host(int N, const int* slots, const int* n_gt, const int* counts, const int32_t* matched,
                               const int64_t* gt_labels, const double* keys, int batch, double pos_fraction, int pred_ld, int num_classes,
                               int64_t* keep_rows, int64_t* gt_sel, int64_t* labels_out, float* img_col, int64_t* pos_rows,
                               int64_t* pred_idx, int* R_out, int* n_pos_out, int* per_image_out);
int cald_train_roi_gather(cald_ctx* ctx, const float* table, const float* gts, const int64_t* idx, int cap, int R, int n_pos,
                          float wx, float wy, float ww, float wh, float* rois_out, float* box_tgt_out);
// ... 50 lines not shown
```

Before: 183.3.

## Reuse kept RPN lookahead logits on cutout views via gathered-row fused conv

Adds a compact 4-wide lookahead head buffer in place of the 15-wide RPN head output, so the prune selector reads a narrower array. For cutout views it also retains the lookahead logits from the clean view and recomputes the fused RPN conv plus head only on the rows that the cutout geometry can affect, using a new gather variant of the h4 look kernel. Both paths are on by default and gated by a gather-cost threshold. This spends extra retained memory and plan-upload bytes to cut the P2/P3 RPN conv work on cutout views.

```diff
diff --git a/cald_amd/_ffi.py b/cald_amd/_ffi.py
--- a/cald_amd/_ffi.py
+++ b/cald_amd/_ffi.py
@@ -217,6 +217,11 @@
     "cald_model_set_cutout_retention_cap": (C.c_int, [C.c_void_p, C.c_int64, c_i64]),
     "cald_op_cutout_fpn_geometry": (C.c_int, [C.c_int, C.c_int, C.c_int, C.c_int, C.c_int, c_i, C.c_int, c_i, c_i]),
     "cald_model_set_look_fuse": (C.c_int, [C.c_void_p, C.c_int, c_i]),
+    "cald_model_set_look_compact": (C.c_int, [C.c_void_p, C.c_int, c_i]),
+    "cald_model_set_cutout_rpn_reuse": (C.c_int, [C.c_void_p, C.c_int, c_i]),
+    "cald_profile_cutout_rpn": (C.c_int, [C.c_void_p, c_d, c_d, c_d, c_d, c_i64, c_i64]),
+    "cald_op_cutout_rpn_geometry": (C.c_int, [C.c_int, C.c_int, C.c_int, C.c_int, C.c_int, c_i, C.c_int, c_i, c_i]),
+    "cald_op_rpn_prune_compact": (C.c_int, [C.c_void_p, C.POINTER(RpnPruneProbe), c_f, c_f]),
     "cald_model_set_row_packing": (C.c_int, [C.c_void_p, C.c_int, c_i]),
     "cald_model_set_box_min_size": (C.c_int, [C.c_void_p, C.c_float, c_f]),
     "cald_profile_dump": (C.c_int, [C.c_void_p, C.c_char_p]),
diff --git a/cald_amd/csrc/conv_h4.hip b/cald_amd/csrc/conv_h4.hip
--- a/cald_amd/csrc/conv_h4.hip
+++ b/cald_amd/csrc/conv_h4.hip
@@ -7,7 +7,7 @@
 #define H4_STAGE 32768
 #define H4_NSTAGE 4
 
-template <int EPI, bool HEAD = false>
+template <int EPI, bool HEAD = false, bool GATHER = false>
 __device__ __forceinline__ void conv_h4_body(const ConvArgs& a, const int blk) {
     extern __shared__ __attribute__((aligned(1024))) unsigned char smem[];
     const int tid = threadIdx.x, lane = tid & 63, wave = __builtin_amdgcn_readfirstlane(tid >> 6);
@@ -38,12 +38,14 @@
         Wi_l = Wi;
         int Mv = so.H * Wo;
         if (a.dyn_rows) { const int d = a.dyn_rows[v]; Mv = d < Mv ? d : Mv; }
+        if (GATHER) Mv = a.gather[v].cum[a.gather[v].nr];
         if (mt >= a.total_mtiles) Mv = 0;
         const int mrow0 = (mt - so.tile_start) * 128 + (lw & 1) * 64;
 #pragma unroll
         for (int i = 0; i < 4; i++) {
             const int m = mrow0 + 16 * i + l_row;
-            const int oy = m / Wo, ox = m - oy * Wo;
+            const int mp = GATHER ? (m < Mv ? gather_pixel(a.gather[v], m, Wo) : 0) : m;
+            const int oy = mp / Wo, ox = mp - oy * Wo;
             const int iy0 = oy * a.stride - a.pad, ix0 = ox * a.stride - a.pad;
             unsigned msk = 0;
             if (m < Mv)
@@ -242,7 +244,10 @@
                         s0 = __builtin_fmaf(hv.z, w[4 * g + 2], s0);
                         s0 = __builtin_fmaf(hv.w, w[4 * g + 3], s0);
                     }
-                    if (m < so.H * so.W) a.head_out[(so.pix_off + m) * (long long)a.head_ld + q] = s0 + a.head_b[q];
+                    if (GATHER) {
+                        const GatherSet& gs = a.gather[v];
+                        if (m < gs.cum[gs.nr]) a.head_out[(so.pix_off + gather_pixel(gs, m, so.W)) * (long long)a.head_ld + q] = s0 + a.head_b[q];
+                    } else if (m < so.H * so.W) a.head_out[(so.pix_off + m) * (long long)a.head_ld + q] = s0 + a.head_b[q];
                 }
             }
         }
@@ -279,14 +284,22 @@
     if (local >= (a.total_mtiles + 1) >> 1) return;
     conv_h4_body<0, true>(a, local);
 }
+__global__ __launch_bounds__(512, 2) void conv_h4_look_gather_kernel(const ConvGroup g) {
+    int i = 0;
+    while (i + 1 < g.n && g.blk0[i + 1] <= (int)blockIdx.x) i++;
+    const int local = (int)blockIdx.x - g.blk0[i];
+    const ConvArgs& a = g.p[i];
+    if (local >= (a.total_mtiles + 1) >> 1) return;
+    conv_h4_body<0, true, true>(a, local);
+}
 
 static bool h4_covers(const ConvArgs& a) {
     if (a.head_out && !(a.head_w && a.head_ld >= 3 && a.Cout == 256 && a.CoutPad == 256 && !a.residual && !a.up && !a.dyn_rows && a.bias && !a.scale && a.relu)) return false;
     return a.w16 && a.in16 && !a.in_relu && a.CoutPad % 256 == 0 && a.Cin % 16 == 0 && a.KH * a.KW <= 32 && !a.mask && !(a.residual && a.up) &&
-           !a.gather && !a.row_map && !a.energy4 && (a.out || a.out16 || a.head_out);
+           !(a.gather && !a.head_out) && !a.row_map && !a.energy4 && (a.out || a.out16 || a.head_out);
 }
 static int h4_mode() { static const int mode = getenv("CALD_H4") ? atoi(getenv("CALD_H4")) : 1; return mode; }
-static PerDeviceOnce h4_once[5];
+static PerDeviceOnce h4_once[6];
 const char* launch_conv_h4(const ConvArgs& a, hipStream_t stream, bool forced) {
     if (!(forced || h4_mode()) || !h4_covers(a) || a.head_out) return nullptr;
     const int wgs = ((a.total_mtiles + 1) >> 1) * (a.CoutPad >> 8);
@@ -302,9 +315,9 @@
 static int h4_group_plan(const ConvArgs* p, int n, bool forced, ConvGroup* g, int* blocks) {
     if (!(forced || h4_mode()) || n < 1 || n > CALD_MAX_GROUP) return 0;
     int blk = 0;
-    const bool head = p[0].head_out != nullptr;
+    const bool head = p[0].head_out != nullptr, gather = p[0].gather != nullptr;
     for (int i = 0; i < n; i++) {
-        if (!h4_covers(p[i]) || p[i].residual || p[i].up || (p[i].head_out != nullptr) != head) return 0;
+        if (!h4_covers(p[i]) || p[i].residual || p[i].up || (p[i].head_out != nullptr) != head || (p[i].gather != nullptr) != gather) return 0;
         if (g) { g->blk0[i] = blk; g->p[i] = p[i]; }
         blk += (((p[i].total_mtiles + 1) >> 1) * (p[i].CoutPad >> 8) + 7) & ~7;
     }
@@ -319,6 +332,11 @@
     const int take = h4_group_plan(p, n, forced, &g, &blk);
     if (!take) return nullptr;
     if (take == 2) return "none (no output tiles)";
+    if (p[0].head_out && p[0].gather) {
+        allow_big_lds(h4_once[5], conv_h4_look_gather_kernel);
+        hipLaunchKernelGGL(conv_h4_look_gather_kernel, dim3((unsigned)blk), dim3(512), (size_t)H4_NSTAGE * H4_STAGE, stream, g);
+        return "conv_h4_look_gather_kernel";
+    }
     if (p[0].head_out) {
         allow_big_lds(h4_once[4], conv_h4_look_kernel);
         hipLaunchKernelGGL(conv_h4_look_kernel, dim3((unsigned)blk), dim3(512), (size_t)H4_NSTAGE * H4_STAGE, stream, g);
diff --git a/cald_amd/csrc/ctx.hip b/cald_amd/csrc/ctx.hip
--- a/cald_amd/csrc/ctx.hip
+++ b/cald_amd/csrc/ctx.hip
@@ -185,6 +185,17 @@
     return 0;
 }
 
+extern "C" int cald_profile_cutout_rpn(cald_ctx* c, double* rows, double* dense_rows, double* tiles, double* dense_tiles, int64_t* gathered, int64_t* gated_off) {
+    if (!c) return fail(CALD_ERR_INVALID, "ctx is null");
+    if (rows) *rows = c->cut_rpn_rows;
+    if (dense_rows) *dense_rows = c->cut_rpn_dense;
+    if (tiles) *tiles = c->cut_rpn_tiles;
+    if (dense_tiles) *dense_tiles = c->cut_rpn_dense_tiles;
+    if (gathered) *gathered = c->cut_rpn_gathered;
+    if (gated_off) *gated_off = c->cut_rpn_gated_off;
+    return 0;
+}
+
 extern "C" int cald_profile_dump(cald_ctx* c, const char* path) {
     if (!c || !path) return fail(CALD_ERR_INVALID, "null argument");
     HIPCHK(hipStreamSynchronize(c->stream));
diff --git a/cald_amd/csrc/forward.hip b/cald_amd/csrc/forward.hip
--- a/cald_amd/csrc/forward.hip
+++ b/cald_amd/csrc/forward.hip
@@ -90,9 +90,11 @@
 struct PruneBufs {
     float *energy[2] = {}, *pn[2] = {}, *rows[2][2] = {}; int *map[2][2] = {}, *nsel[2] = {}; unsigned* p16[2] = {}; unsigned* tau = nullptr;
     float* look[2] = {};
+    float* look4[2] = {};
     void layout(Bump& B, const long long* px, int V, bool capture) {
         for (int i = 0; i < 2; i++) {
             energy[i] = B.get<float>(px[2 + i] * 4); pn[i] = B.get<float>(px[2 + i]); p16[i] = B.get<unsigned>(px[2 + i] * 256);
+            look4[i] = B.get<float>(px[2 + i] * 4);
             for (int s2 = 0; s2 < 2; s2++) { rows[s2][i] = B.get<float>(px[2 + i] * 15); map[s2][i] = B.get<int>(px[2 + i]); }
             if (capture) look[i] = B.get<float>(px[2 + i] * 15);
         }
@@ -256,6 +258,10 @@
 }
 bool cald_host::conv_pack_default() {
     static const bool on = !(getenv("CALD_CONV_PACK") && atoi(getenv("CALD_CONV_PACK")) == 0);
+    return on;
+}
+static bool look_compact_default() {
+    static const bool on = !(getenv("CALD_LOOK_COMPACT") && atoi(getenv("CALD_LOOK_COMPACT")) == 0);
     return on;
 }
 static void offer_packing(cald_model* m, ConvArgs& a, int lin, int lout, int lup, int V) {
@@ -475,7 +481,7 @@
         const bool kept = ru && ru->fpn && !retina;
         if (kept) {
             for (int i = 0; i < 4; i++) Fp.Pf[i] = ru->pf[i];
-            if (prune) for (int i = 0; i < 2; i++) { Fq.p16[i] = ru->p16[i]; Fq.energy[i] = ru->energy[i]; }
+            if (prune) for (int i = 0; i < 2; i++) { Fq.p16[i] = ru->p16[i]; Fq.energy[i] = ru->energy[i]; Fq.look4[i] = ru->look[i]; }
         }
         if ((rc = conv_on(m, m->fpn_inner[nl - 1], Fb.Cf[3], Fp.inner[nl - 1], 5, 5, V, false))) return rc;
         for (int i = nl - 2; i >= 0; i--)
@@ -546,20 +552,46 @@
         name_rpn(0);
         return 0;
     }
-    int look_fused_on(const ConvSpec* sp, bool* fused) {
+    int look_fused_on(const ConvSpec* sp, bool* fused, bool* compact) {
         ConvArgs a[2]; double flops = 0.0; int tiles = 0;
+        const bool cmp = !m->prune_capture && (m->look_compact < 0 ? look_compact_default() : m->look_compact != 0);
         for (int i = 0; i < 2; i++) {
             const double f = fill_conv_args(m, a[i], *sp[i].L, sp[i].in, nullptr, sp[i].level, sp[i].level, V, sp[i].relu);
             if (f < 0.0) return (int)f;
             a[i].in16 = sp[i].in16;
-            a[i].head_w = m->look_head_w; a[i].head_out = Fn.rpn_h[i]; a[i].head_ld = 15;
+            a[i].head_w = m->look_head_w; a[i].head_out = cmp ? Fq.look4[i] : Fn.rpn_h[i]; a[i].head_ld = cmp ? 4 : 15;
             for (int q = 0; q < 3; q++) a[i].head_b[q] = m->look_head_b[q];
             flops += f + 2.0 * (double)level_pix(m->plan, sp[i].level, V) * 256.0 * 3.0; tiles += a[i].total_mtiles;
         }
         if (!m->look_head_w || !conv_h4_group_takes(a, 2, m->look_fuse == 2)) return 0;
+        *compact = cmp;
         if (m->prune_capture)
             for (int i = 0; i < 2; i++) HIPCHK(hipMemsetAsync(Fn.rpn_h[i], 0, (size_t)level_pix(m->plan, 2 + i, V) * 15 * sizeof(float), st));
         ProfLaunch t; int rc;
+        if (ru && ru->mode == 2 && ru->fpn && ru->look[0] && ru->look[1]) {
+            ConvArgs g[2]; double gflops = 0.0, grows = 0.0; int gtiles = 0;
+            for (int i = 0; i < 2; i++) {
+                g[i] = a[i];
+                const char* base = ru->d_gp + (size_t)(2 * ru->nblk + 4 + i) * cut_plan_set_bytes(V);
+                g[i].seg_out = reinterpret_cast<const LevelSeg*>(base);
+                g[i].gather = reinterpret_cast<const GatherSet*>(base + (size_t)(V + 1) * sizeof(LevelSeg));
+                g[i].total_mtiles = ru->rpn_tiles[i];
+                gflops += 2.0 * ru->rpn_rows[i] * 256.0 * (2304.0 + 3.0); gtiles += ru->rpn_tiles[i]; grows += ru->rpn_rows[i];
+            }
+            const bool gathered = cmp && ru->gather_rpn && conv_h4_group_takes(g, 2, true);
+            const double drows = (double)(level_pix(m->plan, 2, V) + level_pix(m->plan, 3, V));
+            c->cut_rpn_rows += gathered ? grows : drows; c->cut_rpn_dense += drows;
+            c->cut_rpn_tiles += gathered ? gtiles : tiles; c->cut_rpn_dense_tiles += tiles;
+            (gathered ? c->cut_rpn_gathered : c->cut_rpn_gated_off)++;
+            if (gathered) {
+                *fused = true;
+                if (!gtiles) return 0;
+                if ((rc = prof_begin(c, t))) return rc;
+                const char* k = launch_conv_h4_group(g, 2, st, true);
+                if (!k) { prof_end(c, t, 0.0, c->prof_tag_now, "refused"); return conv_refused(g[0]); }
+                return prof_end(c, t, gflops, c->prof_tag_now, "mt=%d,Cin=%d,Cout=%d,k=%dx%d,s=%d,group=2,head=3,gathered-rows", gtiles, a[0].Cin, a[0].Cout, a[0].KH, a[0].KW, a[0].stride);
+            }
+        }
         if ((rc = prof_begin(c, t))) return rc;
         const char* k = launch_conv_h4_group(a, 2, st, m->look_fuse == 2);
         *fused = true;
@@ -580,11 +612,12 @@
         }
         pr.tau_key = Fq.tau; pr.stat = c->prof ? c->d_prune_stat : nullptr; pr.check = c->d_prune_check;
         for (int q = 0; q < 3; q++) { pr.c1[q] = m->prune_c1[q]; pr.c0[q] = m->prune_c0[q]; }
-        pr.head_ld = 15; pr.pre_n = m->cfg.rpn_pre_nms_top_n; pr.V = V;
+        pr.head_ld = 15; pr.head_in_ld = 15; pr.pre_n = m->cfg.rpn_pre_nms_top_n; pr.V = V;
         c->prof_tag_now = 1;
         for (int i = 0; i < 2; i++) { sp[i] = {&m->rpn_conv16, Fp.Pf[i], Fn.rpn_tl[i], 2 + i, true}; sp[i].in16 = Fq.p16[i]; }
-        bool fused = false;
-        rc = m->look_fuse ? look_fused_on(sp, &fused) : 0;
+        bool fused = false, compact = false;
+        rc = m->look_fuse ? look_fused_on(sp, &fused, &compact) : 0;
+        if (compact) { for (int i = 0; i < 2; i++) pr.head[i] = Fq.look4[i]; pr.head_in_ld = 4; }
         if (!rc && !fused) {
             rc = conv_group_on(m, sp, 2, V);
             for (int i = 0; i < 2; i++) sp[i] = {&m->rpn_head, Fn.rpn_tl[i], Fn.rpn_h[i], 2 + i, false};
diff --git a/cald_amd/csrc/host.h b/cald_amd/csrc/host.h
--- a/cald_amd/csrc/host.h
+++ b/cald_amd/csrc/host.h
@@ -60,6 +60,8 @@
     long long cut_batches = 0, cut_fallbacks = 0;
     double cut_st_rows[6] = {}, cut_st_dense[6] = {}, cut_st_tiles[6] = {}, cut_st_dense_tiles[6] = {};
     long long cut_kept[3] = {0, 0, 0};
+    double cut_rpn_rows = 0.0, cut_rpn_dense = 0.0, cut_rpn_tiles = 0.0, cut_rpn_dense_tiles = 0.0;
+    long long cut_rpn_gathered = 0, cut_rpn_gated_off = 0;
 };
 
 namespace cald_host {
@@ -115,6 +117,7 @@
     ConvLayer rpn_conv16; bool prune = false; float prune_c1[3] = {0, 0, 0}, prune_c0[3] = {0, 0, 0};
     bool prune_allowed = false;
     int look_fuse = 1; float* look_head_w = nullptr; float look_head_b[3] = {0, 0, 0};
+    int look_compact = -1, cut_rpn = -1;
     int row_packing = -1;
     bool prune_bound_voided = false;
     bool prune_capture = false;
@@ -172,6 +175,10 @@
     float* pf[4] = {}; unsigned* p16[2] = {}; float* energy[2] = {};
     int fpn_tiles[4] = {};
     double fpn_rows[4] = {};
+    float* look[2] = {};
+    bool gather_rpn = false;
+    int rpn_tiles[2] = {};
+    double rpn_rows[2] = {};
 };
 struct FwdFeatures {
     const int (*pad_to)[2] = nullptr;
diff --git a/cald_amd/csrc/host_logic.h b/cald_amd/csrc/host_logic.h
--- a/cald_amd/csrc/host_logic.h
+++ b/cald_amd/csrc/host_logic.h
@@ -346,6 +346,9 @@
     }
     for (int i = 0; i < 4; i++) outp[i] = cut_map(inner[i], 3, 1, 1, Hp >> (2 + i), Wp >> (2 + i));
 }
+static inline void cut_rpn_geometry(int Hp, int Wp, const CutSet* outp, CutSet* rpn2) {
+    for (int i = 0; i < 2; i++) rpn2[i] = cut_map(outp[i], 3, 1, 1, Hp >> (2 + i), Wp >> (2 + i));
+}
 static inline int cut_disjoint(const CutSet& s, CutRect* o, int cap) {
     int ys[2 * CUT_SET_MAX], ny = 0;
     for (int i = 0; i < s.n; i++) { ys[ny++] = s.r[i].y0; ys[ny++] = s.r[i].y1 + 1; }
diff --git a/cald_amd/csrc/kernels.h b/cald_amd/csrc/kernels.h
--- a/cald_amd/csrc/kernels.h
+++ b/cald_amd/csrc/kernels.h
@@ -173,6 +173,7 @@
     float* check;
     float c1[3], c0[3];
     int head_ld, pre_n, V;
+    int head_in_ld;
 };
 void launch_rpn_prune_select(const RpnPruneArgs& a, int max_pix, int stage, hipStream_t st);
 void launch_rpn_prune_scatter(const RpnPruneArgs& a, int max_pix, hipStream_t st);
diff --git a/cald_amd/csrc/model.hip b/cald_amd/csrc/model.hip
--- a/cald_amd/csrc/model.hip
+++ b/cald_amd/csrc/model.hip
@@ -338,6 +338,18 @@
     m->look_fuse = mode;
     return 0;
 }
+extern "C" int cald_model_set_look_compact(cald_model* m, int mode, int* was) {
+    if (!m || mode < -1 || mode > 1) return fail(CALD_ERR_INVALID, "bad argument");
+    if (was) *was = m->look_compact;
+    m->look_compact = mode;
+    return 0;
+}
+extern "C" int cald_model_set_cutout_rpn_reuse(cald_model* m, int mode, int* was) {
+    if (!m || mode < -1 || mode > 1) return fail(CALD_ERR_INVALID, "bad argument");
+    if (was) *was = m->cut_rpn;
+    m->cut_rpn = mode;
+    return 0;
+}
 extern "C" int cald_model_set_box_min_size(cald_model* m, float min_size, float* was) {
     if (!m || !(min_size >= 0.0f)) return fail(CALD_ERR_INVALID, "bad argument");
     if (m->cfg.arch != CALD_ARCH_FRCNN) return fail(CALD_ERR_INVALID, "box_min_size belongs to the Faster R-CNN tail (RetinaNet's always removes small boxes)");
diff --git a/cald_amd/csrc/ops.hip b/cald_amd/csrc/ops.hip
--- a/cald_amd/csrc/ops.hip
+++ b/cald_amd/csrc/ops.hip
@@ -49,6 +49,32 @@
         memset(q, 0, sizeof(int) * (1 + 4 * CUT_SET_MAX));
         q[0] = sets[e].n;
         for (int i = 0; i < sets[e].n; i++) { q[1 + 4 * i] = sets[e].r[i].x0; q[2 + 4 * i] = sets[e].r[i].y0; q[3 + 4 * i] = sets[e].r[i].x1; q[4 + 4 * i] = sets[e].r[i].y1; }
+    }
+    return 0;
+}
+extern "C" int cald_op_cutout_rpn_geometry(int H, int W, int min_size, int max_size, int nrect, const int* rects, int nblk, const int* strides, int* out) {
+    if (!out) return fail(CALD_ERR_INVALID, "bad argument");
+    std::vector<int> fpn((size_t)8 * (1 + 4 * CUT_SET_MAX));
+    if (int rc = cald_op_cutout_fpn_geometry(H, W, min_size, max_size, nrect, rects, nblk, strides, fpn.data())) return rc;
+    int Hr, Wr, Hp, Wp;
+    transform_size(H, W, min_size, max_size, &Hr, &Wr, &Hp, &Wp);
+    CutSet outp[2], rpn[2];
+    for (int i = 0; i < 2; i++) {
+        const int* q = fpn.data() + (size_t)(4 + i) * (1 + 4 * CUT_SET_MAX);
+        outp[i].n = q[0];
+        for (int k = 0; k < q[0]; k++) outp[i].r[k] = {q[1 + 4 * k], q[2 + 4 * k], q[3 + 4 * k], q[4 + 4 * k]};
+    }
+    cut_rpn_geometry(Hp, Wp, outp, rpn);
+    const int per = 1 + 4 * CUT_SET_MAX + 1 + 4 * CALD_GATHER_RECTS;
+    memset(out, 0, sizeof(int) * 2 * per);
+    for (int i = 0; i < 2; i++) {
+        int* q = out + (size_t)i * per;
+        q[0] = rpn[i].n;
+        for (int k = 0; k < rpn[i].n; k++) { q[1 + 4 * k] = rpn[i].r[k].x0; q[2 + 4 * k] = rpn[i].r[k].y0; q[3 + 4 * k] = rpn[i].r[k].x1; q[4 + 4 * k] = rpn[i].r[k].y1; }
+        CutRect rr[CALD_GATHER_RECTS];
+        int* d = q + 1 + 4 * CUT_SET_MAX;
+        d[0] = cut_disjoint(rpn[i], rr, CALD_GATHER_RECTS);
+        for (int k = 0; k < d[0]; k++) { d[1 + 4 * k] = rr[k].x0; d[2 + 4 * k] = rr[k].y0; d[3 + 4 * k] = rr[k].x1; d[4 + 4 * k] = rr[k].y1; }
     }
     return 0;
 }
@@ -644,8 +670,8 @@
     return 0;
 }
 
-extern "C" int cald_op_rpn_prune(cald_ctx* c, cald_rpn_prune_probe* p) {
-    if (!c || !p) return fail(CALD_ERR_INVALID, "cald_op_rpn_prune: null argument");
+static int rpn_prune_probe(cald_ctx* c, cald_rpn_prune_probe* p, const float* const* look4) {
+    if (!c || !p || (look4 && (!look4[0] || !look4[1]))) return fail(CALD_ERR_INVALID, "cald_op_rpn_prune: null argument");
     if (p->V < 1 || p->V > CALD_PRUNE_PROBE_MAX_VIEWS || p->guard < 0 || p->guard > 4096 || p->head_ld < 3 || p->head_ld > 64 || p->pre_n < 1)
         return fail(CALD_ERR_INVALID, "cald_op_rpn_prune: 1..%d views, guard 0..4096, head_ld 3..64, pre_n >= 1", CALD_PRUNE_PROBE_MAX_VIEWS);
     const int V = p->V, ld = p->head_ld; const size_t G = (size_t)p->guard;
@@ -676,6 +702,7 @@
         if ((rc = sd.upload(&pr.energy[l], p->energy[l], pix[l] * 16)) || (rc = sd.upload(&pr.pnorm[l], p->pnorm[l], (pix[l] + G) * 4)) ||
             (rc = sd.upload(&pr.head_out[l], p->head[l], (pix[l] + G) * ld * 4))) return rc;
         pr.head[l] = pr.head_out[l];
+        if (look4 && (rc = sd.upload(&pr.head[l], look4[l], pix[l] * 16))) return rc;
         for (int s = 0; s < 2; s++) {
             if ((rc = sd.upload(&pr.row_map[s][l], p->row_map[s][l], (pix[l] + G) * 4)) || (rc = sd.alloc(&d_rows[s][l], pix[l] * ld * 4))) return rc;
             pr.head_rows[s][l] = d_rows[s][l];
@@ -683,7 +710,7 @@
     }
     for (int s = 0; s < 2; s++) if ((rc = sd.upload(&pr.nsel[s], p->nsel[s], nw * 4))) return rc;
     for (int q = 0; q < 3; q++) { pr.c1[q] = p->c1[q]; pr.c0[q] = p->c0[q]; }
-    pr.head_ld = ld; pr.pre_n = p->pre_n; pr.V = V;
+    pr.head_ld = ld; pr.head_in_ld = look4 ? 4 : ld; pr.pre_n = p->pre_n; pr.V = V;
     auto maps_back = [&](int s) {
         HIPCHK(hipMemcpy(p->nsel[s], pr.nsel[s], nw * 4, hipMemcpyDeviceToHost));
         for (int l = 0; l < 2; l++) HIPCHK(hipMemcpy(p->row_map[s][l], pr.row_map[s][l], (pix[l] + G) * 4, hipMemcpyDeviceToHost));
@@ -719,6 +746,11 @@
     HIPCHK(hipMemcpy(p->check, pr.check, 8, hipMemcpyDeviceToHost));
     HIPCHK(hipMemcpy(p->stat, pr.stat, 32, hipMemcpyDeviceToHost));
     return 0;
+}
+extern "C" int cald_op_rpn_prune(cald_ctx* c, cald_rpn_prune_probe* p) { return rpn_prune_probe(c, p, nullptr); }
+extern "C" int cald_op_rpn_prune_compact(cald_ctx* c, cald_rpn_prune_probe* p, const float* look4_p2, const float* look4_p3) {
+    const float* const look4[2] = {look4_p2, look4_p3};
+    return rpn_prune_probe(c, p, look4);
 }
 
 extern "C" int cald_op_roi_align(cald_ctx* c, const float* const* feats, const int* level_hw, int C, int R, const float* rois, float* out) {
diff --git a/cald_amd/csrc/rpn_prune.hip b/cald_amd/csrc/rpn_prune.hip
--- a/cald_amd/csrc/rpn_prune.hip
+++ b/cald_amd/csrc/rpn_prune.hip
@@ -27,8 +27,8 @@
     const LevelSeg sg = a.seg[l][v];
     const int H = sg.H, W = sg.W, npx = H * W, A = 3, n = npx * A;
     const int k = n < a.pre_n ? n : a.pre_n;
-    const int ld = a.head_ld;
-    const float* head = a.head[l] + sg.pix_off * (long long)ld;
+    const int ld = a.head_ld, ldh = a.head_in_ld;
+    const float* head = a.head[l] + sg.pix_off * (long long)ldh;
     const float* en = a.energy[l] + sg.pix_off * 4;
     float* pnv = a.pnorm[l] + sg.pix_off;
     constexpr int ST = MODE == 2 ? 1 : 0;
@@ -63,7 +63,7 @@
                 for (int p = tid; p < npx; p += 1024) {
                     const float pn = pnv[p];
                     for (int an = 0; an < A; an++) {
-                        const unsigned key = det_orderable(head[(long long)p * ld + an] - bound(an, pn));
+                        const unsigned key = det_orderable(head[(long long)p * ldh + an] - bound(an, pn));
                         if ((key & msk) == prefix) atomicAdd(&hist[(key >> shift) & 255u], 1);
                     }
                 }
@@ -91,7 +91,7 @@
         const float pn = pnv[p];
         bool keep = false, first = false;
         for (int an = 0; an < A; an++) {
-            const float lg = head[(long long)p * ld + an];
+            const float lg = head[(long long)p * ldh + an];
             const float B = bound(an, pn);
             const float ub = lg + B, lb = lg - B;
             if (MODE == 1) keep = keep || !(lb == lb) || det_orderable(lb) >= tau;
@@ -141,13 +141,14 @@
     const float* src = a.head_rows[st][l] + sg.pix_off * (long long)ld;
     const float* pnv = a.pnorm[l] + sg.pix_off;
     float* dst = a.head_out[l] + sg.pix_off * (long long)ld;
+    const float* look = a.head[l] + sg.pix_off * (long long)a.head_in_ld;
     float worst = 0.0f;
     for (int i = blockIdx.x * 256 + threadIdx.x; i < ns * ld; i += gridDim.x * 256) {
         const int r = i / ld, c = i - r * ld;
         const int p = rmap[r];
         const float exact = src[i];
         if (c < 3) {
-            const float approx = dst[(long long)p * ld + c];
+            const float approx = look[(long long)p * a.head_in_ld + c];
             const float B = a.c1[c] * pnv[p] + a.c0[c];
             const float ratio = fabsf(approx - exact) / B;
             worst = (ratio == ratio) ? fmaxf(worst, ratio) : INFINITY;
diff --git a/cald_amd/csrc/sweep.hip b/cald_amd/csrc/sweep.hip
--- a/cald_amd/csrc/sweep.hip
+++ b/cald_amd/csrc/sweep.hip
@@ -61,6 +61,10 @@
 }
 static bool cut_reuse_env() {
     static const bool on = !(getenv("CALD_CUTOUT_REUSE") && atoi(getenv("CALD_CUTOUT_REUSE")) == 0);
+    return on;
+}
+static bool cut_rpn_env() {
+    static const bool on = !(getenv("CALD_CUTOUT_RPN") && atoi(getenv("CALD_CUTOUT_RPN")) == 0);
     return on;
 }
 #define CUT_GATHER_MAX_COST 0.7
@@ -207,7 +211,8 @@
         if (m->prune && prune_ok)
             for (int i = 0; i < 2; i++) {
                 char* p = take((size_t)level_pix(P, 2 + i, nv) * 256 * 4); char* e = take((size_t)level_pix(P, 2 + i, nv) * 4 * 4);
-                if (ru) { ru->p16[i] = reinterpret_cast<unsigned*>(p); ru->energy[i] = reinterpret_cast<float*>(e); }
+                char* a4 = take((size_t)level_pix(P, 2 + i, nv) * 4 * 4);
+                if (ru) { ru->p16[i] = reinterpret_cast<unsigned*>(p); ru->energy[i] = reinterpret_cast<float*>(e); ru->look[i] = reinterpret_cast<float*>(a4); }
             }
         if (ru) ru->fpn = true;
         return off;
@@ -368,16 +373,16 @@
     int cut_plan(int k, int V, const ViewDesc* vs, FwdReuse& ru) {
         cald_model::CutReuse& R = m->cr;
         const bool fpn = bt[k & 1].kept_fpn;
-        const size_t per = cut_plan_set_bytes(V), total = per * (2 * (size_t)nblk + (fpn ? 4 : 0));
+        const size_t per = cut_plan_set_bytes(V), total = per * (2 * (size_t)nblk + (fpn ? 6 : 0));
         if (!R.d_gp) {
-            const size_t cap = cut_plan_set_bytes(CALD_MAX_VIEWS) * (2 * CUT_MAX_BLOCKS + 4);
+            const size_t cap = cut_plan_set_bytes(CALD_MAX_VIEWS) * (2 * CUT_MAX_BLOCKS + 6);
             HIPCHK(hipMalloc((void**)&R.d_gp, cap));
             HIPCHK(hipHostMalloc((void**)&R.h_gp[0], cap)); HIPCHK(hipHostMalloc((void**)&R.h_gp[1], cap));
         }
         plan_of(V, vs, rplan[0]);
         const BatchPlan& P = rplan[0];
         char* const h = R.h_gp[k & 1];
-        std::vector<CutSet> g_out((size_t)V * ngeo), g_t1((size_t)V * ngeo), g_fpn((size_t)V * 4);
+        std::vector<CutSet> g_out((size_t)V * ngeo), g_t1((size_t)V * ngeo), g_fpn((size_t)V * 4), g_rpn((size_t)V * 2);
         for (int v = 0; v < V; v++) {
             int Hr, Wr, Hp, Wp; CutSet pool1;
             transform_size(vs[v].H, vs[v].W, m->cfg.min_size, m->cfg.max_size, &Hr, &Wr, &Hp, &Wp);
@@ -386,6 +391,7 @@
                 CutSet cs[4], inner[4];
                 for (int i = 0; i < 4; i++) cs[i] = g_out[(size_t)v * ngeo + c_blk[i]];
                 cut_fpn_geometry(Hp, Wp, cs, inner, &g_fpn[(size_t)v * 4]);
+                cut_rpn_geometry(Hp, Wp, &g_fpn[(size_t)v * 4], &g_rpn[(size_t)v * 2]);
             }
         }
         auto put_set = [&](size_t index, int lvl, const CutSet* sets, size_t stride_v, int* tiles_out, double* rows_out) {
@@ -457,6 +463,14 @@
             ru.gather_fpn = fpn && m->cr.mode != 2 && 128.0 * fg <= CUT_FPN_MAX_COST * frd;
             c->cut_st_rows[CUT_STAGE_OUTPUT] += ru.gather_fpn ? frg : frd; c->cut_st_dense[CUT_STAGE_OUTPUT] += frd;
             c->cut_st_tiles[CUT_STAGE_OUTPUT] += ru.gather_fpn ? fg : fd; c->cut_st_dense_tiles[CUT_STAGE_OUTPUT] += fd;
+            if (fpn && m->prune && prune_ok) {
+                double rg = 0.0, rd = 0.0;
+                for (int i = 0; i < 2; i++) {
+                    put_set(2 * (size_t)nblk + 4 + i, 2 + i, g_rpn.data() + i, 2, &ru.rpn_tiles[i], &ru.rpn_rows[i]);
+                    rg += ru.rpn_tiles[i]; rd += (double)level_pix(P, 2 + i, V);
+                }
+                ru.gather_rpn = m->cr.mode != 2 && (m->cut_rpn < 0 ? cut_rpn_env() : m->cut_rpn != 0) && 128.0 * rg <= CUT_GATHER_MAX_COST * rd;
+            }
         }
         if (hipMemcpyAsync(R.d_gp, h, total, hipMemcpyHostToDevice, c->stream) != hipSuccess) return fail(CALD_ERR_HIP, "H2D of the cut_out gather plan failed");
         ru.mode = 2; ru.nblk = nblk; ru.d_gp = R.d_gp;
diff --git a/cald_amd/detector.py b/cald_amd/detector.py
--- a/cald_amd/detector.py
+++ b/cald_amd/detector.py
@@ -229,6 +229,16 @@
         _ffi.check(_ffi.lib().cald_model_set_look_fuse(self.handle(), int(mode), C.byref(was)))
         return was.value
 
+    def set_look_compact(self, mode):
+        was = C.c_int(0)
+        _ffi.check(_ffi.lib().cald_model_set_look_compact(self.handle(), int(mode), C.byref(was)))
+        return was.value
+
+    def set_cutout_rpn_reuse(self, mode):
+        was = C.c_int(0)
+        _ffi.check(_ffi.lib().cald_model_set_cutout_rpn_reuse(self.handle(), int(mode), C.byref(was)))
+        return was.value
+
     def set_rpn_prune_capture(self, on):
         _ffi.check(_ffi.lib().cald_model_set_rpn_prune_capture(self.handle(), int(bool(on))))
 
diff --git a/include/cald_hip.h b/include/cald_hip.h
--- a/include/cald_hip.h
+++ b/include/cald_hip.h
@@ -335,6 +335,11 @@
 int cald_model_set_box_min_size(cald_model* m, float min_size, float* was);
 int cald_profile_cutout(cald_ctx* ctx, double* rows3, double* dense_rows3, int64_t* batches, int64_t* fallbacks);
 int cald_profile_cutout_stages(cald_ctx* ctx, double* rows6, double* dense_rows6, double* tiles6, double* dense_tiles6, int64_t* kept3);
+int cald_model_set_look_compact(cald_model* m, int mode, int* was);
+int cald_model_set_cutout_rpn_reuse(cald_model* m, int mode, int* was);
+int cald_profile_cutout_rpn(cald_ctx* ctx, double* rows, double* dense_rows, double* tiles, double* dense_tiles, int64_t* gathered, int64_t* gated_off);
+int cald_op_cutout_rpn_geometry(int H, int W, int min_size, int max_size, int nrect, const int* rects, int nblk, const int* strides, int* out);
+int cald_op_rpn_prune_compact(cald_ctx* ctx, cald_rpn_prune_probe* p, const float* look4_p2, const float* look4_p3);
 int cald_model_set_cutout_retention_cap(cald_model* m, int64_t bytes, int64_t* was);
 int cald_debug_cutout_forward(cald_model* m, int n_views, const cald_view* views, const cald_dets* out, int prune);
 int cald_profile_roi_rows(cald_ctx* ctx, double* mean_rows_per_view, int64_t* views);
```

After: 184.7, median of 6. Within noise of the previous version (+0.8%).
